# neverorfrog/vehicle-control

Measured on AMD Instinct MI355X. Metric: MPC solves/sec (batched, N=20), higher is better.
Workload: dtype f64; 1 GPU; C2 kinematic-bicycle LTV-MPC, B=1024 per GPU, N=20, fp64; batch_per_gpu=1024, global_batch=1024, horizon=20, parallelism=dp1 (independent shards)

## Files before the change

### include/vcmpc.h

```cpp
#ifndef VCMPC_H
#define VCMPC_H

#include <stdint.h>

#ifdef __cplusplus
extern "C" {
#endif

#define VCMPC_ABI_VERSION 13
#define VC_MAX_OBSTACLES 16

typedef struct vc_ctx vc_ctx;

enum vc_model { VC_MODEL_KINEMATIC = 0, VC_MODEL_DYNAMIC = 1, VC_MODEL_CASCADED = 2 };
enum vc_dtype { VC_F64 = 0, VC_F32 = 1 };
enum vc_flags { VC_HOST_PTRS = 0, VC_DEVICE_PTRS = 1 };
enum vc_tyre { VC_TYRE_FIALA = 0, VC_TYRE_LINEAR = 1 };
enum vc_status { VC_SOLVED = 0, VC_MAX_ITER = 1, VC_NONFINITE = 2, VC_OUT_OF_DOMAIN = 3, VC_INFEASIBLE = 4 };
enum vc_error {
  VC_OK = 0,
  VC_E_ARG = -1,
  VC_E_HIP = -2,
  VC_E_UNSUPPORTED = -3
};

typedef struct vc_kin_car {
  double l;
} vc_kin_car;

typedef struct vc_dyn_car {
  double l, m, Izz, a, b, h, eps, Peng;
  double Xdf, Xdr, Xbf, Xbr;
  double Caf, Car;
  double Cd, muf, mur, theta, phi, Av2, Frr;
  int32_t tyre;
  int32_t pad_;
} vc_dyn_car;

typedef struct vc_kin_mpc {
  double w_time, w_ey, w_epsi, w_v, w_w, w_a, w_dev, w_b;
  double a_min, a_max, w_min, w_max;
  double v_min, v_max, delta_min, delta_max, ey_min, ey_max;
  double w_obs;
} vc_kin_mpc;

typedef struct vc_dyn_mpc {
  double w_time, w_speed, w_ey, w_epsi, w_w, w_Fx, w_dev, w_b, w_slip;
  double w_min, w_max;
  double Ux_min, max_speed, delta_min, delta_max, ey_min, ey_max;
  double fx_scale;
  double trust_Fx;
  int32_t sqp_iters;
  int32_t pad_;
  double w_obs;
} vc_dyn_mpc;

typedef struct vc_qp {
  double prox;
  double tol;
  double trust_a;
  double trust_w;
  int32_t max_iter;
  int32_t polish;
  int32_t solver;
  int32_t kin_sqp;
  int32_t shift;
  int32_t ms;
  double elastic;
} vc_qp;

typedef struct vc_casc_mpc {
  int32_t horizon_pm;
  int32_t pad_;
  double ds_pm;
  double w_dev_pm, w_Fy, w_switch;
  double V_min, ey_min_pm, ey_max_pm;
} vc_casc_mpc;

typedef struct vc_obstacles {
  int32_t n;
  int32_t inside;
  double margin_min;
  double s[VC_MAX_OBSTACLES], ey[VC_MAX_OBSTACLES], radius[VC_MAX_OBSTACLES];
} vc_obstacles;

typedef struct vc_params {
  vc_kin_car kin_car;
  vc_dyn_car dyn_car;
  vc_kin_mpc kin_mpc;
  vc_qp qp;
  vc_dyn_mpc dyn_mpc;
  vc_obstacles obs;
  vc_casc_mpc casc;
} vc_params;

int vc_abi_version(void);
int vc_params_sizeof(void);

vc_ctx* vc_create(int device, int model, int N, int max_batch, int dtype, const vc_params* params);
void vc_destroy(vc_ctx* ctx);
const char* vc_last_error(const vc_ctx* ctx);

int vc_set_stream(vc_ctx* ctx, void* stream);

int vc_set_obstacles(vc_ctx* ctx, int n, const double* s, const double* ey, const double* radius,
                     double margin_min);
int vc_synchronize(vc_ctx* ctx);

int vc_set_infeasibility(vc_ctx* ctx, int on, double eps);

int vc_get_farkas(vc_ctx* ctx, int B, void* y, int flags);

int vc_set_sqp_infeasibility(vc_ctx* ctx, int on, double eps);

int vc_get_sqp_farkas(vc_ctx* ctx, int B, void* y, int32_t* qp_index, int flags);

int vc_set_sqp_regularization(vc_ctx* ctx, int levels, double factor);

int vc_get_sqp_regularization(vc_ctx* ctx, int B, int32_t* level, int flags);

int vc_set_casc_infeasibility(vc_ctx* ctx, int on, double eps);

int vc_get_casc_farkas(vc_ctx* ctx, int B, void* y, int32_t* qp_index, int flags);

int vc_solve(vc_ctx* ctx, int B, const void* x0, const void* kappa, const void* ds,
             void* xbar, void* ubar, void* u0, int32_t* status, int32_t* iters, int flags);

int vc_solve_from(vc_ctx* ctx, int B, const void* x0, const void* kappa, const void* ds, const void* ubar_in,
                  void* xbar, void* u_out, void* u0, int32_t* status, int32_t* iters, int flags);

int vc_solve_diag(vc_ctx* ctx, int B, const void* x0, const void* kappa, const void* ds,
                  void* xbar, void* ubar, void* u0, int32_t* status, int32_t* iters, void* diag,
                  int flags);

int vc_solve_debug(vc_ctx* ctx, int B, const void* x0, const void* kappa, const void* ds, void* xbar, void* ubar,
                   void* u0, int32_t* status, int32_t* iters, void* dbg, int flags);
int vc_debug_stride(void);

int vc_debug_qp_fault(vc_ctx* ctx, int sqp_iter, int problem);

int vc_debug_kin_merit(vc_ctx* ctx, int B, const void* x0, const void* kappa, const void* ds, const void* u_prev,
                       void* u, const void* x_prev, void* x, int32_t* status, int32_t* iters, int32_t* st_acc,
                       int32_t* it_acc, int first, int restart, void* u0, void* ls_diag, int flags);

int vc_debug_sqp_breakdown(vc_ctx* ctx, int sqp_iter, int problem, int levels);

int vc_debug_rcp(vc_ctx* ctx, int n, const void* x, void* out, int flags);

int vc_debug_kin_gdots(vc_ctx* ctx, int B, const void* G, const void* vz, const void* vc, void* out_grow,
                       void* out_gt, int flags);

int vc_rollout(vc_ctx* ctx, int B, const void* x0, const void* ubar, const void* kappa,
               const void* ds, void* xbar, int flags);

int vc_linearize(vc_ctx* ctx, int B, const void* xbar, const void* ubar, const void* kappa,
                 const void* ds, void* A, void* Bm, int flags);

int vc_condense(vc_ctx* ctx, int B, const void* x0, const void* ubar, const void* kappa,
                const void* ds, void* H, void* g, int flags);

int vc_plant_step(vc_ctx* ctx, int B, const void* x, const void* u, const void* kappa,
                  double dt, void* x_next, int flags);

int vc_spatial_step(vc_ctx* ctx, int B, const void* x, const void* u, const void* kappa,
                    const void* ds, void* x_next, int flags);

int vc_ode(vc_ctx* ctx, int B, const void* x, const void* u, const void* kappa, int space, void* f, int flags);

int vc_track_set(vc_ctx* ctx, int n_pieces, double h, double length, const double* coef);

int vc_track_k(vc_ctx* ctx, int B, const void* s, void* k, int flags);

int vc_horizon(vc_ctx* ctx, int B, const void* x0, const void* xbar, double mpc_dt, void* kappa, void* ds,
               int flags);

int vc_drive(vc_ctx* ctx, int B, double* x64, const void* u0, double dt, void* x_ctx, int flags);

int vc_simulate(vc_ctx* ctx, int B, int steps, double mpc_dt, double dt, double* x64, void* xbar, void* ubar,
                double* log_x, void* log_u, int32_t* nfail, int flags);

#ifdef __cplusplus
}
#endif
#endif
```

### vehicle-control_amd/csrc/kin_ltv.hip

```cpp
#include <hip/hip_runtime.h>

#include <cstdint>

#include "vc_kernels.hpp"
#include "vc_models.hpp"
#include "vcmpc.h"

#ifndef VC_KIN_LTV_DET
#define VC_KIN_LTV_DET 0
#endif

#ifndef KIN_NU_TOL
#define KIN_NU_TOL 1e-10
#endif
#ifndef KIN_EARLY_F
#define KIN_EARLY_F 100.0
#endif
#ifndef KIN_EARLY_ROUNDS
#define KIN_EARLY_ROUNDS 2
#endif
#ifndef KIN_TAPIA_F
#define KIN_TAPIA_F 1.02
#endif
#ifndef KIN_DUAL_TOL
#define KIN_DUAL_TOL 1e-12
#endif
#ifndef KIN_AL_RHO
#define KIN_AL_RHO 1e1
#endif
#ifndef KIN_DOT_CH
#define KIN_DOT_CH 8
#endif
#ifndef KIN_UPDATE
#define KIN_UPDATE 1
#endif
#ifndef KIN_RSQ_HALLEY
#define KIN_RSQ_HALLEY 1
#endif
#ifndef KIN_STAT_CHECK
#define KIN_STAT_CHECK 0
#endif
#ifndef KIN_STEP_F
#define KIN_STEP_F 0.99
#endif
#ifndef KIN_SOLVE_CH
#define KIN_SOLVE_CH 8
#endif
#ifndef KIN_PANEL_CH
#define KIN_PANEL_CH 6
#endif

#ifndef KIN_XPOSE_ONCE
#define KIN_XPOSE_ONCE 1
#endif

namespace vc {
namespace {

__device__ __forceinline__ double lane_bcast(double v, int src) {
  const int lo = __builtin_amdgcn_readlane(__double2loint(v), src);
  const int hi = __builtin_amdgcn_readlane(__double2hiint(v), src);
  return __hiloint2double(hi, lo);
}
__device__ int amdgcn_writelane(int v, int lane, int old) __asm("llvm.amdgcn.writelane.i32");
__device__ __forceinline__ double lane_put(double old, double v, int dst) {
  const int lo = amdgcn_writelane(__double2loint(v), dst, __double2loint(old));
  const int hi = amdgcn_writelane(__double2hiint(v), dst, __double2hiint(old));
  return __hiloint2double(hi, lo);
}
template <int K>
__device__ __forceinline__ double dpp_row_shr(double v, double ident) {
  const int lo = __builtin_amdgcn_update_dpp(__double2loint(ident), __double2loint(v), 0x110 + K, 0xf, 0xf, false);
  const int hi = __builtin_amdgcn_update_dpp(__double2hiint(ident), __double2hiint(v), 0x110 + K, 0xf, 0xf, false);
  return __hiloint2double(hi, lo);
}
template <typename Op>
__device__ __forceinline__ double wave_reduce(double v, double ident, Op op) {
  v = op(v, dpp_row_shr<1>(v, ident));
  v = op(v, dpp_row_shr<2>(v, ident));
  v = op(v, dpp_row_shr<4>(v, ident));
  v = op(v, dpp_row_shr<8>(v, ident));
  return op(op(lane_bcast(v, 15), lane_bcast(v, 31)), op(lane_bcast(v, 47), lane_bcast(v, 63)));
}
__device__ __forceinline__ double wave_sum(double v) {
  return wave_reduce(v, 0.0, [](double a, double b) { return a + b; });
}
__device__ __forceinline__ double wave_max(double v) {
  return wave_reduce(v, -__builtin_inf(), [](double a, double b) { return fmax(a, b); });
}
__device__ __forceinline__ double wave_min(double v) {
  return wave_reduce(v, __builtin_inf(), [](double a, double b) { return fmin(a, b); });
}
__device__ __forceinline__ void wave_sync() {
  asm volatile("" ::: "memory");
  __builtin_amdgcn_wave_barrier();
  asm volatile("" ::: "memory");
}
__device__ __forceinline__ void fence() { __builtin_amdgcn_sched_barrier(0); }
__device__ __forceinline__ int lane_opaque(int lane) {
  asm volatile("" : "+v"(lane));
  return lane;
}
__device__ __forceinline__ uint32_t lane_range_pick(uint32_t in, int other, int lo, int hi) {
  uint32_t r;
  asm("s_bfm_b64 vcc, %3, %4\n\t"
      "v_mov_b32_e32 %0, %2\n\tv_cndmask_b32_e32 %0, %0, %1, vcc"
      : "=&v"(r)
      : "v"(in), "i"(other), "i"(hi - lo), "i"(lo)
      : "vcc");
  return r;
}
__device__ __forceinline__ void no_hoist() { asm volatile("" ::: "memory"); }

using lds_cdouble = const __attribute__((address_space(3))) double;
__device__ __forceinline__ lds_cdouble* lds_opaque(const double* p) {
  uint32_t a = (uint32_t)(uintptr_t)(lds_cdouble*)p;
  asm volatile("" : "+v"(a));
  return (lds_cdouble*)(uintptr_t)a;
}

#ifdef VC_TIMING
#define VC_TSTAMP(var) \
  fence();              \
  const uint64_t var = __builtin_amdgcn_s_memtime(); \
  fence();
#define VC_TACC(slot, t0) \
  {                      \
    fence();             \
    tacc[slot] += __builtin_amdgcn_s_memtime() - (t0); \
    fence();             \
  }
#else
#define VC_TSTAMP(var)
#define VC_TACC(slot, t0)
#endif
enum { T_SWEEP = 0, T_SETUP, T_RESID, T_BUILD, T_CHOL, T_SOLVE, T_UPDATE, T_POLISH, T_OUT, T_S2, T_S3, T_S4, T_PAL, T_PPASS, T_NUPD, T_UCYC, T_NDROP, T_CFAIL, T_CRM, T_CADD, T_R0CHG, T_STEP, T_TOTAL, T_NSLOT };


template <int N>
struct Dims {
  static constexpr int n = 2 * N;
  static constexpr int NC = 2 * (N - 1);
  static constexpr int LD = n + 1;
  static_assert(n <= 64 && N >= 2, "one wavefront per problem needs 2 <= N <= 32");
};

template <int n>
__host__ __device__ constexpr int lc_base(int k) {
  static_assert(n % 2 == 0, "even n");
  return k * (n - 1) - k * (k - 1) / 2 + (k + 1) / 2;
}
template <int n>
__host__ __device__ constexpr int lc_start(int k) {
  return lc_base<n>(k) + k;
}

template <int N>
struct Smem {
  using D = Dims<N>;
  static constexpr int LC_DUMMY = lc_start<D::n>(D::n);
  static constexpr int LC_ZERO = LC_DUMMY + 1;
  double G[D::NC + 3][D::LD];
  double H[D::n + 1][D::LD];
  alignas(16) double Lc[LC_ZERO + 1];
  alignas(16) double zrow[48];
  double xb[N + 1][KIN_NX + 1];
  double jac[N + 1][9];
  double ub[D::n];
  double kap[N], ds[N];
  union {
    struct {
      double vz[64];
      double vc[64];
    };
    alignas(16) double tb2[128];
  };
  double dinv[64];
#if KIN_XPOSE_ONCE
  alignas(16) double tb3[8 * 18];
#endif
};
static_assert(sizeof(Smem<20>) <= 40960, "LDS of one problem: four must fit a CU's 160 KB");

template <int N>
__host__ __device__ constexpr int crow_stage(int r) {
  return r < N - 1 ? r + 1 : r - (N - 1) + 1;
}

template <int LEN, int SA, int SB, int CH = KIN_DOT_CH>
__device__ __forceinline__ double lds_dot(lds_cdouble* a, lds_cdouble* b) {
  constexpr int NCH = (LEN + CH - 1) / CH;
  double ca[2][CH], cb[2][CH];
  auto fetch = [&](int c, int buf) {
#pragma unroll
    for (int q = 0; q < CH; ++q) {
      const int i = c * CH + q;
      ca[buf][q] = (i < LEN) ? a[i * SA] : 0.0;
      cb[buf][q] = (i < LEN) ? b[i * SB] : 0.0;
    }
  };
  double a0 = 0.0, a1 = 0.0;
  fetch(0, 0);
#pragma unroll
  for (int c = 0; c < NCH; ++c) {
    if (c + 1 < NCH) fetch(c + 1, (c + 1) & 1);
    fence();
#pragma unroll
    for (int q = 0; q < CH; q += 2) {
      a0 += ca[c & 1][q] * cb[c & 1][q];
      a1 += ca[c & 1][q + 1] * cb[c & 1][q + 1];
    }
  }
  fence();
  return a0 + a1;
}

template <int N>
struct GSplit {
  static_assert(N == 20, "the lane plan below is worked out for N = 20 (the one instantiation)");
  static constexpr int NC = Dims<N>::NC, n = Dims<N>::n, LD = Dims<N>::LD;
  static constexpr int T = NC / 2;
  static constexpr int ROW_SHORT = T - (T + 1) / 2;
  static_assert(NC + 2 * (N - 1 - ROW_SHORT) <= 64, "partner lanes of the long rows");
  static constexpr int COL_LONG = n / 2;
  static_assert(n + COL_LONG <= 64, "partner lanes of the long columns");
};

__device__ __forceinline__ double lane_fetch(double v, int byte_lane) {
  const int lo = __builtin_amdgcn_ds_bpermute(byte_lane, __double2loint(v));
  const int hi = __builtin_amdgcn_ds_bpermute(byte_lane, __double2hiint(v));
  return __hiloint2double(hi, lo);
}

template <int T0, int T1, int GS, int D>
__device__ __forceinline__ void gsplit_fetch(double (&a)[5], double (&b)[5], uint32_t g, uint32_t v) {
  static_assert(2 * T0 - D >= 0, "offsets from a segment base are not negative");
  lds_cdouble* gp = (lds_cdouble*)(uintptr_t)g;
  lds_cdouble* vp = (lds_cdouble*)(uintptr_t)v;
#pragma unroll
  for (int t = T0; t < T1; ++t) {
    a[t - T0] = gp[(2 * t - D) * GS];
    b[t - T0] = vp[2 * t - D];
  }
}
template <int CNT>
__device__ __forceinline__ double gsplit_fma(const double (&a)[5], const double (&b)[5], double acc) {
#pragma unroll
  for (int q = 0; q < CNT; ++q) acc = __builtin_fma(a[q], b[q], acc);
  return acc;
}
template <int N, int GS, int D2, int D3>
__device__ __forceinline__ double gsplit_chain(const uint32_t (&g)[4], const uint32_t (&v)[4], bool shrt,
                                               double& stash) {
  static_assert(GSplit<N>::T == 19, "segments of 5, 5, 4 and 5 steps");
  double a0[5], b0[5], a1[5], b1[5];
  gsplit_fetch<0, 5, GS, 0>(a0, b0, g[0], v[0]);
  gsplit_fetch<5, 10, GS, 0>(a1, b1, g[1], v[1]);
  fence();
  double acc = gsplit_fma<5>(a0, b0, 0.0);
  gsplit_fetch<10, 14, GS, D2>(a0, b0, g[2], v[2]);
  fence();
  acc = gsplit_fma<5>(a1, b1, acc);
  gsplit_fetch<14, 19, GS, D3>(a1, b1, g[3], v[3]);
  fence();
  stash = acc;
  acc = shrt ? 0.0 : acc;
  acc = gsplit_fma<4>(a0, b0, acc);
  fence();
  acc = gsplit_fma<5>(a1, b1, acc);
  fence();
  return acc;
}

template <int N>
__device__ double grow_dot(const Smem<N>& s, int lane) {
  using P = GSplit<N>;
  constexpr int NC = P::NC, LD = P::LD;
  const int l = lane_opaque(lane);
  const bool part = l >= NC;
  const bool shrt = uint32_t(l) < uint32_t(P::ROW_SHORT) || uint32_t(l - (N - 1)) < uint32_t(P::ROW_SHORT);
  const int r = min(part ? l - (l < NC + (N - 1 - P::ROW_SHORT) ? NC - P::ROW_SHORT : N) : l, NC);
  const uint32_t odd = part ? 8u : 0u;
  const uint32_t fwd = shrt ? 0u : 8u * uint32_t(P::T);
  const uint32_t g0 = (uint32_t)(uintptr_t)(lds_cdouble*)&s.G[0][0] + uint32_t(r) * (8u * LD) + odd;
  const uint32_t v0 = (uint32_t)(uintptr_t)(lds_cdouble*)&s.vz[0] + odd;
  const uint32_t g[4] = {g0, g0, g0 + fwd, g0 + fwd}, v[4] = {v0, v0, v0 + fwd, v0 + fwd};
  double stash;
  const double acc = gsplit_chain<N, 1, P::T, P::T>(g, v, shrt, stash);
  const double other = lane_fetch(acc, 4 * (l + (l < N - 1 ? NC - P::ROW_SHORT : N)));
  const double y = acc + (shrt ? stash : other);
  return l < NC ? y : 0.0;
}

template <int N>
__device__ double gt_dot(const Smem<N>& s, int lane) {
  using P = GSplit<N>;
  constexpr int n = P::n, LD = P::LD;
  const int l = lane_opaque(lane);
  const bool part = l >= n;
  const bool shrt = uint32_t(l - P::COL_LONG) < uint32_t(n - P::COL_LONG);
  const int j = part ? l - n : l;
  const uint32_t ms = shrt ? 1u : 0u, mp = part ? 1u : 0u;
  const uint32_t gp = (uint32_t)(uintptr_t)(lds_cdouble*)&s.G[0][0] + uint32_t(j) * 8u + mp * (8u * LD);
  const uint32_t vp = (uint32_t)(uintptr_t)(lds_cdouble*)&s.vc[0] + mp * 8u;
  constexpr int SH[4] = {10, 18, 0, 1}, D[4] = {0, 0, 9, 0};
  uint32_t g[4], v[4];
#pragma unroll
  for (int k = 0; k < 4; ++k) {
    g[k] = gp + uint32_t(D[k] * 8 * LD) + ms * uint32_t((SH[k] - D[k]) * 8 * LD);
    v[k] = vp + uint32_t(D[k] * 8) + ms * uint32_t((SH[k] - D[k]) * 8);
  }
  double stash;
  const double acc = gsplit_chain<N, LD, D[2], D[3]>(g, v, shrt, stash);
  const double other = lane_fetch(acc, 4 * (l + n));
  const double y = acc + (shrt ? stash : other);
  return l < n ? y : 0.0;
}


template <int N>
__device__ double h_dot(const Smem<N>& s, int lane) {
  constexpr int n = Dims<N>::n;
  const int j = lane < n ? lane : 0;
  return lds_dot<n, 1, 1>(lds_opaque(&s.H[j][0]), lds_opaque(&s.vz[0]));
}

__device__ __forceinline__ void kin_sincos(double x, double& sn, double& cs) {
  const double n = __builtin_rint(x * 6.36619772367581382433e-01);
  const double y = fma(-n, 6.07710050650619224932e-11, fma(-n, 1.57079632673412561417e+00, x));
  const double z = y * y;
  const double rs = fma(z, fma(z, fma(z, fma(z, 1.58969099521155010221e-10, -2.50507602534068634195e-08),
                                      2.75573137070700676789e-06), -1.98412698298579493134e-04),
                        8.33333333332248946124e-03);
  const double sk = fma(z * y, fma(z, rs, -1.66666666666666324348e-01), y);
  const double rc = z * fma(z, fma(z, fma(z, fma(z, fma(z, -1.13596475577881948265e-11, 2.08757232129817482790e-09),
                                                  -2.75573143513906633035e-07), 2.48015872894767294178e-05),
                                   -1.38888888888741095749e-03), 4.16666666666666019037e-02);
  const double hz = 0.5 * z, w = 1.0 - hz;
  const double ck = w + (((1.0 - w) - hz) + z * rc);
  const int q = int(n) & 3;
  const double a = (q & 1) ? ck : sk, b = (q & 1) ? sk : ck;
  sn = (q & 2) ? -a : a;
  cs = ((q + 1) & 2) ? -b : b;
}

__device__ __forceinline__ double rsq_nr(double d) {
  double inv = __builtin_amdgcn_rsq(d);
#if KIN_RSQ_HALLEY
  const double e = fma(-d, inv * inv, 1.0);
  return fma(inv * e, fma(0.375, e, 0.5), inv);
#else
  inv = inv * (1.5 - 0.5 * d * inv * inv);
  inv = inv * (1.5 - 0.5 * d * inv * inv);
  return inv;
#endif
}

template <int N>
__device__ __forceinline__ void store_rows(const double (&Mr)[Dims<N>::n], Smem<N>& s, int lane) {
}

template <int N>
struct RowRegs {
  int lo[Dims<N>::n], hi[Dims<N>::n];
};
template <int N>
__device__ __forceinline__ void row_put(RowRegs<N>& R, int k, double v) {
  asm("v_accvgpr_write_b32 %0, %1" : "=a"(R.lo[k]) : "v"(__double2loint(v)));
  asm("v_accvgpr_write_b32 %0, %1" : "=a"(R.hi[k]) : "v"(__double2hiint(v)));
}
#define KIN_FS_STEP(k, w, lo)                    \
  "v_mul_f64 v[252:253], %[acc], %[dj]\n\t"      \
  "s_bfm_b64 exec, " #w ", " #lo "\n\t"          \
  "v_readlane_b32 vcc_lo, v252, " #k "\n\t"      \
  "v_readlane_b32 vcc_hi, v253, " #k "\n\t"      \
  "v_accvgpr_read_b32 v254, %[l" #k "]\n\t"      \
  "v_accvgpr_read_b32 v255, %[h" #k "]\n\t"      \
  "v_fma_f64 %[acc], -v[254:255], vcc, %[acc]\n\t"
#define KIN_FS_ROW(k) [l##k] "a"(Lr.lo[k]), [h##k] "a"(Lr.hi[k])
template <int N>
__device__ __forceinline__ void forward_sweep(const RowRegs<N>& Lr, double& acc, double dj) {
  static_assert(Dims<N>::n == 40, "the sweep's 40 steps are written out");
  asm("s_mov_b64 s[98:99], exec\n\t"
      KIN_FS_STEP(0,63,1) KIN_FS_STEP(1,62,2) KIN_FS_STEP(2,61,3)
      KIN_FS_STEP(3,60,4) KIN_FS_STEP(4,59,5) KIN_FS_STEP(5,58,6)
      KIN_FS_STEP(6,57,7) KIN_FS_STEP(7,56,8) KIN_FS_STEP(8,55,9)
      KIN_FS_STEP(9,54,10) KIN_FS_STEP(10,53,11) KIN_FS_STEP(11,52,12)
      KIN_FS_STEP(12,51,13) KIN_FS_STEP(13,50,14) KIN_FS_STEP(14,49,15)
      KIN_FS_STEP(15,48,16) KIN_FS_STEP(16,47,17) KIN_FS_STEP(17,46,18)
      KIN_FS_STEP(18,45,19) KIN_FS_STEP(19,44,20) KIN_FS_STEP(20,43,21)
      KIN_FS_STEP(21,42,22) KIN_FS_STEP(22,41,23) KIN_FS_STEP(23,40,24)
      KIN_FS_STEP(24,39,25) KIN_FS_STEP(25,38,26) KIN_FS_STEP(26,37,27)
      KIN_FS_STEP(27,36,28) KIN_FS_STEP(28,35,29) KIN_FS_STEP(29,34,30)
      KIN_FS_STEP(30,33,31) KIN_FS_STEP(31,32,32) KIN_FS_STEP(32,31,33)
      KIN_FS_STEP(33,30,34) KIN_FS_STEP(34,29,35) KIN_FS_STEP(35,28,36)
      KIN_FS_STEP(36,27,37) KIN_FS_STEP(37,26,38) KIN_FS_STEP(38,25,39)
      KIN_FS_STEP(39,24,40)
      "s_mov_b64 exec, s[98:99]"
      : [acc] "+v"(acc)
      : [dj] "v"(dj),
        KIN_FS_ROW(0), KIN_FS_ROW(1), KIN_FS_ROW(2), KIN_FS_ROW(3), KIN_FS_ROW(4), KIN_FS_ROW(5),
        KIN_FS_ROW(6), KIN_FS_ROW(7), KIN_FS_ROW(8), KIN_FS_ROW(9), KIN_FS_ROW(10), KIN_FS_ROW(11),
        KIN_FS_ROW(12), KIN_FS_ROW(13), KIN_FS_ROW(14), KIN_FS_ROW(15), KIN_FS_ROW(16), KIN_FS_ROW(17),
        KIN_FS_ROW(18), KIN_FS_ROW(19), KIN_FS_ROW(20), KIN_FS_ROW(21), KIN_FS_ROW(22), KIN_FS_ROW(23),
        KIN_FS_ROW(24), KIN_FS_ROW(25), KIN_FS_ROW(26), KIN_FS_ROW(27), KIN_FS_ROW(28), KIN_FS_ROW(29),
        KIN_FS_ROW(30), KIN_FS_ROW(31), KIN_FS_ROW(32), KIN_FS_ROW(33), KIN_FS_ROW(34), KIN_FS_ROW(35),
        KIN_FS_ROW(36), KIN_FS_ROW(37), KIN_FS_ROW(38), KIN_FS_ROW(39)
      : "vcc", "s98", "s99", "v252", "v253", "v254", "v255");
}
#undef KIN_FS_STEP
#undef KIN_FS_ROW

template <int N>
__device__ double chol_solve(const RowRegs<N>& Lr, const Smem<N>& s, double b, int lane) {
  constexpr int n = Dims<N>::n;
  constexpr int CH = KIN_SOLVE_CH;
  static_assert(n % CH == 0, "backward prefetch chunks");
  const int row = lane < n ? lane : 0;
  lds_cdouble* col = lds_opaque(&s.Lc[lc_base<n>(row)]);
  const double dj = s.dinv[row];
  double acc = b;
  forward_sweep<N>(Lr, acc, dj);
  acc *= dj;
  double x = 0.0;
  double lk[2][CH];
  lds_cdouble* zero = lds_opaque(&s.zrow[0]);
  auto fetch = [&](int c, int buf) {
    lds_cdouble* src = row < n - 1 - c * CH ? col : zero;
#pragma unroll
    for (int q = 0; q < CH; ++q) lk[buf][q] = src[n - 1 - c * CH - q];
  };
  fetch(0, 0);
#pragma unroll
  for (int c = 0; c < n / CH; ++c) {
    if (c + 1 < n / CH) fetch(c + 1, (c + 1) & 1);
    fence();
#pragma unroll
    for (int q = 0; q < CH; ++q) {
      const int k = n - 1 - c * CH - q;
      const double xk = lane_bcast(acc * dj, k);
      x = lane_put(x, xk, k);
      acc -= lk[c & 1][q] * xk;
    }
    fence();
  }
  return x;
}

enum { ROWS_G = 0, ROWS_E = 1 };
template <int N, int KIND>
__host__ __device__ constexpr int row_extent(int r) {
  if (KIND == ROWS_G) return r < Dims<N>::NC ? 2 * crow_stage<N>(r) : 0;
  return r < N ? 2 * (r + 1) : (r < N + 2 ? 2 * N : 0);
}
template <int N, int KIND>
__host__ __device__ constexpr int gram_rows() {
  return KIND == ROWS_G ? Dims<N>::NC : N + 2;
}
template <int N, int KIND>
__host__ __device__ constexpr bool kstep_hits(int ks, int I) {
  for (int q = 0; q < 4; ++q)
    if (row_extent<N, KIND>(4 * ks + q) > 16 * I) return true;
  return false;
}

using d4 = __attribute__((ext_vector_type(4))) double;
using d2 = __attribute__((ext_vector_type(2))) double;
template <int N>
struct Tiles {
  static constexpr int n = Dims<N>::n, NB = (n + 15) / 16, NT = NB * (NB + 1) / 2, BLD = 16 * NB + 2;
  static constexpr int count(bool full) { return full ? NB * NB : NT; }
};

template <int N, int KIND, bool FULL>
__device__ __forceinline__ void gram_mfma(d4 (&acc)[Tiles<N>::count(FULL)], const double* rows, const double* w,
                                          int lane) {
  constexpr int n = Dims<N>::n, LD = Dims<N>::LD, NB = Tiles<N>::NB;
  constexpr int KS = (gram_rows<N, KIND>() + 3) / 4;
  lane = lane_opaque(lane);
  const int lr = lane >> 4, lc = lane & 15;
  lds_cdouble* R = lds_opaque(rows);
  lds_cdouble* W = lds_opaque(w);
  double gk[KS][NB], wk[KS];
#pragma unroll
  for (int ks = 0; ks < KS; ++ks) {
    const int r = 4 * ks + lr;
    wk[ks] = W[r];
#pragma unroll
    for (int J = 0; J < NB; ++J) {
      const int c = 16 * J + lc;
      gk[ks][J] = R[r * LD + (c < n ? c : n)];
    }
  }
  fence();
#pragma unroll
  for (int ks = 0; ks < KS; ++ks) {
#pragma unroll
    for (int I = 0, t = 0; I < NB; ++I) {
      const double a = wk[ks] * gk[ks][I];
#pragma unroll
      for (int J = 0; J < (FULL ? NB : I + 1); ++J, ++t)
        if (kstep_hits<N, KIND>(ks, I > J ? I : J))
          acc[t] = __builtin_amdgcn_mfma_f64_16x16x4f64(a, gk[ks][J], acc[t], 0, 0, 0);
    }
  }
}

template <int N, bool FULL>
__device__ __forceinline__ void tiles_to_rows(double (&Mr)[Dims<N>::n], const d4 (&acc)[Tiles<N>::count(FULL)],
                                              Smem<N>& s, int lane) {
  constexpr int n = Dims<N>::n, NB = Tiles<N>::NB, BLD = Tiles<N>::BLD;
  static_assert(16 * BLD <= Smem<N>::LC_DUMMY, "transpose buffer must fit the factor storage");
  static_assert(16 * NB <= 48, "zero row length");
  lane = lane_opaque(lane);
  const int lr = lane >> 4, lc = lane & 15;
  double* buf = &s.Lc[0];
  const int myI = lane >> 4;
#pragma unroll
  for (int I = 0, t0 = 0; I < NB; ++I, t0 += FULL ? NB : I) {
    wave_sync();
#pragma unroll
    for (int J = 0; J < (FULL ? NB : I + 1); ++J) {
#pragma unroll
      for (int q = 0; q < 4; ++q) buf[(lr + 4 * q) * BLD + 16 * J + lc] = acc[t0 + J][q];
    }
    wave_sync();
    using lds_cd2 = const __attribute__((address_space(3))) d2;
    lds_cd2* brow = (lds_cd2*)lds_opaque(myI == I ? &buf[lc * BLD] : &s.zrow[0]);
#pragma unroll
    for (int i = 0; i < n; i += 2) {
      const int iend = FULL ? n : 16 * (I + 1);
      if (i < iend) {
        const d2 p = brow[i / 2];
        if (I == 0) { Mr[i] = p.x; Mr[i + 1] = p.y; }
        else { Mr[i] += p.x; Mr[i + 1] += p.y; }
      } else if (I == 0) {
        Mr[i] = 0.0;
        Mr[i + 1] = 0.0;
      }
    }
  }
  wave_sync();
}

template <int N>
__device__ __forceinline__ void build_normal_acc(d4 (&acc)[Tiles<N>::NT], Smem<N>& s, double wb, double hjj, int lane) {
  constexpr int n = Dims<N>::n, LD = Dims<N>::LD, NB = Tiles<N>::NB;
  static_assert(4 * ((Dims<N>::NC + 3) / 4) <= Dims<N>::NC + 2, "G zero rows cover the last k-step");
  lane = lane_opaque(lane);
  const int lr = lane >> 4, lc = lane & 15;
  const int jd = lane < n ? lane : n;
  s.H[jd][jd] = hjj + wb;
  wave_sync();
  {
    lds_cdouble* H = lds_opaque(&s.H[0][0]);
#pragma unroll
    for (int I = 0, t = 0; I < NB; ++I) {
#pragma unroll
      for (int J = 0; J <= I; ++J, ++t) {
        const int c = 16 * J + lc < n ? 16 * J + lc : n;
#pragma unroll
        for (int q = 0; q < 4; ++q) {
          const int r0 = 16 * I + 4 * q;
          acc[t][q] = r0 < n ? H[(r0 + lr) * LD + c] : 0.0;
        }
      }
    }
  }
  s.H[jd][jd] = hjj;
  gram_mfma<N, ROWS_G, false>(acc, &s.G[0][0], &s.vc[0], lane);
}

template <int N>
__device__ __forceinline__ void build_normal_mfma(double (&Mr)[Dims<N>::n], Smem<N>& s, double wb, double hjj,
                                                  int lane) {
  d4 acc[Tiles<N>::NT];
  build_normal_acc<N>(acc, s, wb, hjj, lane);
  tiles_to_rows<N, false>(Mr, acc, s, lane);
}

template <int N>
__device__ bool factor_blocked(RowRegs<N>& Lr, d4 (&acc)[Tiles<N>::NT], Smem<N>& s, int lane) {
  constexpr int n = Dims<N>::n, NB = Tiles<N>::NB;
  double Mr[n];
  constexpr int DUMMY = Smem<N>::LC_DUMMY;
  static_assert(NB == 3 && n > 32 && n <= 40, "three panels, the last one at most 8 wide");
  static_assert(lc_start<n>(16) + 16 * 18 <= DUMMY, "panel 0/1 transpose buffer inside the factor storage");
  static_assert((lc_start<n>(16) & 1) == 0, "16-byte aligned transpose buffer");
  lane = lane_opaque(lane);
  const int lr = lane >> 4, lc = lane & 15, myI = lane >> 4;
  bool ok = true;
  double pa, pb, pc, pi1, pl21, pi2;
  using lds_double = __attribute__((address_space(3))) double;
  using lds_char = __attribute__((address_space(3))) char;
  const uint32_t lane8 = 8u * uint32_t(lane);
  auto col_store = [&](int k, double v) {
    const uint32_t off = lane_range_pick(lane8, 8 * (DUMMY - lc_base<n>(k)), k, n);
    *(lds_double*)((lds_char*)&s.Lc[lc_base<n>(k)] + off) = v;
  };
  auto part = [&](int p, int k) {
    if (p == 0) {
      pa = lane_bcast(Mr[k], k);
      pb = lane_bcast(Mr[k], k + 1);
      pc = lane_bcast(Mr[k + 1], k + 1);
      pi1 = rsq_nr(pa);
    } else if (p == 1) {
      pl21 = pb * pi1;
      const double d2 = fma(-pl21, pl21, pc);
      pi2 = rsq_nr(d2);
      ok = ok && (pa > 0.0) && (d2 > 0.0);
    } else {
      const double x = Mr[k] * pi1;
      const double y = fma(-x, pl21, Mr[k + 1]) * pi2;
      Mr[k] = x;
      Mr[k + 1] = y;
      col_store(k, x);
      col_store(k + 1, y);
      s.dinv[k] = pi1;
      s.dinv[k + 1] = pi2;
    }
  };
  using lds_cd2 = const __attribute__((address_space(3))) d2;
#pragma unroll
  for (int p = 0; p < NB; ++p) {
    const int c0 = 16 * p, c1 = (16 * p + 16 < n) ? 16 * p + 16 : n, W = c1 - c0;
    double* tb = p < 2 ? &s.Lc[lc_start<n>(16)] : &s.tb2[0];
    const int TS = p < 2 ? 18 : 10;
#if KIN_XPOSE_ONCE
    static_assert(2 * 16 * 18 + 8 * 18 <= DUMMY, "panel 0's three buffers inside the factor storage");
    {
      auto tbuf = [&](int I) -> double* {
        return p == 0 ? &s.Lc[16 * 18 * I] : (p == 1 ? (I == 1 ? tb : &s.tb3[0]) : tb);
      };
      wave_sync();
#pragma unroll
      for (int I = p; I < NB; ++I) {
        const int t = I * (I + 1) / 2 + p;
        double* tbI = tbuf(I);
#pragma unroll
        for (int q = 0; q < 4; ++q) {
          const int r = lr + 4 * q;
          if (16 * I + 4 * q < n)
            tbI[(lc < W ? r * TS + lc : 8 * TS + lc)] = acc[t][q];
        }
      }
      wave_sync();
      const double* own = p == 0 ? &s.Lc[16 * 18 * myI + lc * TS]
                                 : (p == 1 ? (myI == 1 ? &tb[lc * TS] : &s.tb3[lc * TS]) : &tb[lc * TS]);
      lds_cd2* src = (lds_cd2*)lds_opaque(myI >= p && lane < n ? own : &s.zrow[0]);
#pragma unroll
      for (int i = 0; i < W; i += 2) {
        const d2 v = src[i / 2];
        Mr[c0 + i] = 0.0 + v.x;
        Mr[c0 + i + 1] = 0.0 + v.y;
      }
    }
#else
#pragma unroll
    for (int i = c0; i < c1; ++i) Mr[i] = 0.0;
#pragma unroll
    for (int I = p; I < NB; ++I) {
      const int t = I * (I + 1) / 2 + p;
      wave_sync();
#pragma unroll
      for (int q = 0; q < 4; ++q) {
        const int r = lr + 4 * q;
        if (4 * q < W)
          tb[(lc < W ? r * TS + lc : 8 * TS + lc)] = acc[t][q];
      }
      wave_sync();
      lds_cd2* src = (lds_cd2*)lds_opaque(myI == I && lc < W ? &tb[lc * TS] : &s.zrow[0]);
#pragma unroll
      for (int i = 0; i < W; i += 2) {
        const d2 v = src[i / 2];
        Mr[c0 + i] += v.x;
        Mr[c0 + i + 1] += v.y;
      }
    }
#endif
    wave_sync();
    part(0, c0);
    part(1, c0);
    part(2, c0);
#pragma unroll
    for (int k = c0; k + 2 < c1; k += 2) {
      wave_sync();
      fence();
      const double x = Mr[k], y = Mr[k + 1];
      const double* cA = &s.Lc[lc_base<n>(k)];
      const double* cB = &s.Lc[lc_base<n>(k + 1)];
      constexpr int CH = KIN_PANEL_CH;
      const int J0 = k + 4, NCH = (c1 - J0 + CH - 1) / CH;
      double u0[2][CH], u1[2][CH];
      auto load = [&](int ch, int buf) {
#pragma unroll
        for (int q = 0; q < CH; ++q) {
          const int j = J0 + ch * CH + q;
          u0[buf][q] = j < c1 ? cA[j] : 0.0;
          u1[buf][q] = j < c1 ? cB[j] : 0.0;
        }
      };
      if (NCH > 0) load(0, 0);
#pragma unroll
      for (int j = k + 2; j < k + 4; ++j)
        Mr[j] = fma(-y, lane_bcast(y, j), fma(-x, lane_bcast(x, j), Mr[j]));
      part(0, k + 2);
#pragma unroll
      for (int ch = 0; ch < NCH; ++ch) {
        if (ch + 1 < NCH) load(ch + 1, (ch + 1) & 1);
        fence();
#pragma unroll
        for (int q = 0; q < CH; ++q) {
          const int j = J0 + ch * CH + q;
          if (j < c1) Mr[j] = fma(-y, u1[ch & 1][q], fma(-x, u0[ch & 1][q], Mr[j]));
        }
        if (ch + 1 < 3) part(ch + 1, k + 2);
        fence();
      }
#pragma unroll
      for (int pp = NCH + 1; pp < 3; ++pp) {
        part(pp, k + 2);
        fence();
      }
    }
    wave_sync();
    if (p + 1 < NB) {
      lds_cdouble* Lc = lds_opaque(&s.Lc[0]);
      lds_cdouble* Z = lds_opaque(&s.zrow[0]);
#pragma unroll
      for (int ks = 0; ks < W / 4; ++ks) {
        const int kk = c0 + 4 * ks + lr;
        double op[NB];
#pragma unroll
        for (int I = p + 1; I < NB; ++I) {
          const int jj = 16 * I + lc;
          op[I] = jj < n ? Lc[lc_base<n>(kk) + jj] : Z[0];
        }
#pragma unroll
        for (int I = p + 1; I < NB; ++I) {
#pragma unroll
          for (int J = p + 1; J <= I; ++J) {
            const int t = I * (I + 1) / 2 + J;
            acc[t] = __builtin_amdgcn_mfma_f64_16x16x4f64(-op[I], op[J], acc[t], 0, 0, 0);
          }
        }
      }
    }
  }
#pragma unroll
  for (int k = 0; k < n; ++k) row_put<N>(Lr, k, Mr[k]);
  wave_sync();
  return ok;
}

__device__ __forceinline__ double wave_prefix(double v, int lane) {
  v += dpp_row_shr<1>(v, 0.0);
  v += dpp_row_shr<2>(v, 0.0);
  v += dpp_row_shr<4>(v, 0.0);
  v += dpp_row_shr<8>(v, 0.0);
  const double r0 = lane_bcast(v, 15), r1 = lane_bcast(v, 31), r2 = lane_bcast(v, 47);
  return v + (lane >= 16 ? r0 : 0.0) + (lane >= 32 ? r1 : 0.0) + (lane >= 48 ? r2 : 0.0);
}

template <int N>
__device__ bool factor_update(RowRegs<N>& Lr, Smem<N>& s, int upd, int j, bool fixed, double sqrho,
                              int lane) {
  constexpr int n = Dims<N>::n;
  double Mr[n];
  constexpr int DUMMY = Smem<N>::LC_DUMMY, ZERO = Smem<N>::LC_ZERO;
  lane = lane_opaque(lane);
  const int row = lane < n ? lane : 0;
  auto below = [&](int k, int other) { return lane > k && lane < n ? lc_base<n>(k) + lane : other; };
  double z;
  if (upd == 1) {
    z = s.Lc[below(j, ZERO)];
    wave_sync();
    s.Lc[below(j, DUMMY)] = 0.0;
    s.Lc[lane < j ? lc_base<n>(lane) + j : DUMMY] = 0.0;
    s.Lc[lc_start<n>(j)] = 1.0;
    s.dinv[j] = 1.0;
  } else {
    z = (lane < n && !fixed) ? sqrho * s.G[j][lane < n ? lane : n] : 0.0;
  }
  wave_sync();
  {
    lds_cdouble* L = lds_opaque(&s.Lc[0]);
#pragma unroll
    for (int k = 0; k < n; ++k) Mr[k] = L[below(k, ZERO)];
  }
#pragma unroll
  for (int k = 0; k < n; ++k) row_put<N>(Lr, k, Mr[k]);
  const double dj = s.dinv[row];
  double acc = z;
  forward_sweep<N>(Lr, acc, dj);
  const double y = lane < n ? acc * dj : 0.0;
  const double t = 1.0 + wave_prefix(y * y, lane);
  const double sk = sqrt(t / (t - y * y)), ck = y / t;
  const bool ok = __ballot(!(sk > 0.5 && sk < 1e150)) == 0ull;
  wave_sync();
  if (lane < n) {
    s.Lc[lc_start<n>(row)] *= sk;
    s.dinv[row] = dj / sk;
  }
  s.tb2[2 * lane] = ck;
  s.tb2[2 * lane + 1] = sk;
  wave_sync();
  {
    using lds_cd2 = const __attribute__((address_space(3))) d2;
    lds_cd2* cs = (lds_cd2*)lds_opaque(&s.tb2[0]);
    double w = z;
#pragma unroll
    for (int k = 0; k < n - 1; ++k) {
      const double yk = lane_bcast(y, k);
      const d2 c = cs[k];
      w = lane_put(w, 0.0, k);
      const double l = Mr[k];
      w = fma(-yk, l, w);
      Mr[k] = fma(c.x, w, l) * c.y;
    }
  }
#pragma unroll
  for (int k = 0; k < n - 1; ++k) s.Lc[below(k, DUMMY)] = Mr[k];
#pragma unroll
  for (int k = 0; k < n; ++k) row_put<N>(Lr, k, Mr[k]);
  wave_sync();
  return ok;
}

struct Side {
  double lo, hi, slo, shi, llo, lhi;
  bool hasLo, hasHi;
};

}

template <int N, bool DET>
__global__ __launch_bounds__(64) void kin_ltv_kernel(KinLtvArgs A) {
  using D = Dims<N>;
  constexpr int n = D::n, NC = D::NC;
  __shared__ Smem<N> s;
  const int lane = threadIdx.x;
  const int b = xcd_problem(blockIdx.x, A.B);
  if (b >= A.B) return;
  const vc_kin_mpc& W = A.w;
#ifdef VC_TIMING
  uint64_t tacc[T_NSLOT] = {};
#endif
  VC_TSTAMP(t_all0)

  if (lane < n) s.ub[lane] = A.ubar[(size_t)b * n + lane];
  if (lane < N) {
    s.kap[lane] = A.kappa[(size_t)b * N + lane];
    s.ds[lane] = A.ds[(size_t)b * N + lane];
  }
  if (lane < KIN_NX) s.xb[0][lane] = A.x0[(size_t)b * KIN_NX + lane];
  for (int i = lane; i < 2 * D::LD; i += 64) (&s.G[NC][0])[i] = 0.0;
  if (lane < 48) s.zrow[lane] = 0.0;
  if (lane == 0) s.Lc[Smem<N>::LC_ZERO] = 0.0;
  wave_sync();

  VC_TSTAMP(t_sweep0)
  constexpr int LD = Dims<N>::LD;
  double* E = &s.H[0][0];
  bool finite = true;
  {
    double x[KIN_NX];
#pragma unroll
    for (int i = 0; i < KIN_NX; ++i) x[i] = s.xb[0][i];
#pragma unroll 1
    for (int k = 0; k < N; ++k) {
      const double u2[2] = {s.ub[2 * k], s.ub[2 * k + 1]};
      const double h = s.ds[k];
      double f[KIN_NX];
      {
        double sn, cs;
        kin_sincos((lane & 1) ? x[1] : x[4], sn, cs);
        const double se = lane_bcast(sn, 0), ce = lane_bcast(cs, 0);
        const double sd = lane_bcast(sn, 1), cd = lane_bcast(cs, 1);
        const double kap = s.kap[k];
        const double rho = 1.0 - x[3] * kap;
        const int r4 = lane & 3;
        const double num = r4 == 0 ? se : (r4 == 1 ? sd : rho);
        const double den = r4 == 0 ? ce : (r4 == 1 ? cd * A.L : (r4 == 2 ? ce : x[0] * ce));
        const double quo = num * rcp_nr(den);
        const double te = lane_bcast(quo, 0), tdl = lane_bcast(quo, 1);
        const double rc = lane_bcast(quo, 2), q = lane_bcast(quo, 3);
        f[0] = q * u2[0];
        f[1] = q * u2[1];
        f[2] = 1.0;
        f[3] = rho * te;
        f[4] = tdl * rc - kap;
        f[5] = q;
      }
#pragma unroll
      for (int i = 0; i < KIN_NX; ++i) x[i] += h * f[i];
      if (lane == 0) {
#pragma unroll
        for (int i = 0; i < KIN_NX; ++i) s.xb[k + 1][i] = x[i];
      }
    }
#pragma unroll
    for (int i = 0; i < KIN_NX; ++i) finite = finite && isfinite(x[i]);
  }
  wave_sync();
  if (lane < N) {
    const double ey = s.xb[lane + 1][3];
    double cw, lin;
    if (lane + 1 < N) {
      const double hs = s.ds[lane + 1];
      const double td = W.w_dev * hs;
      double tb = W.w_b * hs;
      asm volatile("" : "+v"(tb));
      cw = td;
      lin = ey * td;
      if (ey < W.ey_min) { cw = __builtin_fma(W.w_dev, hs, tb); lin = __builtin_fma(ey - W.ey_min, tb, lin); }
      if (ey > W.ey_max) { cw = cw + tb; lin = __builtin_fma(ey - W.ey_max, tb, lin); }
    } else {
      cw = W.w_ey;
      lin = W.w_ey * ey;
    }
    s.vc[lane] = 2.0 * cw;
    s.vz[lane] = 2.0 * lin;
  }
  wave_sync();
  VC_TACC(T_SWEEP, t_sweep0)
  VC_TSTAMP(t_s20)
  {
    const int k = lane < N ? lane : 0;
    double xk[KIN_NX];
#pragma unroll
    for (int i = 0; i < KIN_NX; ++i) xk[i] = s.xb[k][i];
    const KinJac J = kin_spatial_jac(xk, s.kap[k], A.L);
    double* jr = s.jac[lane < N ? lane : N];
    jr[0] = J.q; jr[1] = J.qv; jr[2] = J.qey; jr[3] = J.qep;
    jr[4] = J.J33; jr[5] = J.J34; jr[6] = J.J41; jr[7] = J.J43; jr[8] = J.J44;
    if (A.obs.n > 0 && lane >= 1 && lane < N) {
      double p, q;
      obstacle_ey_model<double>(A.obs, xk[2], xk[3], W.w_obs * s.ds[k], p, q);
      s.vc[k - 1] += q;
      s.vz[k - 1] += p;
    }
  }
  wave_sync();
  VC_TACC(T_S2, t_s20)
  VC_TSTAMP(t_s30)
  double gj = 0.0;
  double cv = 0, cd = 0, cey = 0, cep = 0, ct = 0;
  {
    const int jcol = lane < n ? lane : n;
    double jn[9], hn, an, wn;
    auto fetch = [&](int k) {
#pragma unroll
      for (int q = 0; q < 9; ++q) jn[q] = s.jac[k][q];
      hn = s.ds[k]; an = s.ub[2 * k]; wn = s.ub[2 * k + 1];
    };
    fetch(0);
#pragma unroll 1
    for (int k = 0; k < N; ++k) {
      double J[9];
#pragma unroll
      for (int q = 0; q < 9; ++q) J[q] = jn[q];
      const double h = hn, a = an, w = wn;
      const double lin2 = s.vz[k];
      if (k + 1 < N) fetch(k + 1);
      const double dq = J[1] * cv + J[2] * cey + J[3] * cep;
      const double ncv = cv + h * a * dq + (lane == 2 * k ? h * J[0] : 0.0);
      const double ncd = cd + h * w * dq + (lane == 2 * k + 1 ? h * J[0] : 0.0);
      const double ncey = cey + h * (J[4] * cey + J[5] * cep);
      const double ncep = cep + h * (J[6] * cd + J[7] * cey + J[8] * cep);
      ct += h * dq;
      cv = ncv; cd = ncd; cey = ncey; cep = ncep;
      const bool has = k + 1 <= N - 1;
      s.G[has ? k : NC + 2][jcol] = cv;
      s.G[has ? (N - 1) + k : NC + 2][jcol] = cd;
      E[k * LD + jcol] = cey;
      gj += lin2 * cey;
    }
    E[N * LD + jcol] = cv;
    E[(N + 1) * LD + jcol] = cep;
  }
  wave_sync();
  VC_TACC(T_S3, t_s30)
  VC_TSTAMP(t_s40)
  double Hr[n];
  double hjj;
  {
    const double vN = s.xb[N][0];
    const double cwv = (vN >= W.v_max) ? W.w_v : 0.0;
    gj += 2.0 * cwv * (vN - W.v_max) * cv;
    gj += 2.0 * W.w_epsi * s.xb[N][4] * cep;
    gj += W.w_time * ct;
    if (lane < 4) s.vc[N + lane] = lane == 0 ? 2.0 * cwv : (lane == 1 ? 2.0 * W.w_epsi : 0.0);
    for (int i = lane; i < 2 * LD; i += 64) E[(N + 2) * LD + i] = 0.0;
    wave_sync();
    d4 acc[Tiles<N>::count(true)];
#pragma unroll
    for (int t = 0; t < Tiles<N>::count(true); ++t) acc[t] = d4{0.0, 0.0, 0.0, 0.0};
    gram_mfma<N, ROWS_E, true>(acc, E, &s.vc[0], lane);
    tiles_to_rows<N, true>(Hr, acc, s, lane);
  }
  const int kq = lane >> 1;
  double dself = 2.0 * A.qp.prox, dm2 = 0.0, dp2 = 0.0;
  if (lane < n) {
    if (lane & 1) {
      dself += 2.0 * W.w_w;
      gj += 2.0 * W.w_w * s.ub[lane];
    } else {
      if (kq >= 1) {
        dself += 2.0 * W.w_a; dm2 = -2.0 * W.w_a;
        gj += 2.0 * W.w_a * (s.ub[lane] - s.ub[lane - 2]);
      }
      if (kq <= N - 2) {
        dself += 2.0 * W.w_a; dp2 = -2.0 * W.w_a;
        gj -= 2.0 * W.w_a * (s.ub[lane + 2] - s.ub[lane]);
      }
    }
  }
  gj = (lane < n) ? gj : 0.0;
  {
    const int j = lane < n ? lane : n;
#pragma unroll
    for (int i = 0; i < n; ++i) s.H[j][i] = Hr[i];
    s.H[j][n] = 0.0;
    s.H[j][j] += dself;
    s.H[j][j >= 2 ? j - 2 : j] += dm2;
    s.H[j][j + 2 < n ? j + 2 : j] += dp2;
    hjj = lane < n ? s.H[j][j] : 0.0;
  }
  wave_sync();
  if (A.mode == 1) {
    if (lane < n) {
#pragma unroll
      for (int i = 0; i < n; ++i) A.H_out[((size_t)b * n + lane) * n + i] = s.H[lane][i];
      A.g_out[(size_t)b * n + lane] = gj;
    }
    return;
  }

  VC_TACC(T_S4, t_s40)
  VC_TSTAMP(t_setup0)
  Side bx, cs;
  {
    const bool isw = lane & 1;
    const double u = (lane < n) ? s.ub[lane] : 0.0;
    bx.lo = (isw ? W.w_min : W.a_min) - u;
    bx.hi = (isw ? W.w_max : W.a_max) - u;
    const double tr = isw ? A.qp.trust_w : A.qp.trust_a;
    if (tr > 0.0) {
      bx.lo = fmax(bx.lo, -tr);
      bx.hi = fmin(bx.hi, tr);
    }
    bx.hasLo = bx.hasHi = (lane < n);
    const int st = crow_stage<N>(lane < NC ? lane : 0);
    if (lane < N - 1) {
      cs.lo = W.v_min - s.xb[st][0];
      cs.hi = 0.0;
      cs.hasLo = true; cs.hasHi = false;
    } else if (lane < NC) {
      cs.lo = W.delta_min - s.xb[st][1];
      cs.hi = W.delta_max - s.xb[st][1];
      cs.hasLo = cs.hasHi = true;
    } else {
      cs.lo = cs.hi = 0.0;
      cs.hasLo = cs.hasHi = false;
    }
  }
  const double mtot = double(4 * N + 3 * (N - 1));
  double scale, hdiag_max;
  {
    double m = fabs(gj);
    if (bx.hasLo) m = fmax(m, fabs(bx.lo));
    if (bx.hasHi) m = fmax(m, fabs(bx.hi));
    if (cs.hasLo) m = fmax(m, fabs(cs.lo));
    if (cs.hasHi) m = fmax(m, fabs(cs.hi));
    scale = 1.0 + wave_max(m);
    hdiag_max = fmax(wave_max(hjj), 1.0);
  }
  double z = 0.0;
  bx.slo = bx.hasLo ? fmax(-bx.lo, 1.0) : 1.0;
  bx.shi = bx.hasHi ? fmax(bx.hi, 1.0) : 1.0;
  bx.llo = bx.hasLo ? 1.0 : 0.0;
  bx.lhi = bx.hasHi ? 1.0 : 0.0;
  cs.slo = cs.hasLo ? fmax(-cs.lo, 1.0) : 1.0;
  cs.shi = cs.hasHi ? fmax(cs.hi, 1.0) : 1.0;
  cs.llo = cs.hasLo ? 1.0 : 0.0;
  cs.lhi = cs.hasHi ? 1.0 : 0.0;
  [[maybe_unused]] double Rbox = 0.0, l1_inf = 1.0;
  [[maybe_unused]] bool infeas = false;
  if constexpr (DET) Rbox = wave_sum(lane < n ? fmax(bx.hi, -bx.lo) : 0.0);

  VC_TACC(T_SETUP, t_setup0)
  const int max_iter = A.qp.max_iter;
  const double tol = A.qp.tol * scale;
  int it = 0;
  bool converged = false, chol_fail = false, near = false;
  double last_res = 0.0, last_mu = 0.0;
  RowRegs<N> Mr;
  double rd = 0.0, rlo_b = 0.0, rhi_b = 0.0, rlo_c = 0.0, rhi_c = 0.0;
  auto true_residuals = [&]() {
    wave_sync();
    s.vz[lane] = (lane < n) ? z : 0.0;
    s.vc[lane] = (lane < NC) ? (cs.lhi - cs.llo) : 0.0;
    wave_sync();
    const double yc = grow_dot<N>(s, lane);
    fence();
    const double hz = h_dot<N>(s, lane);
    fence();
    const double gtl = gt_dot<N>(s, lane);
    rd = (lane < n) ? (hz + gj + (bx.lhi - bx.llo) + gtl) : 0.0;
    rlo_b = bx.hasLo ? (z - bx.lo - bx.slo) : 0.0;
    rhi_b = bx.hasHi ? (bx.hi - z - bx.shi) : 0.0;
    rlo_c = cs.hasLo ? (yc - cs.lo - cs.slo) : 0.0;
    rhi_c = cs.hasHi ? (cs.hi - yc - cs.shi) : 0.0;
  };
  auto max_residual = [&]() {
    return wave_max(fmax(fmax(fabs(rd), fmax(fabs(rlo_b), fabs(rhi_b))), fmax(fabs(rlo_c), fabs(rhi_c))));
  };
  int tapb = 0;
  const double tol_early = KIN_EARLY_F > 0.0 ? fmax(tol, KIN_EARLY_F * tol) : tol;
  int e_set = 0;
#ifdef VC_TIMING
  uint64_t e_fmask = 0;
  bool e_row = false, e_have = false;
#endif
  double tol_cur = tol_early;
  bool polished = false, pchol_fail = false;
  int rounds = 0;
#pragma unroll 1
  for (;;) {
  if (finite) {
#pragma unroll 1
    for (;;) {
      no_hoist();
      VC_TSTAMP(t_res0)
      if (it == 0) true_residuals();
      const double mu = wave_sum(__builtin_fma(cs.shi, cs.lhi,
                                               __builtin_fma(cs.slo, cs.llo,
                                                             __builtin_fma(bx.shi, bx.lhi, bx.slo * bx.llo)))) / mtot;
      double res = max_residual();
      if (it > 0 && res <= tol_cur && mu <= tol_cur) {
        true_residuals();
        res = max_residual();
      }
      converged = res <= tol_cur && mu <= tol_cur;
      last_res = res;
      last_mu = mu;
      if (converged || it >= max_iter || !isfinite(res) || !isfinite(mu)) break;
      if constexpr (DET) {
        if (it >= 1) {
          const double dcs = __builtin_fma(cs.hi, cs.lhi, -(cs.lo * cs.llo));
          const double dl = wave_sum(__builtin_fma(bx.hi, bx.lhi, __builtin_fma(-bx.lo, bx.llo, dcs)));
          if (dl < 0.0) {
            const double l1 = wave_sum((bx.llo + bx.lhi) + (cs.llo + cs.lhi));
            wave_sync();
            s.vc[lane] = (lane < NC) ? (cs.lhi - cs.llo) : 0.0;
            wave_sync();
            const double gtl = gt_dot<N>(s, lane);
            const double cmax = wave_max(lane < n ? fabs((bx.lhi - bx.llo) + gtl) : 0.0);
            if (__builtin_fma(Rbox, cmax, dl) / l1 < -A.detect_eps) {
              infeas = true;
              l1_inf = l1;
              break;
            }
            const double q = lane < n ? gtl : 0.0;
            const double aq = fabs(q);
            const double l1s = wave_sum((cs.llo + cs.lhi) + aq);
            const double dys = wave_sum(__builtin_fma(q > 0.0 ? -bx.lo : bx.hi, aq, dcs));
            if (dys / l1s < -A.detect_eps) {
              infeas = true;
              l1_inf = l1s;
              bx.lhi = fmax(-q, 0.0);
              bx.llo = fmax(q, 0.0);
              break;
            }
          }
        }
      }
      ++it;
      const double wlo_b = bx.hasLo ? bx.llo / bx.slo : 0.0;
      const double whi_b = bx.hasHi ? bx.lhi / bx.shi : 0.0;
      const double wlo_c = cs.hasLo ? cs.llo / cs.slo : 0.0;
      const double whi_c = cs.hasHi ? cs.lhi / cs.shi : 0.0;
      wave_sync();
      s.vc[lane] = (lane < NC) ? wlo_c + whi_c : 0.0;
      wave_sync();
      VC_TACC(T_RESID, t_res0)
      VC_TSTAMP(t_build0)
      d4 nacc[Tiles<N>::NT];
      build_normal_acc<N>(nacc, s, wlo_b + whi_b, hjj, lane);
      VC_TACC(T_BUILD, t_build0)
      VC_TSTAMP(t_chol0)
      const bool chol_ok = factor_blocked<N>(Mr, nacc, s, lane);
      VC_TACC(T_CHOL, t_chol0)
      if (!chol_ok) {
        chol_fail = true;
        near = res <= 1e-6 * scale && mu <= tol;
        break;
      }
#ifdef VC_TIMING
      const uint64_t t_sol_before = tacc[T_SOLVE];
#endif
      VC_TSTAMP(t_step0)
      const double islo_b = bx.hasLo ? rcp_nr(bx.slo) : 0.0, ishi_b = bx.hasHi ? rcp_nr(bx.shi) : 0.0;
      const double islo_c = cs.hasLo ? rcp_nr(cs.slo) : 0.0, ishi_c = cs.hasHi ? rcp_nr(cs.shi) : 0.0;
      const double illo_b = bx.hasLo ? rcp_nr(bx.llo) : 0.0, ilhi_b = bx.hasHi ? rcp_nr(bx.lhi) : 0.0;
      const double illo_c = cs.hasLo ? rcp_nr(cs.llo) : 0.0, ilhi_c = cs.hasHi ? rcp_nr(cs.lhi) : 0.0;
      double sm = 0.0, pp1 = 0.0, pp2 = 0.0, pp3 = 0.0, pp4 = 0.0;
#pragma unroll 1
      for (int pass = 0; pass < 2; ++pass) {
        no_hoist();
        const double rclo_b = __builtin_fma(bx.slo, bx.llo, pp1) - sm, rchi_b = __builtin_fma(bx.shi, bx.lhi, pp2) - sm;
        const double rclo_c = __builtin_fma(cs.slo, cs.llo, pp3) - sm, rchi_c = __builtin_fma(cs.shi, cs.lhi, pp4) - sm;
        const double thi_b = ishi_b * -rchi_b, thi_c = ishi_c * -rchi_c;
        const double tlo_b = islo_b * rclo_b, tlo_c = islo_c * rclo_c;
        const double eb = (bx.hasHi ? __builtin_fma(-whi_b, rhi_b, thi_b) : 0.0) +
                          (bx.hasLo ? __builtin_fma(wlo_b, rlo_b, tlo_b) : 0.0);
        const double ec = (cs.hasHi ? __builtin_fma(-whi_c, rhi_c, thi_c) : 0.0) +
                          (cs.hasLo ? __builtin_fma(wlo_c, rlo_c, tlo_c) : 0.0);
        wave_sync();
        s.vc[lane] = (lane < NC) ? ec : 0.0;
        wave_sync();
        const double gte = gt_dot<N>(s, lane);
        const double rhs = (lane < n) ? (-rd - eb - gte) : 0.0;
        VC_TSTAMP(t_sol0)
        const double dz = chol_solve<N>(Mr, s, rhs, lane);
        VC_TACC(T_SOLVE, t_sol0)
        wave_sync();
        s.vz[lane] = (lane < n) ? dz : 0.0;
        wave_sync();
        const double dyc = grow_dot<N>(s, lane);
        const double d1 = bx.hasLo ? dz + rlo_b : 0.0;
        const double d2 = bx.hasLo ? __builtin_fma(islo_b, -rclo_b, -(wlo_b * (dz + rlo_b))) : 0.0;
        const double d3 = bx.hasHi ? rhi_b - dz : 0.0;
        const double d4 = bx.hasHi ? __builtin_fma(-whi_b, rhi_b - dz, thi_b) : 0.0;
        const double e1 = cs.hasLo ? dyc + rlo_c : 0.0;
        const double e2 = cs.hasLo ? __builtin_fma(islo_c, -rclo_c, -(wlo_c * (dyc + rlo_c))) : 0.0;
        const double e3 = cs.hasHi ? rhi_c - dyc : 0.0;
        const double e4 = cs.hasHi ? __builtin_fma(-whi_c, rhi_c - dyc, thi_c) : 0.0;
        const double tmax = wave_max(fmax(fmax(fmax(-d1 * islo_b, -d2 * illo_b), fmax(-d3 * ishi_b, -d4 * ilhi_b)),
                                          fmax(fmax(-e1 * islo_c, -e2 * illo_c), fmax(-e3 * ishi_c, -e4 * ilhi_c))));
        const double amax = 1.0 / fmax(1.0, tmax);
        if (pass == 0) {
          const double mua = wave_sum((bx.slo + amax * d1) * (bx.llo + amax * d2) +
                                      (bx.shi + amax * d3) * (bx.lhi + amax * d4) +
                                      (cs.slo + amax * e1) * (cs.llo + amax * e2) +
                                      (cs.shi + amax * e3) * (cs.lhi + amax * e4)) / mtot;
          const double sr = mua / mu;
          sm = sr * sr * sr * mu;
          pp1 = d1 * d2; pp2 = d3 * d4; pp3 = e1 * e2; pp4 = e3 * e4;
        } else {
          const double al = KIN_STEP_F * amax;
          {
            auto tap = [&](double dl, double il, double dsv, double is) -> int {
              const double lr = fma(al * dl, il, 1.0), sr = fma(al * dsv, is, 1.0);
              return lr > KIN_TAPIA_F * sr ? 1 : (sr > KIN_TAPIA_F * lr ? 2 : 0);
            };
            tapb = tap(d2, illo_b, d1, islo_b) | (tap(d4, ilhi_b, d3, ishi_b) << 2) |
                   (tap(e2, illo_c, e1, islo_c) << 4) | (tap(e4, ilhi_c, e3, ishi_c) << 6);
          }
          z = (lane < n) ? z + al * dz : z;
          bx.slo += al * d1; bx.llo += al * d2; bx.shi += al * d3; bx.lhi += al * d4;
          cs.slo += al * e1; cs.llo += al * e2; cs.shi += al * e3; cs.lhi += al * e4;
          const double om = 1.0 - al;
          rd *= om; rlo_b *= om; rhi_b *= om; rlo_c *= om; rhi_c *= om;
        }
      }
      VC_TACC(T_STEP, t_step0)
#ifdef VC_TIMING
      tacc[T_STEP] -= tacc[T_SOLVE] - t_sol_before;
#endif
    }
  }

  VC_TSTAMP(t_pol0)
  if ((converged || near) && A.qp.polish > 0) {
    constexpr double AL_RHO = KIN_AL_RHO;
    constexpr int AL_MAX = 16;
    const double ptol = 1e-9 * scale, dtol = KIN_DUAL_TOL * scale;
    auto guess = [&](bool has, double l, double sv, int t) { return has && (t == 1 || (t == 0 && l > sv)); };
    bool alo_b = guess(bx.hasLo, bx.llo, bx.slo, tapb & 3);
    bool ahi_b = guess(bx.hasHi, bx.lhi, bx.shi, (tapb >> 2) & 3);
    bool alo_c = guess(cs.hasLo, cs.llo, cs.slo, (tapb >> 4) & 3);
    bool ahi_c = guess(cs.hasHi, cs.lhi, cs.shi, (tapb >> 6) & 3);
    auto pack = [&]() { return int(alo_b) | (int(ahi_b) << 1) | (int(alo_c) << 2) | (int(ahi_c) << 3); };
    if (tol_cur <= tol && __ballot(e_set != 0 && pack() != (e_set & 15)) == 0ull && __ballot(e_set != 0) != 0ull) {
      const int t = e_set >> 4;
      alo_b = t & 1; ahi_b = (t >> 1) & 1; alo_c = (t >> 2) & 1; ahi_c = (t >> 3) & 1;
    }
    const int max_rounds = tol_cur > tol ? min(A.qp.polish, KIN_EARLY_ROUNDS) : A.qp.polish;
    double rho_k = 0.0;
    int upd = 0, upd_j = 0;
#pragma unroll 1
    for (int round = 0; round < max_rounds; ++round) {
      no_hoist();
      const int set0 = pack();
#ifdef VC_TIMING
      if (round == 0 && tol_cur <= tol && e_have) {
        const bool fx = (lane < n) && (alo_b || ahi_b);
        const uint64_t fm = __ballot(fx);
        const bool ract = (lane < NC) && (alo_c || ahi_c);
        tacc[T_CFAIL] = 1;
        tacc[T_CRM] = __builtin_popcountll(e_fmask & ~fm) + __builtin_popcountll(__ballot(e_row && !ract));
        tacc[T_CADD] = __builtin_popcountll(fm & ~e_fmask) + __builtin_popcountll(__ballot(ract && !e_row));
      }
#endif
      ++rounds;
      const bool fixed = (lane < n) && (alo_b || ahi_b);
      const double zfix = fixed ? (alo_b ? bx.lo : bx.hi) : 0.0;
      const uint64_t fmask = __ballot(fixed);
      const bool act = (lane < NC) && (alo_c || ahi_c);
      wave_sync();
      s.vz[lane] = (lane < n) ? zfix : 0.0;
      wave_sync();
      const double gfix = grow_dot<N>(s, lane);
      double gn2 = 0.0;
      {
        const int r = lane < NC ? lane : 0;
#pragma unroll 2
        for (int i = 0; i < 2 * (N - 1); ++i) {
          const double gi = ((fmask >> i) & 1ull) ? 0.0 : s.G[r][i];
          gn2 += gi * gi;
        }
      }
      const double rho_new = (act && gn2 > 1e-28) ? AL_RHO * hdiag_max / gn2 : 0.0;
      const double rho_c = (KIN_UPDATE && rho_k > 0.0 && rho_new > 0.0) ? rho_k : rho_new;
      const double bnd_c = act ? ((alo_c ? cs.lo : cs.hi) - gfix) : 0.0;
      const double base = (lane < n) ? -(gj + h_dot<N>(s, lane)) : 0.0;
      wave_sync();
      s.vc[lane] = rho_c;
      wave_sync();
      VC_TSTAMP(t_pf0)
      bool updated = false;
      if (KIN_UPDATE && upd != 0) {
        const bool same = __ballot(lane < NC && rho_c != rho_k && !(upd == 2 && lane == upd_j)) == 0ull;
        VC_TSTAMP(t_u0)
        if (same) updated = factor_update<N>(Mr, s, upd, upd_j, fixed, sqrt(lane_bcast(rho_c, upd_j)), lane);
#ifdef VC_TIMING
        if (updated) tacc[T_NUPD] += 1;
#endif
        VC_TACC(T_UCYC, t_u0)
      }
      rho_k = rho_c;
      if (!updated) {
        d4 pacc[Tiles<N>::NT];
        build_normal_acc<N>(pacc, s, 0.0, hjj, lane);
        const int pl = lane_opaque(lane), plr = pl >> 4, plc = pl & 15;
#pragma unroll
        for (int I = 0, t = 0; I < Tiles<N>::NB; ++I) {
#pragma unroll
          for (int J = 0; J <= I; ++J, ++t) {
            const int c = 16 * J + plc;
            const bool fc = (fmask >> c) & 1ull;
#pragma unroll
            for (int q = 0; q < 4; ++q) {
              const int r = 16 * I + plr + 4 * q;
              const bool fr = (fmask >> r) & 1ull;
              pacc[t][q] = (fr || fc) ? (r == c ? 1.0 : 0.0) : pacc[t][q];
            }
          }
        }
        if (!factor_blocked<N>(Mr, pacc, s, lane)) {
          pchol_fail = true;
          break;
        }
      }
      VC_TACC(T_UPDATE, t_pf0)
      VC_TSTAMP(t_pal0)
      double nu_c = (act && rho_c > 0.0) ? ((ahi_c ? cs.lhi : 0.0) - (alo_c ? cs.llo : 0.0)) : 0.0;

      const bool al_act = act && rho_c > 0.0;
      const double bnd_al = alo_c ? cs.lo : cs.hi;
      double zp = 0.0, emax = 0.0;
      {
        wave_sync();
        s.vc[lane] = (lane < NC) ? (nu_c - rho_c * bnd_c) : 0.0;
        wave_sync();
        const double gtn = gt_dot<N>(s, lane);
        const double rhs = (lane < n) ? (fixed ? zfix : (base - gtn)) : 0.0;
        zp = chol_solve<N>(Mr, s, rhs, lane);
        wave_sync();
        s.vz[lane] = (lane < n) ? zp : 0.0;
        wave_sync();
        const double yr = grow_dot<N>(s, lane);
        double rr = al_act ? (yr - bnd_al) : 0.0;
        const double ie = 1.0 / (1e-14 * scale), inu = KIN_NU_TOL > 0.0 ? 1.0 / (KIN_NU_TOL * scale) : 0.0;
        auto crit = [&](double r) { return wave_max(fmax(fabs(r) * ie, fabs(rho_c * r) * inu)); };
#ifdef VC_TIMING
        tacc[T_PPASS] += 1;
#endif
        if (crit(rr) > 1.0) {
          double pd = rho_c * rr;
          double rz = wave_sum(rr * pd);
#pragma unroll 1
          for (int it = 1; it < AL_MAX; ++it) {
            no_hoist();
            wave_sync();
            s.vc[lane] = (lane < NC) ? pd : 0.0;
            wave_sync();
            const double gtp = gt_dot<N>(s, lane);
            const double zq = chol_solve<N>(Mr, s, (lane < n && !fixed) ? gtp : 0.0, lane);
            wave_sync();
            s.vz[lane] = (lane < n) ? zq : 0.0;
            wave_sync();
            const double gq = grow_dot<N>(s, lane);
            const double q = al_act ? gq : 0.0;
            const double pq = wave_sum(pd * q);
#ifdef VC_TIMING
            tacc[T_PPASS] += 1;
#endif
            if (!(pq > 0.0)) break;
            const double al = rz / pq;
            nu_c = fma(al, pd, nu_c);
            zp = fma(-al, zq, zp);
            rr = fma(-al, q, rr);
            if (crit(rr) <= 1.0) break;
            const double zt = rho_c * rr;
            const double rzn = wave_sum(rr * zt);
            pd = fma(rzn / rz, pd, zt);
            rz = rzn;
          }
        }
      }
      VC_TACC(T_PAL, t_pal0)
      wave_sync();
      s.vz[lane] = (lane < n) ? zp : 0.0;
      s.vc[lane] = (lane < NC) ? nu_c : 0.0;
      wave_sync();
      const double gtnu = gt_dot<N>(s, lane);
      const double grad = (lane < n) ? (h_dot<N>(s, lane) + gj + gtnu) : 0.0;
      const double ypc = grow_dot<N>(s, lane);
#if KIN_STAT_CHECK
      emax = wave_max(fmax(al_act ? fabs(ypc - bnd_al) : 0.0, (lane < n && !fixed) ? fabs(grad) : 0.0));
#else
      emax = wave_max(al_act ? fabs(ypc - bnd_al) : 0.0);
#endif
      const double dv_b = (lane < n) ? (ahi_b ? grad : (alo_b ? -grad : -1.0)) : -1.0;
      const double dv_c = (lane < NC) ? (ahi_c ? -nu_c : (alo_c ? nu_c : -1.0)) : -1.0;
      const double pv_b = (lane < n && !fixed) ? fmax(bx.lo - zp, zp - bx.hi) : -1.0;
      const double pv_c = (lane < NC && !(act && rho_c > 0.0))
                              ? fmax(cs.hasLo ? cs.lo - ypc : -1.0, cs.hasHi ? ypc - cs.hi : -1.0)
                              : -1.0;
      const double dmax = wave_max(fmax(dv_b, dv_c));
      const double pmax = wave_max(fmax(pv_b, pv_c));
      if (dmax <= dtol && pmax <= ptol) {
        if (emax <= ptol) {
          z = (lane < n) ? zp : z;
          polished = true;
        }
        break;
      }
      const bool dual = dmax > dtol;
      const double worst = dual ? dmax : pmax;
      const double vb = dual ? dv_b : pv_b, vcr = dual ? dv_c : pv_c;
      const uint64_t who = __ballot(fmax(vb, vcr) == worst);
      const int sel = __builtin_ffsll((long long)who) - 1;
      const bool sel_box = (__ballot(vb >= vcr) >> sel) & 1ull;
      upd = dual ? 0 : (sel_box ? 1 : 2);
      upd_j = sel;
#ifdef VC_TIMING
      if (dual) tacc[T_NDROP] += 1;
#endif
      if (lane == sel) {
        if (vb >= vcr) {
          if (dual) { alo_b = false; ahi_b = false; }
          else if (zp < bx.lo) alo_b = true;
          else ahi_b = true;
        } else {
          if (dual) { alo_c = false; ahi_c = false; }
          else if (ypc < cs.lo) alo_c = true;
          else ahi_c = true;
        }
      }
#ifdef VC_TIMING
      int r0code = 0;
      if (tol_cur > tol && round == 0) {
        int tside = 0;
        if (vb >= vcr) tside = (dual ? (ahi_b ? (tapb >> 2) : tapb) : (zp < bx.lo ? tapb : (tapb >> 2))) & 3;
        else tside = (dual ? (ahi_c ? (tapb >> 6) : (tapb >> 4)) : (ypc < cs.lo ? (tapb >> 4) : (tapb >> 6))) & 3;
        const int code = 1 + (dual ? 2 : (vb >= vcr ? 0 : 1)) + 3 * tside;
        r0code = __builtin_amdgcn_readlane(code, sel);
#ifdef VC_TIMING
        tacc[T_R0CHG] = (uint64_t)r0code;
#endif
      }
#endif
      if (tol_cur > tol) e_set = 256 | set0 | (pack() << 4);
#ifdef VC_TIMING
      if (tol_cur > tol) {
        e_fmask = fmask;
        e_row = rho_k > 0.0;
        e_have = true;
      }
#endif
    }
  }

  VC_TACC(T_POLISH, t_pol0)
  if (polished || !converged || chol_fail || tol_cur <= tol) break;
  tol_cur = tol;
  converged = false;
  pchol_fail = false;
  }
  VC_TSTAMP(t_out0)
  int32_t st;
  if (!finite) st = VC_NONFINITE;
  else if (polished || converged) st = VC_SOLVED;
  else st = VC_MAX_ITER;
  if (!finite) z = 0.0;
  if constexpr (DET) {
    if (infeas) {
      st = VC_INFEASIBLE;
      z = 0.0;
    }
    if (A.farkas) {
      double* fk = A.farkas + (size_t)b * (7 * N - 3);
      if (lane < n) {
        fk[2 * lane] = infeas ? bx.lhi / l1_inf : 0.0;
        fk[2 * lane + 1] = infeas ? bx.llo / l1_inf : 0.0;
      }
      if (lane < N - 1) {
        fk[4 * N + 3 * lane] = infeas ? cs.llo / l1_inf : 0.0;
      } else if (lane < NC) {
        const int r = lane - (N - 1);
        fk[4 * N + 3 * r + 1] = infeas ? cs.lhi / l1_inf : 0.0;
        fk[4 * N + 3 * r + 2] = infeas ? cs.llo / l1_inf : 0.0;
      }
    }
  }
  wave_sync();
  if (lane < n) {
    s.vz[lane] = z;
    A.u_out[(size_t)b * n + lane] = s.ub[lane] + z;
  }
  wave_sync();
  if (lane < 2) A.u0[(size_t)b * 2 + lane] = s.ub[lane] + s.vz[lane];
  if (lane == 0) {
    A.status[b] = st;
    A.iters[b] = it;
    if (A.diag) {
#ifdef VC_TIMING
      constexpr size_t DS = 4 + T_NSLOT;
#else
      constexpr size_t DS = 4;
#endif
      A.diag[(size_t)b * DS + 0] = last_res / scale;
      A.diag[(size_t)b * DS + 1] = last_mu / scale;
      A.diag[(size_t)b * DS + 2] = double((chol_fail ? 1 : 0) | (converged ? 2 : 0) | (polished ? 4 : 0) |
                                          (pchol_fail ? 8 : 0) | (DET && infeas ? 32 : 0));
      A.diag[(size_t)b * DS + 3] = double(rounds);
    }
  }
  {
    const double y = grow_dot<N>(s, lane);
    const int slot = lane < N - 1 ? 64 + lane + 1
                                  : (lane < NC ? n + (lane - (N - 1)) + 1 : (lane == NC ? 64 : (lane == NC + 1 ? n : 127)));
    wave_sync();
    s.tb2[slot] = y;
    wave_sync();
    double ey = 0.0, ep = 0.0, eyk = 0.0, epk = 0.0;
#pragma unroll 4
    for (int k = 0; k < N; ++k) {
      const double h = s.ds[k], dd = s.vz[n + k];
      eyk = lane_put(eyk, ey, k);
      epk = lane_put(epk, ep, k);
      const double ney = ey + h * (s.jac[k][4] * ey + s.jac[k][5] * ep);
      const double nep = ep + h * (s.jac[k][6] * dd + s.jac[k][7] * ey + s.jac[k][8] * ep);
      ey = ney; ep = nep;
    }
    eyk = lane_put(eyk, ey, N);
    epk = lane_put(epk, ep, N);
    const double eyn = __shfl_down(eyk, 1), epn = __shfl_down(epk, 1);
    const int k = lane < N ? lane : 0;
    const double q = s.jac[k][0], qv = s.jac[k][1], qey = s.jac[k][2], qep = s.jac[k][3];
    const double h = s.ds[k], a = s.ub[2 * k], w = s.ub[2 * k + 1];
    const double da = s.vz[2 * k], dw = s.vz[2 * k + 1];
    const double dv = s.vc[k], dd = s.vz[n + k];
    const double dq = qv * dv + qey * eyk + qep * epk;
    const double dt = wave_prefix(lane < N ? h * dq : 0.0, lane);
    wave_sync();
    if (lane < N) {
      double* xr = s.xb[k + 1];
      xr[0] += dv + h * (a * dq + q * da);
      xr[1] += dd + h * (w * dq + q * dw);
      xr[3] += eyn;
      xr[4] += epn;
      xr[5] += dt;
    }
    wave_sync();
    double* xo = A.x_out + (size_t)b * (N + 1) * KIN_NX;
    for (int i = lane; i < (N + 1) * KIN_NX; i += 64) xo[i] = s.xb[i / KIN_NX][i % KIN_NX];
  }
  VC_TACC(T_OUT, t_out0)
  VC_TACC(T_TOTAL, t_all0)
#ifdef VC_TIMING
  if (A.diag && lane < T_NSLOT) {
    double v = 0.0;
#pragma unroll
    for (int i = 0; i < T_NSLOT; ++i) v = (i == lane) ? double(tacc[i]) : v;
    A.diag[(size_t)b * (4 + T_NSLOT) + 4 + lane] = v;
  }
#endif
}

#if VC_KIN_LTV_DET
hipError_t launch_kin_ltv_det(const KinLtvArgs& a, int N, hipStream_t stream) {
  if (a.B <= 0) return hipSuccess;
  switch (N) {
    case 20:
      hipLaunchKernelGGL((kin_ltv_kernel<20, true>), dim3(a.B), dim3(64), 0, stream, a);
      return hipGetLastError();
    default:
      return hipErrorInvalidValue;
  }
}
#else
template <int N>
__global__ __launch_bounds__(64) void kin_gdots_kernel(int B, const double* G, const double* vz, const double* vc,
                                                       double* out_grow, double* out_gt) {
  constexpr int n = Dims<N>::n, NC = Dims<N>::NC, LD = Dims<N>::LD;
  __shared__ Smem<N> s;
  const int lane = threadIdx.x;
  const int b = blockIdx.x;
  if (b >= B) return;
  for (int i = lane; i < (NC + 3) * LD; i += 64) (&s.G[0][0])[i] = 0.0;
  wave_sync();
  for (int i = lane; i < NC * n; i += 64) s.G[i / n][i % n] = G[(size_t)b * NC * n + i];
  s.vz[lane] = lane < n ? vz[(size_t)b * n + lane] : 0.0;
  s.vc[lane] = lane < NC ? vc[(size_t)b * NC + lane] : 0.0;
  wave_sync();
  out_grow[(size_t)b * 64 + lane] = grow_dot<N>(s, lane);
  out_gt[(size_t)b * 64 + lane] = gt_dot<N>(s, lane);
}

hipError_t launch_kin_gdots(int B, int N, const double* G, const double* vz, const double* vc, double* out_grow,
                            double* out_gt, hipStream_t stream) {
  if (B <= 0) return hipSuccess;
  if (N != 20) return hipErrorInvalidValue;
  hipLaunchKernelGGL(kin_gdots_kernel<20>, dim3(B), dim3(64), 0, stream, B, G, vz, vc, out_grow, out_gt);
  return hipGetLastError();
}

size_t kin_ltv_smem_bytes(int N) {
  switch (N) {
    case 20: return sizeof(Smem<20>);
    default: return 0;
  }
}

hipError_t launch_kin_ltv(const KinLtvArgs& a, int N, hipStream_t stream) {
  if (a.B <= 0) return hipSuccess;
  if (a.detect && a.mode == 0) return launch_kin_ltv_det(a, N, stream);
  switch (N) {
    case 20:
      hipLaunchKernelGGL((kin_ltv_kernel<20, false>), dim3(a.B), dim3(64), 0, stream, a);
      return hipGetLastError();
    default:
      return hipErrorInvalidValue;
  }
}
#endif

}
```

### vehicle-control_amd/csrc/vc_kernels.hpp

```cpp
#pragma once
#include <hip/hip_runtime.h>

#include <cstddef>
#include <cstdint>

#include "vc_models.hpp"
#include "vcmpc.h"

#ifdef VC_TIMING
#define VC_DIAG_COLS 16
#define VC_DYN_DIAG_COLS 19
#define VC_CASC_DIAG_COLS 17
#define VC_ST_DIAG_COLS 13
#else
#define VC_DIAG_COLS 4
#define VC_DYN_DIAG_COLS 4
#define VC_CASC_DIAG_COLS 4
#define VC_ST_DIAG_COLS 4
#endif

#define VC_OBS_MARGIN_MIN 0.05

namespace vc {

__device__ __forceinline__ int xcd_problem(int g, int B) {
  const int q = B >> 3;
  return g < 8 * q ? (g & 7) * q + (g >> 3) : g;
}

inline int device_cus() {
  int dev = 0, n = 0;
  if (hipGetDevice(&dev) != hipSuccess || hipDeviceGetAttribute(&n, hipDeviceAttributeMultiprocessorCount, dev) != hipSuccess)
    return 256;
  return n > 0 ? n : 256;
}
constexpr int wg_per_cu(size_t lds) {
  const size_t g = (lds + 511) / 512 * 512, n = 163840 / (g ? g : 1);
  return n < 4 ? (int)n : 4;
}

struct GBuf {
  __amdgpu_buffer_rsrc_t r;
  static __device__ __forceinline__ double* uniform(double* p) {
    const uint64_t u = (uint64_t)p;
    const uint32_t lo = __builtin_amdgcn_readfirstlane((uint32_t)u), hi = __builtin_amdgcn_readfirstlane((uint32_t)(u >> 32));
    return (double*)(((uint64_t)hi << 32) | lo);
  }
  __device__ __forceinline__ GBuf(double* base, uint32_t bytes)
      : r(__builtin_amdgcn_make_buffer_rsrc(base, (short)0, (int)bytes, 0x00020000)) {}
  __device__ __forceinline__ double ld(uint32_t off) const {
    return __builtin_bit_cast(double, __builtin_amdgcn_raw_buffer_load_b64(r, off, 0, 0));
  }

  __device__ __forceinline__ void st(uint32_t off, double v) const {
    typedef __attribute__((ext_vector_type(2))) unsigned u2;
    __builtin_amdgcn_raw_buffer_store_b64(__builtin_bit_cast(u2, v), r, off, 0, 0);
  }
  __device__ __forceinline__ void st2(uint32_t off, double v0, double v1) const {
    typedef __attribute__((ext_vector_type(4))) unsigned u4;
    typedef __attribute__((ext_vector_type(2))) double d2v;
    const d2v v = {v0, v1};
    __builtin_amdgcn_raw_buffer_store_b128(__builtin_bit_cast(u4, v), r, off, 0, 0);
  }
};

__device__ __forceinline__ double rcp_nr(double x) {
  const double r0 = __builtin_amdgcn_rcp(x);
  double e = fma(-x, r0, 1.0);
  double r = fma(r0, e, r0);
  e = fma(-x, r, 1.0);
  r = fma(r, e, r);
  return isfinite(r) ? r : r0;
}

constexpr int DOM_HALVINGS = 8;
template <typename T>
__device__ __forceinline__ bool dyn_in_domain(const T* x, T kappa) {
  const T sdot = (x[0] * cos(x[6]) - x[1] * sin(x[6])) / (T(1) - kappa * x[5]);
  return x[0] > T(0) && sdot > T(0);
}

template <typename T>
__device__ __forceinline__ bool pm_in_domain(const T* p, T kappa) {
  const T sdot = p[0] * cos(p[3]) / (T(1) - kappa * p[2]);
  return p[0] > T(0) && sdot > T(0);
}

template <typename T>
__device__ __forceinline__ void obstacle_ey_model(const vc_obstacles& o, T s, T ey, T wds, T& p, T& q) {
  T ps = T(0), qs = T(0);
  const T mmin = T(o.margin_min);
  for (int j = 0; j < o.n; ++j) {
    const T a = s - T(o.s[j]);
    const T e = ey - T(o.ey[j]);
    const T d2 = a * a + e * e;
    const T d = sqrt(d2);
    const T dc = d > T(1e-6) ? d : T(1e-6);
    const T m0 = d - (T(o.radius[j]) + T(0.1));
    const T m = (o.inside && m0 < -mmin) ? m0 : (m0 > mmin ? m0 : mmin);
    const T d1 = e / dc;
    const T dd = (a * a) / (dc * dc * dc);
    const T im = T(1) / m;
    const T c1 = wds * im * im;
    ps -= c1 * d1;
    qs += c1 * (T(2) * d1 * d1 * im - dd);
  }
  p = ps;
  q = qs > T(0) ? qs : T(0);
}

template <int R>
struct StageRows8 {
  double m[R][8];
  __device__ __forceinline__ double& at(int k, int i) { return m[k][(i + (k >> 2)) & 7]; }
  __device__ __forceinline__ const double& at(int k, int i) const { return m[k][(i + (k >> 2)) & 7]; }
};

struct KinLtvArgs {
  const double* x0;
  const double* kappa;
  const double* ds;
  const double* ubar;
  double* u_out;
  double* x_out;
  const double* x_in;
  double* u0;
  int32_t* status;
  int32_t* iters;
  double* diag;
  double* H_out;
  double* g_out;
  int mode;
  int B;
  double L;
  vc_kin_mpc w;
  vc_qp qp;
  vc_obstacles obs;
  int detect;
  double detect_eps;
  double* farkas;
};

struct KinMeritArgs {
  const double* x0;
  const double* kappa;
  const double* ds;
  const double* u_prev;
  double* ubar;
  double* x_out;
  const double* x_prev;
  double* u0;
  const int32_t* qp_status;
  const int32_t* qp_iters;
  int32_t* status;
  int32_t* iters;
  int32_t* st_acc;
  int32_t* it_acc;
  double* ls_diag;
  int B, N;
  int first;
  int restart;
  int ms;
  double L;
  vc_kin_mpc w;
  vc_obstacles obs;
};

struct DynSqpArgs {
  const float* x0;
  const float* kappa;
  const float* ds;
  const float* ubar;
  float* u_out;
  float* x_out;
  float* u0;
  int32_t* status;
  int32_t* iters;
  float* diag;
  float* dbg;
  int B;
  DynCoef<float> car;
  vc_dyn_mpc w;
  vc_qp qp;
  vc_obstacles obs;
};

struct StSqpArgs {
  const double* x0;
  const double* kappa;
  const double* ds;
  const double* ubar;
  double* u_out;
  double* x_out;
  double* u0;
  int32_t* status;
  int32_t* iters;
  double* diag;
  double* jws;
  int B;
  DynCoef<double> car;
  vc_dyn_mpc w;
  vc_qp qp;
  vc_obstacles obs;
  int detect;
  double detect_eps;
  double* farkas;
  int32_t* qp_index;
  int reg_levels;
  double reg_factor;
  int32_t* level;
  int dbg_levels;
  int dbg_sqp_iter;
  int dbg_problem;
};

struct CascSqpArgs {
  const double* x0;
  const double* kappa;
  const double* ds;
  const double* ubar;
  double* u_out;
  double* x_out;
  double* u0;
  int32_t* status;
  int32_t* iters;
  double* diag;
  double* jws;
  double* H_out;
  double* g_out;
  int mode;
  int B;
  DynCoef<double> car;
  vc_dyn_mpc w;
  vc_casc_mpc cw;
  vc_qp qp;
  vc_obstacles obs;
  int detect;
  double detect_eps;
  double* farkas;
  int32_t* qp_index;
};

struct ModelArgs {
  int model;
  int B, N;
  int M;
  int shift;
  double L;
  DynCoef<double> dyn64;
  DynCoef<float> dyn32;
};
template <typename T>
__host__ __device__ inline const DynCoef<T>& dyn_coef(const ModelArgs& m);
template <>
__host__ __device__ inline const DynCoef<double>& dyn_coef<double>(const ModelArgs& m) { return m.dyn64; }
template <>
__host__ __device__ inline const DynCoef<float>& dyn_coef<float>(const ModelArgs& m) { return m.dyn32; }

struct TrackTable {
  const double* coef;
  int n;
  double h, length;
};

hipError_t launch_track_k(const TrackTable& tt, int dtype, int B, const void* s, void* k, hipStream_t st);
hipError_t launch_horizon(const TrackTable& tt, int model, int dtype, int B, int N, int M, double ds_pm,
                          const void* x0, bool x0_fp64, const void* xbar, double mpc_dt, void* kappa, void* ds,
                          void* x0_out, hipStream_t st);
hipError_t launch_drive(const ModelArgs& m, int dtype, const TrackTable& tt, double* x64, const void* u0, double dt,
                        void* x_ctx, const int32_t* status, void* xbar, void* ubar, int32_t* nfail, double* log_x,
                        void* log_u, const void* kappa, hipStream_t st);
hipError_t launch_kin_ltv(const KinLtvArgs& a, int N, hipStream_t stream);
hipError_t launch_kin_ltv_det(const KinLtvArgs& a, int N, hipStream_t stream);
hipError_t launch_kin_ric(const KinLtvArgs& a, int N, hipStream_t stream);
hipError_t launch_kin_merit(const KinMeritArgs& a, hipStream_t stream);
hipError_t launch_rcp_probe(int n, const double* x, double* out, hipStream_t st);
hipError_t launch_kin_gdots(int B, int N, const double* G, const double* vz, const double* vc, double* out_grow,
                            double* out_gt, hipStream_t stream);
hipError_t launch_kin_qp_fault(const KinLtvArgs& a, int N, int b, hipStream_t stream);
bool kin_ric_built(int N);
hipError_t launch_dyn_sqp(const DynSqpArgs& a, int N, hipStream_t stream);
hipError_t launch_casc_sqp(const CascSqpArgs& a, int N, int M, hipStream_t stream);
hipError_t launch_casc_ric(const CascSqpArgs& a, int N, int M, hipStream_t stream);
bool casc_ric_built(int N, int M);
size_t casc_ric_jws_doubles(int N, int M, int B);
hipError_t launch_st_sqp(const StSqpArgs& a, int N, hipStream_t stream);
hipError_t launch_st_sqp_reg(const StSqpArgs& a, int N, hipStream_t stream);
bool st_sqp_built(int N);
size_t st_sqp_jws_doubles(int N, int B);
bool casc_sqp_built(int N, int M);
size_t dyn_sqp_smem_bytes(int N);
int dyn_sqp_debug_stride();
size_t kin_ltv_smem_bytes(int N);
hipError_t launch_ode(const ModelArgs& m, int dtype, const void* x, const void* u, const void* kappa, int space,
                      void* f, hipStream_t st);
hipError_t launch_plant_step(const ModelArgs& m, int dtype, const void* x, const void* u, const void* kappa, double dt,
                             void* xn, hipStream_t st);
hipError_t launch_spatial_step(const ModelArgs& m, int dtype, const void* x, const void* u, const void* kappa,
                               const void* ds, void* xn, hipStream_t st);
hipError_t launch_rollout(const ModelArgs& m, int dtype, const void* x0, const void* ubar, const void* kappa,
                          const void* ds, void* xbar, hipStream_t st);
hipError_t launch_kin_linearize(const ModelArgs& m, const void* xbar, const void* ubar, const void* kappa,
                                const void* ds, void* A, void* Bm, hipStream_t st);

}
```

### vehicle-control_amd/csrc/vcmpc_abi.hip

```cpp
#include <hip/hip_runtime.h>

#include <cmath>
#include <cstdarg>
#include <cstdio>
#include <cstring>
#include <string>
#include <vector>

#include "vc_kernels.hpp"
#include "vcmpc.h"


struct Detect {
  bool on = false;
  double eps = 1e-9;
  void* farkas = nullptr;
  void* qp_index = nullptr;
  size_t rows = 0;
  int B = 0;
};

struct Regularize {
  int levels = 0;
  double factor = 10.0;
  void* level = nullptr;
  size_t level_bytes = 0;
  int B = 0, K = 0;
  int dbg_sqp_iter = -1, dbg_problem = -1, dbg_levels = 0;
};

struct vc_ctx {
  int device = 0, model = 0, N = 0, max_batch = 0, dtype = 0;
  vc_params p{};
  hipStream_t own = nullptr;
  hipStream_t stream = nullptr;
  void* arena = nullptr;
  size_t arena_bytes = 0;
  void* track = nullptr;
  int track_n = 0;
  double track_h = 0.0, track_len = 0.0;
  void* sim = nullptr;
  size_t sim_bytes = 0;
  void* ls = nullptr;
  size_t ls_bytes = 0;
  void* jw = nullptr;
  size_t jw_bytes = 0;
  int fault_iter = -1, fault_problem = -1;
  Detect det;
  Regularize reg;
  std::string err;
};

namespace {
thread_local std::string g_create_err;

int fail(vc_ctx* c, int code, const char* fmt, ...) {
  char buf[512];
  va_list ap;
  va_start(ap, fmt);
  vsnprintf(buf, sizeof(buf), fmt, ap);
  va_end(ap);
  if (c) c->err = buf;
  else g_create_err = buf;
  return code;
}

#define VC_HIP(ctx, call)                                                                         \
  do {                                                                                            \
    hipError_t e_ = (call);                                                                       \
    if (e_ != hipSuccess) return fail((ctx), VC_E_HIP, "%s: %s", #call, hipGetErrorString(e_)); \
  } while (0)

size_t esize(const vc_ctx* c) { return c->dtype == VC_F32 ? 4 : 8; }

int ensure_scratch(vc_ctx* c, void** p, size_t* have, size_t need) {
  if (need <= *have) return 0;
  VC_HIP(c, hipStreamSynchronize(c->stream));
  if (*p) VC_HIP(c, hipFree(*p));
  *p = nullptr;
  *have = 0;
  VC_HIP(c, hipMalloc(p, need));
  *have = need;
  return 0;
}
int nx_of(const vc_ctx* c) { return c->model == VC_MODEL_KINEMATIC ? 6 : 8; }

int ensure_arena(vc_ctx* c, size_t bytes) {
  if (bytes <= c->arena_bytes) return 0;
  VC_HIP(c, hipSetDevice(c->device));
  if (c->arena) VC_HIP(c, hipFree(c->arena));
  c->arena = nullptr;
  c->arena_bytes = 0;
  VC_HIP(c, hipMalloc(&c->arena, bytes));
  c->arena_bytes = bytes;
  return 0;
}

size_t al256(size_t b) { return (b + 255) & ~size_t(255); }

struct Ptr {
  void* p = nullptr;
  template <class T> operator T*() const { return static_cast<T*>(p); }
};

class Staging {
 public:
  Staging(vc_ctx* c, int flags) : c_(c), host_(flags == VC_HOST_PTRS) {}

  struct Pair {
    Ptr rd, wr;
  };
  Pair pair(const void* src, void* dst, size_t bytes) {
    if (!host_) return {{const_cast<void*>(src)}, {dst}};
    if (!src && !dst) return {};
    const size_t at = off_;
    off_ += al256(bytes);
    if (!placing_) return {};
    void* dev = static_cast<char*>(c_->arena) + at;
    if (src && bytes && err_ == hipSuccess) err_ = hipMemcpyAsync(dev, src, bytes, hipMemcpyHostToDevice, c_->stream);
    if (dst && bytes) outs_.push_back({dst, dev, bytes});
    return {{src ? dev : nullptr}, {dst ? dev : nullptr}};
  }
  Ptr in(const void* host, size_t bytes) { return pair(host, nullptr, bytes).rd; }
  Ptr out(void* host, size_t bytes) { return pair(nullptr, host, bytes).wr; }
  Ptr inout(void* host, size_t bytes) { return pair(host, host, bytes).wr; }

  template <class F>
  int bind(F&& declare) {
    declare();
    if (!host_) return 0;
    if (int r = ensure_arena(c_, off_ ? off_ : 256)) return r;
    off_ = 0;
    placing_ = true;
    declare();
    if (err_ != hipSuccess) return fail(c_, VC_E_HIP, "hipMemcpyAsync (H2D): %s", hipGetErrorString(err_));
    return 0;
  }

  int finish() {
    if (!host_) return 0;
    for (const Out& o : outs_) VC_HIP(c_, hipMemcpyAsync(o.host, o.dev, o.bytes, hipMemcpyDeviceToHost, c_->stream));
    VC_HIP(c_, hipStreamSynchronize(c_->stream));
    return 0;
  }

 private:
  struct Out {
    void* host;
    const void* dev;
    size_t bytes;
  };
  vc_ctx* c_;
  bool host_, placing_ = false;
  size_t off_ = 0;
  hipError_t err_ = hipSuccess;
  std::vector<Out> outs_;
};

int check_common(vc_ctx* c, int B, int flags) {
  if (!c) return VC_E_ARG;
  if (B < 0 || B > c->max_batch) return fail(c, VC_E_ARG, "batch %d outside [0, max_batch=%d]", B, c->max_batch);
  if (flags != VC_HOST_PTRS && flags != VC_DEVICE_PTRS) return fail(c, VC_E_ARG, "bad flags %d", flags);
  hipError_t e = hipSetDevice(c->device);
  if (e != hipSuccess) return fail(c, VC_E_HIP, "hipSetDevice: %s", hipGetErrorString(e));
  return 0;
}

vc::ModelArgs model_args(const vc_ctx* c, int B) {
  vc::ModelArgs m{};
  m.model = c->model;
  m.B = B;
  m.N = c->N;
  m.M = c->model == VC_MODEL_CASCADED ? c->p.casc.horizon_pm : 0;
  m.shift = c->p.qp.shift;
  m.L = c->p.kin_car.l;
  m.dyn64 = vc::make_dyn_coef<double>(c->p.dyn_car);
  m.dyn32 = vc::make_dyn_coef<float>(c->p.dyn_car);
  return m;
}

int nh_of(const vc_ctx* c) { return c->N + (c->model == VC_MODEL_CASCADED ? c->p.casc.horizon_pm : 0); }
int ns_of(const vc_ctx* c) { return c->model == VC_MODEL_KINEMATIC ? c->N + 1 : nh_of(c); }
vc::TrackTable track_table(const vc_ctx* c) {
  return vc::TrackTable{static_cast<const double*>(c->track), c->track_n, c->track_h, c->track_len};
}

bool kin_condensed_cfg(const vc_ctx* c) {
  return vc::kin_ltv_smem_bytes(c->N) > 0 && (c->p.qp.solver == 0 || c->p.qp.solver == 2) && c->p.qp.kin_sqp <= 0 &&
         !c->p.qp.ms && c->p.qp.elastic == 0.0;
}
bool kin_condensed(const vc_ctx* c) { return kin_condensed_cfg(c) && (!c->det.on || c->p.qp.solver == 2); }
bool kin_solve_built(const vc_ctx* c) {
  return c->model == VC_MODEL_KINEMATIC && c->dtype == VC_F64 && (kin_condensed(c) || vc::kin_ric_built(c->N));
}
bool dyn_solve_built(const vc_ctx* c) {
  if (c->model != VC_MODEL_DYNAMIC) return false;
  if (c->dtype == VC_F32) return vc::dyn_sqp_smem_bytes(c->N) > 0;
  return vc::st_sqp_built(c->N);
}
bool casc_stagewise(const vc_ctx* c) {
  return c->p.qp.solver != 2 && vc::casc_ric_built(c->N, c->p.casc.horizon_pm);
}
bool casc_solve_built(const vc_ctx* c) {
  return c->model == VC_MODEL_CASCADED && c->dtype == VC_F64 &&
         (casc_stagewise(c) || vc::casc_sqp_built(c->N, c->p.casc.horizon_pm));
}

int set_detection(vc_ctx* c, int on, double eps, size_t rows, bool with_index) {
  Detect& d = c->det;
  if (on && !d.farkas) {
    VC_HIP(c, hipSetDevice(c->device));
    const size_t nb = (size_t)(c->max_batch > 0 ? c->max_batch : 1);
    VC_HIP(c, hipMalloc(&d.farkas, nb * rows * 8));
    if (with_index) VC_HIP(c, hipMalloc(&d.qp_index, nb * 4));
  }
  d.on = on != 0;
  d.eps = eps > 0.0 ? eps : 1e-9;
  d.rows = rows;
  d.B = 0;
  return 0;
}

int get_detection(vc_ctx* c, const char* who, int model, int B, void* y, int32_t* qp_index, bool with_index,
                  int flags) {
  if (int r = check_common(c, B, flags)) return r;
  const Detect& d = c->det;
  if (c->model != model || !d.on || !d.farkas || (with_index && !d.qp_index))
    return fail(c, VC_E_ARG, "%s: infeasibility detection is off", who);
  if (model == VC_MODEL_KINEMATIC && c->p.qp.kin_sqp > 0)
    return fail(c, VC_E_UNSUPPORTED, "%s: kin_sqp > 0 solves several QPs per call", who);
  if (B > d.B) return fail(c, VC_E_ARG, "%s: B=%d exceeds the last solve's %d", who, B, d.B);
  if (!y) return fail(c, VC_E_ARG, "null pointer");
  if (B == 0) return 0;
  const hipMemcpyKind kind = flags == VC_DEVICE_PTRS ? hipMemcpyDeviceToDevice : hipMemcpyDeviceToHost;
  VC_HIP(c, hipMemcpyAsync(y, d.farkas, (size_t)B * d.rows * 8, kind, c->stream));
  if (qp_index) VC_HIP(c, hipMemcpyAsync(qp_index, d.qp_index, (size_t)B * 4, kind, c->stream));
  if (flags != VC_DEVICE_PTRS) VC_HIP(c, hipStreamSynchronize(c->stream));
  return 0;
}

template <class Args>
bool arm_detection(vc_ctx* c, Args& a, int B) {
  if (!c->det.on) return false;
  a.detect = 1;
  a.detect_eps = c->det.eps;
  a.farkas = (double*)c->det.farkas;
  c->det.B = B;
  return true;
}

int arm_regularization(vc_ctx* c, vc::StSqpArgs& a, int B) {
  Regularize& r = c->reg;
  if (r.levels > 0) {
    const int K = c->p.dyn_mpc.sqp_iters;
    if (int e = ensure_scratch(c, &r.level, &r.level_bytes, (size_t)B * K * 4)) return e;
    a.reg_levels = r.levels;
    a.reg_factor = r.factor;
    a.level = (int32_t*)r.level;
    r.B = B;
    r.K = K;
  }
  if (r.dbg_sqp_iter >= 0 && r.dbg_levels > 0) {
    a.dbg_levels = r.dbg_levels;
    a.dbg_sqp_iter = r.dbg_sqp_iter;
    a.dbg_problem = r.dbg_problem;
  }
  return 0;
}

int casc_solve(vc_ctx* c, int B, const void* x0, const void* kappa, const void* ds, void* xbar, void* ubar, void* u0,
               int32_t* status, int32_t* iters, void* diag, int flags, int mode = 0, void* H_out = nullptr,
               void* g_out = nullptr) {
  const int Hs = c->N + c->p.casc.horizon_pm, n = 2 * Hs, nx = 8, nu = 2;
  const vc_dyn_mpc& w = c->p.dyn_mpc;
  if (w.sqp_iters < 1 || w.sqp_iters > 64) return fail(c, VC_E_ARG, "dyn_mpc.sqp_iters=%d outside [1,64]", w.sqp_iters);
  if (!(w.fx_scale > 0)) return fail(c, VC_E_ARG, "dyn_mpc.fx_scale must be > 0");
  if (c->p.qp.max_iter < 1) return fail(c, VC_E_ARG, "qp.max_iter must be >= 1");
  if (!(c->p.casc.ds_pm > 0)) return fail(c, VC_E_ARG, "casc.ds_pm must be > 0");
  vc::CascSqpArgs a{};
  a.B = B;
  a.mode = mode;
  a.car = vc::make_dyn_coef<double>(c->p.dyn_car);
  a.w = w;
  a.cw = c->p.casc;
  a.qp = c->p.qp;
  a.obs = c->p.obs;
  Staging st(c, flags);
  if (int r = st.bind([&] {
        a.x0 = st.in(x0, (size_t)B * nx * 8);
        a.kappa = st.in(kappa, (size_t)B * Hs * 8);
        a.ds = st.in(ds, (size_t)B * Hs * 8);
        const Staging::Pair u = st.pair(ubar, mode == 0 ? ubar : nullptr, (size_t)B * Hs * nu * 8);
        a.ubar = u.rd;
        a.u_out = u.wr;
        if (mode == 0) {
          a.x_out = st.out(xbar, (size_t)B * Hs * nx * 8);
          a.u0 = st.out(u0, (size_t)B * nu * 8);
          a.status = st.out(status, (size_t)B * 4);
          a.iters = st.out(iters, (size_t)B * 4);
          a.diag = st.out(diag, (size_t)B * VC_CASC_DIAG_COLS * 8);
        } else {
          a.H_out = st.out(H_out, (size_t)B * n * n * 8);
          a.g_out = st.out(g_out, (size_t)B * n * 8);
        }
      }))
    return r;
  if (mode == 0 && casc_stagewise(c)) {
    if (const size_t jd = vc::casc_ric_jws_doubles(c->N, c->p.casc.horizon_pm, B)) {
      if (int r = ensure_scratch(c, &c->jw, &c->jw_bytes, (size_t)B * jd * 8)) return r;
      a.jws = (double*)c->jw;
    }
    if (arm_detection(c, a, B)) a.qp_index = (int32_t*)c->det.qp_index;
    VC_HIP(c, vc::launch_casc_ric(a, c->N, c->p.casc.horizon_pm, c->stream));
  }
  else VC_HIP(c, vc::launch_casc_sqp(a, c->N, c->p.casc.horizon_pm, c->stream));
  return st.finish();
}

int st_solve(vc_ctx* c, int B, const void* x0, const void* kappa, const void* ds, void* xbar, void* ubar, void* u0,
             int32_t* status, int32_t* iters, void* diag, int flags) {
  const int N = c->N, nx = 8, nu = 2;
  const vc_dyn_mpc& w = c->p.dyn_mpc;
  vc::StSqpArgs a{};
  a.B = B;
  a.car = vc::make_dyn_coef<double>(c->p.dyn_car);
  a.w = w;
  a.qp = c->p.qp;
  a.obs = c->p.obs;
  Staging st(c, flags);
  if (int r = st.bind([&] {
        a.x0 = st.in(x0, (size_t)B * nx * 8);
        a.kappa = st.in(kappa, (size_t)B * N * 8);
        a.ds = st.in(ds, (size_t)B * N * 8);
        a.ubar = a.u_out = st.inout(ubar, (size_t)B * N * nu * 8);
        a.x_out = st.out(xbar, (size_t)B * N * nx * 8);
        a.u0 = st.out(u0, (size_t)B * nu * 8);
        a.status = st.out(status, (size_t)B * 4);
        a.iters = st.out(iters, (size_t)B * 4);
        a.diag = st.out(diag, (size_t)B * VC_ST_DIAG_COLS * 8);
      }))
    return r;
  if (const size_t jd = vc::st_sqp_jws_doubles(N, B)) {
    if (int r = ensure_scratch(c, &c->jw, &c->jw_bytes, (size_t)B * jd * 8)) return r;
    a.jws = (double*)c->jw;
  }
  if (arm_detection(c, a, B)) a.qp_index = (int32_t*)c->det.qp_index;
  if (int r = arm_regularization(c, a, B)) return r;
  VC_HIP(c, vc::launch_st_sqp(a, N, c->stream));
  return st.finish();
}

int dyn_solve(vc_ctx* c, int B, const void* x0, const void* kappa, const void* ds, void* xbar, void* ubar, void* u0,
              int32_t* status, int32_t* iters, void* diag, int flags, void* dbg = nullptr) {
  const int N = c->N, nx = 8, nu = 2;
  const vc_dyn_mpc& w = c->p.dyn_mpc;
  if (w.sqp_iters < 1 || w.sqp_iters > 64) return fail(c, VC_E_ARG, "dyn_mpc.sqp_iters=%d outside [1,64]", w.sqp_iters);
  if (!(w.fx_scale > 0)) return fail(c, VC_E_ARG, "dyn_mpc.fx_scale must be > 0");
  if (c->p.qp.max_iter < 1) return fail(c, VC_E_ARG, "qp.max_iter must be >= 1");
  if (c->dtype == VC_F64) return st_solve(c, B, x0, kappa, ds, xbar, ubar, u0, status, iters, diag, flags);
  vc::DynSqpArgs a{};
  a.B = B;
  a.car = vc::make_dyn_coef<float>(c->p.dyn_car);
  a.w = w;
  a.qp = c->p.qp;
  a.obs = c->p.obs;
  Staging st(c, flags);
  if (int r = st.bind([&] {
        a.x0 = st.in(x0, (size_t)B * nx * 4);
        a.kappa = st.in(kappa, (size_t)B * N * 4);
        a.ds = st.in(ds, (size_t)B * N * 4);
        a.ubar = a.u_out = st.inout(ubar, (size_t)B * N * nu * 4);
        a.x_out = st.out(xbar, (size_t)B * N * nx * 4);
        a.u0 = st.out(u0, (size_t)B * nu * 4);
        a.status = st.out(status, (size_t)B * 4);
        a.iters = st.out(iters, (size_t)B * 4);
        a.diag = st.out(diag, (size_t)B * VC_DYN_DIAG_COLS * 4);
        a.dbg = st.out(dbg, (size_t)B * vc::dyn_sqp_debug_stride() * 4);
      }))
    return r;
  VC_HIP(c, vc::launch_dyn_sqp(a, N, c->stream));
  return st.finish();
}
}

extern "C" {

int vc_abi_version(void) { return VCMPC_ABI_VERSION; }
int vc_params_sizeof(void) { return (int)sizeof(vc_params); }

static const char* obstacles_invalid(const vc_obstacles& o) {
  static thread_local char msg[96];
  if (o.n < 0 || o.n > VC_MAX_OBSTACLES) {
    snprintf(msg, sizeof msg, "n=%d obstacles outside [0,%d]", o.n, VC_MAX_OBSTACLES);
    return msg;
  }
  for (int j = 0; j < o.n; ++j)
    if (!std::isfinite(o.s[j]) || !std::isfinite(o.ey[j]) || !std::isfinite(o.radius[j])) {
      snprintf(msg, sizeof msg, "obstacle %d is not finite", j);
      return msg;
    }
  return nullptr;
}

vc_ctx* vc_create(int device, int model, int N, int max_batch, int dtype, const vc_params* params) {
  g_create_err.clear();
  if (!params) { fail(nullptr, VC_E_ARG, "params is NULL"); return nullptr; }
  if (model != VC_MODEL_KINEMATIC && model != VC_MODEL_DYNAMIC && model != VC_MODEL_CASCADED) {
    fail(nullptr, VC_E_ARG, "bad model %d", model);
    return nullptr;
  }
  if (model == VC_MODEL_CASCADED && (params->casc.horizon_pm < 1 || params->casc.horizon_pm > 4096)) {
    fail(nullptr, VC_E_ARG, "cascaded context needs casc.horizon_pm >= 1 (got %d)", params->casc.horizon_pm);
    return nullptr;
  }
  if (dtype != VC_F64 && dtype != VC_F32) { fail(nullptr, VC_E_ARG, "bad dtype %d", dtype); return nullptr; }
  if (N < 1 || N > 4096) { fail(nullptr, VC_E_ARG, "bad horizon N=%d", N); return nullptr; }
  if (max_batch < 1) { fail(nullptr, VC_E_ARG, "bad max_batch %d", max_batch); return nullptr; }
  if (params->obs.inside != 0 && params->obs.inside != 1) {
    fail(nullptr, VC_E_ARG, "obs.inside=%d must be 0 or 1", params->obs.inside);
    return nullptr;
  }
  if (model == VC_MODEL_KINEMATIC && params->obs.inside) {
    fail(nullptr, VC_E_ARG, "obs.inside=1 is not supported by the kinematic model (dynamic / cascaded only)");
    return nullptr;
  }
  int ndev = 0;
  hipError_t e = hipGetDeviceCount(&ndev);
  if (e != hipSuccess || ndev == 0) {
    fail(nullptr, VC_E_HIP, "no HIP device available (%s)", hipGetErrorString(e));
    return nullptr;
  }
  if (device < 0 || device >= ndev) { fail(nullptr, VC_E_ARG, "device %d not in [0,%d)", device, ndev); return nullptr; }
  e = hipSetDevice(device);
  if (e != hipSuccess) { fail(nullptr, VC_E_HIP, "hipSetDevice: %s", hipGetErrorString(e)); return nullptr; }
  if (const char* why = obstacles_invalid(params->obs)) {
    fail(nullptr, VC_E_ARG, "params->obs: %s", why);
    return nullptr;
  }
  vc_ctx* c = new vc_ctx();
  c->device = device;
  c->model = model;
  c->N = N;
  c->max_batch = max_batch;
  c->dtype = dtype;
  c->p = *params;
  if (!(c->p.obs.margin_min > 0)) c->p.obs.margin_min = VC_OBS_MARGIN_MIN;
  e = hipStreamCreateWithFlags(&c->own, hipStreamNonBlocking);
  if (e != hipSuccess) {
    fail(nullptr, VC_E_HIP, "hipStreamCreate: %s", hipGetErrorString(e));
    delete c;
    return nullptr;
  }
  c->stream = c->own;
  return c;
}

void vc_destroy(vc_ctx* c) {
  if (!c) return;
  (void)hipSetDevice(c->device);
  if (c->stream) (void)hipStreamSynchronize(c->stream);
  if (c->arena) (void)hipFree(c->arena);
  if (c->track) (void)hipFree(c->track);
  if (c->sim) (void)hipFree(c->sim);
  if (c->ls) (void)hipFree(c->ls);
  if (c->jw) (void)hipFree(c->jw);
  if (c->det.farkas) (void)hipFree(c->det.farkas);
  if (c->det.qp_index) (void)hipFree(c->det.qp_index);
  if (c->reg.level) (void)hipFree(c->reg.level);
  if (c->own) (void)hipStreamDestroy(c->own);
  delete c;
}

const char* vc_last_error(const vc_ctx* c) { return c ? c->err.c_str() : g_create_err.c_str(); }

int vc_set_stream(vc_ctx* c, void* stream) {
  if (!c) return VC_E_ARG;
  c->stream = stream ? static_cast<hipStream_t>(stream) : c->own;
  return 0;
}

int vc_set_obstacles(vc_ctx* c, int n, const double* s, const double* ey, const double* radius, double margin_min) {
  if (!c) return VC_E_ARG;
  if (n < 0 || n > VC_MAX_OBSTACLES) return fail(c, VC_E_ARG, "n=%d obstacles outside [0,%d]", n, VC_MAX_OBSTACLES);
  if (n > 0 && (!s || !ey || !radius)) return fail(c, VC_E_ARG, "null pointer");
  vc_obstacles o{};
  o.n = n;
  o.inside = c->p.obs.inside;
  o.margin_min = margin_min > 0 ? margin_min : c->p.obs.margin_min;
  for (int j = 0; j < n; ++j) {
    o.s[j] = s[j];
    o.ey[j] = ey[j];
    o.radius[j] = radius[j];
  }
  if (const char* why = obstacles_invalid(o)) return fail(c, VC_E_ARG, "%s", why);
  c->p.obs = o;
  return 0;
}

int vc_synchronize(vc_ctx* c) {
  if (!c) return VC_E_ARG;
  VC_HIP(c, hipSetDevice(c->device));
  VC_HIP(c, hipStreamSynchronize(c->stream));
  return 0;
}

int vc_set_infeasibility(vc_ctx* c, int on, double eps) {
  if (!c) return VC_E_ARG;
  if (c->model != VC_MODEL_KINEMATIC || c->dtype != VC_F64 || !vc::kin_ric_built(c->N))
    return fail(c, VC_E_UNSUPPORTED,
                "vc_set_infeasibility: the stagewise kinematic kernel only (kinematic fp64, N=10..60 step 10); "
                "model=%d dtype=%d N=%d", c->model, c->dtype, c->N);
  return set_detection(c, on, eps, (size_t)(7 * c->N - 3), false);
}

int vc_get_farkas(vc_ctx* c, int B, void* y, int flags) {
  return get_detection(c, "vc_get_farkas", VC_MODEL_KINEMATIC, B, y, nullptr, false, flags);
}

int vc_set_sqp_infeasibility(vc_ctx* c, int on, double eps) {
  if (!c) return VC_E_ARG;
  if (c->model != VC_MODEL_DYNAMIC || c->dtype != VC_F64 || !vc::st_sqp_built(c->N))
    return fail(c, VC_E_UNSUPPORTED,
                "vc_set_sqp_infeasibility: the single-track fp64 SQP kernel only (dynamic fp64, N=20..60 step 10); "
                "model=%d dtype=%d N=%d", c->model, c->dtype, c->N);
  if (!(c->p.dyn_mpc.trust_Fx > 0))
    return fail(c, VC_E_ARG, "vc_set_sqp_infeasibility: dyn_mpc.trust_Fx must be > 0 (it bounds |dz|_1)");
  return set_detection(c, on, eps, (size_t)(12 * c->N - 3), true);
}

int vc_get_sqp_farkas(vc_ctx* c, int B, void* y, int32_t* qp_index, int flags) {
  return get_detection(c, "vc_get_sqp_farkas", VC_MODEL_DYNAMIC, B, y, qp_index, true, flags);
}

int vc_set_sqp_regularization(vc_ctx* c, int levels, double factor) {
  if (!c) return VC_E_ARG;
  if (c->model != VC_MODEL_DYNAMIC || c->dtype != VC_F64 || !vc::st_sqp_built(c->N))
    return fail(c, VC_E_UNSUPPORTED,
                "vc_set_sqp_regularization: the single-track fp64 SQP kernel only (dynamic fp64, N=20..60 step 10); "
                "model=%d dtype=%d N=%d", c->model, c->dtype, c->N);
  if (levels < 0 || levels > 6) return fail(c, VC_E_ARG, "vc_set_sqp_regularization: levels=%d outside [0,6]", levels);
  const double f = factor <= 0.0 ? 10.0 : factor;
  if (!(f > 1.0)) return fail(c, VC_E_ARG, "vc_set_sqp_regularization: factor=%g must be > 1 (<= 0 keeps 10)", factor);
  c->reg.levels = levels;
  c->reg.factor = f;
  c->reg.B = 0;
  return 0;
}

int vc_get_sqp_regularization(vc_ctx* c, int B, int32_t* level, int flags) {
  if (int r = check_common(c, B, flags)) return r;
  const Regularize& g = c->reg;
  if (g.levels <= 0) return fail(c, VC_E_ARG, "vc_get_sqp_regularization: the regularised retry is off");
  if (B > g.B) return fail(c, VC_E_ARG, "vc_get_sqp_regularization: B=%d exceeds the last solve's %d", B, g.B);
  if (!level) return fail(c, VC_E_ARG, "null pointer");
  if (B == 0) return 0;
  const hipMemcpyKind kind = flags == VC_DEVICE_PTRS ? hipMemcpyDeviceToDevice : hipMemcpyDeviceToHost;
  VC_HIP(c, hipMemcpyAsync(level, g.level, (size_t)B * g.K * 4, kind, c->stream));
  if (flags != VC_DEVICE_PTRS) VC_HIP(c, hipStreamSynchronize(c->stream));
  return 0;
}

int vc_debug_sqp_breakdown(vc_ctx* c, int sqp_iter, int problem, int levels) {
  if (!c) return VC_E_ARG;
  c->reg.dbg_sqp_iter = sqp_iter;
  c->reg.dbg_problem = problem;
  c->reg.dbg_levels = levels;
  return 0;
}

int vc_set_casc_infeasibility(vc_ctx* c, int on, double eps) {
  if (!c) return VC_E_ARG;
  if (c->model != VC_MODEL_CASCADED || c->dtype != VC_F64 || !vc::casc_ric_built(c->N, c->p.casc.horizon_pm))
    return fail(c, VC_E_UNSUPPORTED,
                "vc_set_casc_infeasibility: the stagewise cascaded fp64 SQP kernel only (cascaded fp64, N=20, "
                "horizon_pm=15/25/35/40); model=%d dtype=%d N=%d horizon_pm=%d", c->model, c->dtype, c->N,
                c->p.casc.horizon_pm);
  if (c->p.qp.solver == 2)
    return fail(c, VC_E_UNSUPPORTED,
                "vc_set_casc_infeasibility: qp.solver=2 asks for the condensed kernel, which has no detection");
  if (!(c->p.dyn_mpc.trust_Fx > 0))
    return fail(c, VC_E_ARG, "vc_set_casc_infeasibility: dyn_mpc.trust_Fx must be > 0 (it bounds |dz|_1)");
  return set_detection(c, on, eps, (size_t)(12 * c->N - 3 + 6 * c->p.casc.horizon_pm), true);
}

int vc_get_casc_farkas(vc_ctx* c, int B, void* y, int32_t* qp_index, int flags) {
  return get_detection(c, "vc_get_casc_farkas", VC_MODEL_CASCADED, B, y, qp_index, true, flags);
}

static int kin_solve(vc_ctx* c, int B, const void* x0, const void* kappa, const void* ds, void* xbar,
                     const void* ubar_in, void* u_out, void* u0, int32_t* status, int32_t* iters, void* diag,
                     int flags);

int vc_solve(vc_ctx* c, int B, const void* x0, const void* kappa, const void* ds, void* xbar, void* ubar, void* u0,
             int32_t* status, int32_t* iters, int flags) {
  return vc_solve_diag(c, B, x0, kappa, ds, xbar, ubar, u0, status, iters, nullptr, flags);
}

int vc_solve_from(vc_ctx* c, int B, const void* x0, const void* kappa, const void* ds, const void* ubar_in,
                  void* xbar, void* u_out, void* u0, int32_t* status, int32_t* iters, int flags) {
  if (int r = check_common(c, B, flags)) return r;
  if (!ubar_in || !u_out) return fail(c, VC_E_ARG, "null pointer");
  if (ubar_in == u_out) return vc_solve(c, B, x0, kappa, ds, xbar, u_out, u0, status, iters, flags);
  if (c->model == VC_MODEL_KINEMATIC && kin_solve_built(c)) {
    if (!x0 || !kappa || !ds || !xbar || !u0 || !status || !iters) return fail(c, VC_E_ARG, "null pointer");
    if (B == 0) return 0;
    return kin_solve(c, B, x0, kappa, ds, xbar, ubar_in, u_out, u0, status, iters, nullptr, flags);
  }
  const int H = c->N + (c->model == VC_MODEL_CASCADED ? c->p.casc.horizon_pm : 0);
  const size_t bytes = (size_t)B * H * 2 * (c->dtype == VC_F32 ? 4 : 8);
  if (flags == VC_HOST_PTRS) std::memcpy(u_out, ubar_in, bytes);
  else VC_HIP(c, hipMemcpyAsync(u_out, ubar_in, bytes, hipMemcpyDeviceToDevice, c->stream));
  return vc_solve(c, B, x0, kappa, ds, xbar, u_out, u0, status, iters, flags);
}

int vc_solve_diag(vc_ctx* c, int B, const void* x0, const void* kappa, const void* ds, void* xbar, void* ubar,
                  void* u0, int32_t* status, int32_t* iters, void* diag, int flags) {
  if (int r = check_common(c, B, flags)) return r;
  if (!kin_solve_built(c) && !dyn_solve_built(c) && !casc_solve_built(c))
    return fail(c, VC_E_UNSUPPORTED,
                "vc_solve: model=%d dtype=%d N=%d not built (kinematic fp64 N=10..60 step 10, dynamic fp64 "
                "N=20..60 step 10, dynamic fp32 N=40, cascaded fp64 N=20 + 40 are)", c->model, c->dtype, c->N);
  if (!x0 || !kappa || !ds || !xbar || !ubar || !u0 || !status || !iters) return fail(c, VC_E_ARG, "null pointer");
  if (B == 0) return 0;
  if (c->model == VC_MODEL_DYNAMIC) return dyn_solve(c, B, x0, kappa, ds, xbar, ubar, u0, status, iters, diag, flags);
  if (c->model == VC_MODEL_CASCADED) return casc_solve(c, B, x0, kappa, ds, xbar, ubar, u0, status, iters, diag, flags);
  return kin_solve(c, B, x0, kappa, ds, xbar, ubar, ubar, u0, status, iters, diag, flags);
}

static int kin_solve(vc_ctx* c, int B, const void* x0, const void* kappa, const void* ds, void* xbar,
                     const void* ubar_in, void* u_out, void* u0, int32_t* status, int32_t* iters, void* diag,
                     int flags) {
  if (c->p.qp.elastic < 0.0 && c->p.qp.kin_sqp <= 0)
    return fail(c, VC_E_ARG, "vc_qp.elastic < 0 (elastic on failure) needs kin_sqp > 0; rho > 0 for one QP step");
  const int N = c->N, nx = 6, nu = 2;
  vc::KinLtvArgs a{};
  a.mode = 0;
  a.B = B;
  a.L = c->p.kin_car.l;
  a.w = c->p.kin_mpc;
  a.qp = c->p.qp;
  a.obs = c->p.obs;
  const size_t u_bytes = (size_t)B * N * nu * 8, x_bytes = (size_t)B * (N + 1) * nx * 8;
  Staging st(c, flags);
  if (int r = st.bind([&] {
        a.x0 = st.in(x0, (size_t)B * nx * 8);
        a.kappa = st.in(kappa, (size_t)B * N * 8);
        a.ds = st.in(ds, (size_t)B * N * 8);
        const Staging::Pair u = st.pair(ubar_in, u_out, u_bytes);
        a.ubar = u.rd;
        a.u_out = u.wr;
        a.x_in = a.x_out = st.pair(c->p.qp.ms ? xbar : nullptr, xbar, x_bytes).wr;
        a.u0 = st.out(u0, (size_t)B * nu * 8);
        a.status = st.out(status, (size_t)B * 4);
        a.iters = st.out(iters, (size_t)B * 4);
        a.diag = st.out(diag, (size_t)B * VC_DIAG_COLS * 8);
      }))
    return r;
  arm_detection(c, a, B);
  const int S = c->p.qp.kin_sqp;
  if (S > 0 && (const void*)a.ubar != (const void*)a.u_out) {
    VC_HIP(c, hipMemcpyAsync(a.u_out, a.ubar, u_bytes, hipMemcpyDeviceToDevice, c->stream));
    a.ubar = a.u_out;
  }
  if (S <= 0) {
    if (kin_condensed(c)) VC_HIP(c, vc::launch_kin_ltv(a, N, c->stream));
    else VC_HIP(c, vc::launch_kin_ric(a, N, c->stream));
  } else {
    const size_t o_up = 0, o_st = al256(u_bytes), o_it = o_st + al256((size_t)B * 4),
                 o_xp = o_it + al256((size_t)B * 4), total = o_xp + al256(x_bytes);
    if (int r = ensure_scratch(c, &c->ls, &c->ls_bytes, total)) return r;
    char* base = static_cast<char*>(c->ls);
    vc::KinMeritArgs m{};
    m.x0 = a.x0;
    m.kappa = a.kappa;
    m.ds = a.ds;
    m.u_prev = (const double*)(base + o_up);
    m.ubar = a.u_out;
    m.x_out = a.x_out;
    m.u0 = a.u0;
    m.qp_status = a.status;
    m.qp_iters = a.iters;
    m.status = a.status;
    m.iters = a.iters;
    m.st_acc = (int32_t*)(base + o_st);
    m.it_acc = (int32_t*)(base + o_it);
    m.ls_diag = nullptr;
    m.ms = c->p.qp.ms;
    m.restart = S > 1;
    m.x_prev = (const double*)(base + o_xp);
    m.B = B;
    m.N = N;
    m.L = a.L;
    m.w = a.w;
    m.obs = a.obs;
    const bool elastic_retry = c->p.qp.elastic < 0.0 && !kin_condensed(c);
    if (c->p.qp.elastic < 0.0) a.qp.elastic = 0.0;
    for (int i = 0; i < S; ++i) {
      VC_HIP(c, hipMemcpyAsync(base + o_up, a.u_out, u_bytes, hipMemcpyDeviceToDevice, c->stream));
      if (m.ms) VC_HIP(c, hipMemcpyAsync(base + o_xp, a.x_out, x_bytes, hipMemcpyDeviceToDevice, c->stream));
      if (kin_condensed(c)) VC_HIP(c, vc::launch_kin_ltv(a, N, c->stream));
      else VC_HIP(c, vc::launch_kin_ric(a, N, c->stream));
      if (elastic_retry) {
        vc::KinLtvArgs e = a;
        e.qp.elastic = c->p.qp.elastic;
        e.ubar = (const double*)(base + o_up);
        if (m.ms) e.x_in = (const double*)(base + o_xp);
        VC_HIP(c, vc::launch_kin_ric(e, N, c->stream));
      }
      if (i == c->fault_iter && c->fault_problem >= 0 && c->fault_problem < B)
        VC_HIP(c, vc::launch_kin_qp_fault(a, N, c->fault_problem, c->stream));
      m.first = i == 0;
      VC_HIP(c, vc::launch_kin_merit(m, c->stream));
    }
  }
  return st.finish();
}

int vc_solve_debug(vc_ctx* c, int B, const void* x0, const void* kappa, const void* ds, void* xbar, void* ubar,
                   void* u0, int32_t* status, int32_t* iters, void* dbg, int flags) {
  if (int r = check_common(c, B, flags)) return r;
  if (!dyn_solve_built(c)) return fail(c, VC_E_UNSUPPORTED, "vc_solve_debug: dynamic fp32 N=40 contexts only");
  if (!x0 || !kappa || !ds || !xbar || !ubar || !u0 || !status || !iters || !dbg)
    return fail(c, VC_E_ARG, "null pointer");
  if (B == 0) return 0;
  return dyn_solve(c, B, x0, kappa, ds, xbar, ubar, u0, status, iters, nullptr, flags, dbg);
}

int vc_debug_stride(void) { return vc::dyn_sqp_debug_stride(); }

int vc_debug_rcp(vc_ctx* c, int n, const void* x, void* out, int flags) {
  if (!c) return VC_E_ARG;
  if (n < 0 || n > c->max_batch) return fail(c, VC_E_ARG, "n %d outside [0, max_batch=%d]", n, c->max_batch);
  if (int r = check_common(c, 0, flags)) return r;
  if (!x || !out) return fail(c, VC_E_ARG, "null pointer");
  if (n == 0) return 0;
  Ptr dx, dout;
  Staging st(c, flags);
  if (int r = st.bind([&] {
        dx = st.in(x, (size_t)n * 8);
        dout = st.out(out, (size_t)n * 32);
      }))
    return r;
  VC_HIP(c, vc::launch_rcp_probe(n, dx, dout, c->stream));
  return st.finish();
}

int vc_debug_kin_gdots(vc_ctx* c, int B, const void* G, const void* vz, const void* vc, void* out_grow,
                       void* out_gt, int flags) {
  if (int r = check_common(c, B, flags)) return r;
  if (c->model != VC_MODEL_KINEMATIC || c->dtype != VC_F64 || vc::kin_ltv_smem_bytes(c->N) == 0)
    return fail(c, VC_E_UNSUPPORTED, "vc_debug_kin_gdots: kinematic fp64 contexts with the fused kernel's N only");
  if (!G || !vz || !vc || !out_grow || !out_gt) return fail(c, VC_E_ARG, "null pointer");
  if (B == 0) return 0;
  const int N = c->N, n = 2 * N, NC = 2 * (N - 1);
  Ptr dG, dvz, dvc, dgrow, dgt;
  Staging st(c, flags);
  if (int r = st.bind([&] {
        dG = st.in(G, (size_t)B * NC * n * 8);
        dvz = st.in(vz, (size_t)B * n * 8);
        dvc = st.in(vc, (size_t)B * NC * 8);
        dgrow = st.out(out_grow, (size_t)B * 64 * 8);
        dgt = st.out(out_gt, (size_t)B * 64 * 8);
      }))
    return r;
  VC_HIP(c, vc::launch_kin_gdots(B, N, dG, dvz, dvc, dgrow, dgt, c->stream));
  return st.finish();
}

int vc_debug_qp_fault(vc_ctx* c, int sqp_iter, int problem) {
  if (!c) return VC_E_ARG;
  c->fault_iter = sqp_iter;
  c->fault_problem = problem;
  return 0;
}

int vc_debug_kin_merit(vc_ctx* c, int B, const void* x0, const void* kappa, const void* ds, const void* u_prev,
                       void* u, const void* x_prev, void* x, int32_t* status, int32_t* iters, int32_t* st_acc,
                       int32_t* it_acc, int first, int restart, void* u0, void* ls_diag, int flags) {
  if (int r = check_common(c, B, flags)) return r;
  if (c->model != VC_MODEL_KINEMATIC || c->dtype != VC_F64)
    return fail(c, VC_E_UNSUPPORTED, "vc_debug_kin_merit: kinematic fp64 contexts only; model=%d dtype=%d", c->model,
                c->dtype);
  const bool ms = c->p.qp.ms != 0;
  if (!x0 || !kappa || !ds || !u_prev || !u || !x || !status || !iters || !st_acc || !it_acc || !u0 || !ls_diag ||
      (ms && !x_prev))
    return fail(c, VC_E_ARG, "null pointer");
  if (B == 0) return 0;
  const int N = c->N, nx = 6, nu = 2;
  const size_t u_bytes = (size_t)B * N * nu * 8, x_bytes = (size_t)B * (N + 1) * nx * 8;
  vc::KinMeritArgs m{};
  m.B = B;
  m.N = N;
  m.first = first != 0;
  m.restart = restart != 0;
  m.ms = ms;
  m.L = c->p.kin_car.l;
  m.w = c->p.kin_mpc;
  m.obs = c->p.obs;
  Staging st(c, flags);
  if (int r = st.bind([&] {
        m.x0 = st.in(x0, (size_t)B * nx * 8);
        m.kappa = st.in(kappa, (size_t)B * N * 8);
        m.ds = st.in(ds, (size_t)B * N * 8);
        m.u_prev = st.in(u_prev, u_bytes);
        m.ubar = st.inout(u, u_bytes);
        m.x_out = st.pair(ms ? x : nullptr, x, x_bytes).wr;
        m.x_prev = ms ? (const double*)st.in(x_prev, x_bytes) : (const double*)m.x_out;
        m.qp_status = m.status = st.inout(status, (size_t)B * 4);
        m.qp_iters = m.iters = st.inout(iters, (size_t)B * 4);
        m.st_acc = st.inout(st_acc, (size_t)B * 4);
        m.it_acc = st.inout(it_acc, (size_t)B * 4);
        m.u0 = st.out(u0, (size_t)B * nu * 8);
        m.ls_diag = st.out(ls_diag, (size_t)B * 4 * 8);
      }))
    return r;
  VC_HIP(c, vc::launch_kin_merit(m, c->stream));
  return st.finish();
}

int vc_condense(vc_ctx* c, int B, const void* x0, const void* ubar, const void* kappa, const void* ds, void* H,
                void* g, int flags) {
  if (int r = check_common(c, B, flags)) return r;
  const bool casc_cond = c->model == VC_MODEL_CASCADED && c->dtype == VC_F64 &&
                         vc::casc_sqp_built(c->N, c->p.casc.horizon_pm);
  if (!(kin_solve_built(c) && kin_condensed_cfg(c)) && !casc_cond)
    return fail(c, VC_E_UNSUPPORTED, "vc_condense: model=%d dtype=%d N=%d not built", c->model, c->dtype, c->N);
  if (!x0 || !kappa || !ds || !ubar || !H || !g) return fail(c, VC_E_ARG, "null pointer");
  if (B == 0) return 0;
  if (c->model == VC_MODEL_CASCADED)
    return casc_solve(c, B, x0, kappa, ds, nullptr, const_cast<void*>(ubar), nullptr, nullptr, nullptr, nullptr, flags,
                      1, H, g);
  const int N = c->N, n = 2 * N;
  vc::KinLtvArgs a{};
  a.mode = 1;
  a.B = B;
  a.L = c->p.kin_car.l;
  a.w = c->p.kin_mpc;
  a.qp = c->p.qp;
  a.obs = c->p.obs;
  Staging st(c, flags);
  if (int r = st.bind([&] {
        a.x0 = st.in(x0, (size_t)B * 6 * 8);
        a.kappa = st.in(kappa, (size_t)B * N * 8);
        a.ds = st.in(ds, (size_t)B * N * 8);
        a.ubar = st.in(ubar, (size_t)B * n * 8);
        a.H_out = st.out(H, (size_t)B * n * n * 8);
        a.g_out = st.out(g, (size_t)B * n * 8);
      }))
    return r;
  VC_HIP(c, vc::launch_kin_ltv(a, N, c->stream));
  return st.finish();
}

int vc_rollout(vc_ctx* c, int B, const void* x0, const void* ubar, const void* kappa, const void* ds, void* xbar,
               int flags) {
  if (int r = check_common(c, B, flags)) return r;
  if (!x0 || !ubar || !kappa || !ds || !xbar) return fail(c, VC_E_ARG, "null pointer");
  if (B == 0) return 0;
  const int N = c->N, nx = nx_of(c);
  const size_t es = esize(c);
  vc::ModelArgs m = model_args(c, B);
  Ptr dx0, dubar, dkappa, dds, dxbar;
  Staging st(c, flags);
  if (int r = st.bind([&] {
        dx0 = st.in(x0, (size_t)B * nx * es);
        dubar = st.in(ubar, (size_t)B * N * 2 * es);
        dkappa = st.in(kappa, (size_t)B * N * es);
        dds = st.in(ds, (size_t)B * N * es);
        dxbar = st.out(xbar, (size_t)B * (N + 1) * nx * es);
      }))
    return r;
  VC_HIP(c, vc::launch_rollout(m, c->dtype, dx0, dubar, dkappa, dds, dxbar, c->stream));
  return st.finish();
}

int vc_linearize(vc_ctx* c, int B, const void* xbar, const void* ubar, const void* kappa, const void* ds, void* A,
                 void* Bm, int flags) {
  if (int r = check_common(c, B, flags)) return r;
  if (c->model != VC_MODEL_KINEMATIC || c->dtype != VC_F64)
    return fail(c, VC_E_UNSUPPORTED, "vc_linearize: only the kinematic fp64 model is built");
  if (!xbar || !ubar || !kappa || !ds || !A || !Bm) return fail(c, VC_E_ARG, "null pointer");
  if (B == 0) return 0;
  const int N = c->N;
  vc::ModelArgs m = model_args(c, B);
  Ptr dxbar, dubar, dkappa, dds, dA, dBm;
  Staging st(c, flags);
  if (int r = st.bind([&] {
        dxbar = st.in(xbar, (size_t)B * (N + 1) * 6 * 8);
        dubar = st.in(ubar, (size_t)B * N * 2 * 8);
        dkappa = st.in(kappa, (size_t)B * N * 8);
        dds = st.in(ds, (size_t)B * N * 8);
        dA = st.out(A, (size_t)B * N * 36 * 8);
        dBm = st.out(Bm, (size_t)B * N * 12 * 8);
      }))
    return r;
  VC_HIP(c, vc::launch_kin_linearize(m, dxbar, dubar, dkappa, dds, dA, dBm, c->stream));
  return st.finish();
}

int vc_plant_step(vc_ctx* c, int B, const void* x, const void* u, const void* kappa, double dt, void* x_next,
                  int flags) {
  if (int r = check_common(c, B, flags)) return r;
  if (!x || !u || !kappa || !x_next) return fail(c, VC_E_ARG, "null pointer");
  if (B == 0) return 0;
  const int nx = nx_of(c);
  const size_t es = esize(c);
  vc::ModelArgs m = model_args(c, B);
  Ptr dx, du, dkappa, dnext;
  Staging st(c, flags);
  if (int r = st.bind([&] {
        dx = st.in(x, (size_t)B * nx * es);
        du = st.in(u, (size_t)B * 2 * es);
        dkappa = st.in(kappa, (size_t)B * es);
        dnext = st.out(x_next, (size_t)B * nx * es);
      }))
    return r;
  VC_HIP(c, vc::launch_plant_step(m, c->dtype, dx, du, dkappa, dt, dnext, c->stream));
  return st.finish();
}

int vc_ode(vc_ctx* c, int B, const void* x, const void* u, const void* kappa, int space, void* f, int flags) {
  if (int r = check_common(c, B, flags)) return r;
  if (!x || !u || !kappa || !f) return fail(c, VC_E_ARG, "null pointer");
  if (space != 0 && space != 1) return fail(c, VC_E_ARG, "vc_ode: space must be 0 (temporal) or 1 (spatial)");
  if (B == 0) return 0;
  const int nx = nx_of(c);
  const size_t es = esize(c);
  vc::ModelArgs m = model_args(c, B);
  Ptr dx, du, dkappa, df;
  Staging st(c, flags);
  if (int r = st.bind([&] {
        dx = st.in(x, (size_t)B * nx * es);
        du = st.in(u, (size_t)B * 2 * es);
        dkappa = st.in(kappa, (size_t)B * es);
        df = st.out(f, (size_t)B * nx * es);
      }))
    return r;
  VC_HIP(c, vc::launch_ode(m, c->dtype, dx, du, dkappa, space, df, c->stream));
  return st.finish();
}

int vc_spatial_step(vc_ctx* c, int B, const void* x, const void* u, const void* kappa, const void* ds, void* x_next,
                    int flags) {
  if (int r = check_common(c, B, flags)) return r;
  if (!x || !u || !kappa || !ds || !x_next) return fail(c, VC_E_ARG, "null pointer");
  if (B == 0) return 0;
  const int nx = nx_of(c);
  const size_t es = esize(c);
  vc::ModelArgs m = model_args(c, B);
  Ptr dx, du, dkappa, dds, dnext;
  Staging st(c, flags);
  if (int r = st.bind([&] {
        dx = st.in(x, (size_t)B * nx * es);
        du = st.in(u, (size_t)B * 2 * es);
        dkappa = st.in(kappa, (size_t)B * es);
        dds = st.in(ds, (size_t)B * es);
        dnext = st.out(x_next, (size_t)B * nx * es);
      }))
    return r;
  VC_HIP(c, vc::launch_spatial_step(m, c->dtype, dx, du, dkappa, dds, dnext, c->stream));
  return st.finish();
}

int vc_track_set(vc_ctx* c, int n_pieces, double h, double length, const double* coef) {
  if (!c) return VC_E_ARG;
  if (n_pieces < 1 || !(h > 0) || !(length > 0) || !coef)
    return fail(c, VC_E_ARG, "vc_track_set: need n_pieces >= 1, h > 0, length > 0, coef");
  for (int i = 0; i < 4 * n_pieces; ++i)
    if (!std::isfinite(coef[i])) return fail(c, VC_E_ARG, "vc_track_set: coef[%d] not finite", i);
  VC_HIP(c, hipSetDevice(c->device));
  VC_HIP(c, hipStreamSynchronize(c->stream));
  if (c->track) VC_HIP(c, hipFree(c->track));
  c->track = nullptr;
  c->track_n = 0;
  VC_HIP(c, hipMalloc(&c->track, (size_t)n_pieces * 4 * sizeof(double)));
  VC_HIP(c, hipMemcpy(c->track, coef, (size_t)n_pieces * 4 * sizeof(double), hipMemcpyHostToDevice));
  c->track_n = n_pieces;
  c->track_h = h;
  c->track_len = length;
  return 0;
}

int vc_track_k(vc_ctx* c, int B, const void* s, void* k, int flags) {
  if (int r = check_common(c, B, flags)) return r;
  if (!s || !k) return fail(c, VC_E_ARG, "null pointer");
  if (!c->track) return fail(c, VC_E_ARG, "vc_track_k: no track table (vc_track_set)");
  if (B == 0) return 0;
  const size_t es = esize(c);
  Ptr dpos, dk;
  Staging st(c, flags);
  if (int r = st.bind([&] {
        dpos = st.in(s, B * es);
        dk = st.out(k, B * es);
      }))
    return r;
  VC_HIP(c, vc::launch_track_k(track_table(c), c->dtype, B, dpos, dk, c->stream));
  return st.finish();
}

int vc_horizon(vc_ctx* c, int B, const void* x0, const void* xbar, double mpc_dt, void* kappa, void* ds,
               int flags) {
  if (int r = check_common(c, B, flags)) return r;
  if (!x0 || !xbar || !kappa || !ds) return fail(c, VC_E_ARG, "null pointer");
  if (!c->track) return fail(c, VC_E_ARG, "vc_horizon: no track table (vc_track_set)");
  if (B == 0) return 0;
  const int N = c->N, nx = nx_of(c), NS = ns_of(c), NH = nh_of(c), M = NH - N;
  const double ds_pm = c->p.casc.ds_pm;
  const size_t es = esize(c);
  Ptr dx0, dxbar, dkappa, dds;
  Staging st(c, flags);
  if (int r = st.bind([&] {
        dx0 = st.in(x0, (size_t)B * nx * es);
        dxbar = st.in(xbar, (size_t)B * NS * nx * es);
        dkappa = st.out(kappa, (size_t)B * NH * es);
        dds = st.out(ds, (size_t)B * NH * es);
      }))
    return r;
  VC_HIP(c, vc::launch_horizon(track_table(c), c->model, c->dtype, B, N, M, ds_pm, dx0, c->dtype == VC_F64, dxbar,
                               mpc_dt, dkappa, dds, nullptr, c->stream));
  return st.finish();
}

int vc_drive(vc_ctx* c, int B, double* x64, const void* u0, double dt, void* x_ctx, int flags) {
  if (int r = check_common(c, B, flags)) return r;
  if (!x64 || !u0) return fail(c, VC_E_ARG, "null pointer");
  if (!c->track) return fail(c, VC_E_ARG, "vc_drive: no track table (vc_track_set)");
  if (B == 0) return 0;
  const int nx = nx_of(c);
  const size_t es = esize(c);
  vc::ModelArgs m = model_args(c, B);
  Ptr dx, du0, dctx;
  Staging st(c, flags);
  if (int r = st.bind([&] {
        dx = st.inout(x64, (size_t)B * nx * 8);
        du0 = st.in(u0, (size_t)B * 2 * es);
        dctx = st.out(x_ctx, (size_t)B * nx * es);
      }))
    return r;
  VC_HIP(c, vc::launch_drive(m, c->dtype, track_table(c), dx, du0, dt, dctx, nullptr, nullptr, nullptr, nullptr,
                             nullptr, nullptr, nullptr, c->stream));
  return st.finish();
}

int vc_simulate(vc_ctx* c, int B, int steps, double mpc_dt, double dt, double* x64, void* xbar, void* ubar,
                double* log_x, void* log_u, int32_t* nfail, int flags) {
  if (int r = check_common(c, B, flags)) return r;
  if (!x64 || !xbar || !ubar) return fail(c, VC_E_ARG, "null pointer");
  if (steps < 0) return fail(c, VC_E_ARG, "steps %d < 0", steps);
  if (!c->track) return fail(c, VC_E_ARG, "vc_simulate: no track table (vc_track_set)");
  if (!kin_solve_built(c) && !dyn_solve_built(c) && !casc_solve_built(c))
    return fail(c, VC_E_UNSUPPORTED, "vc_simulate: model=%d dtype=%d N=%d has no built vc_solve", c->model, c->dtype,
                c->N);
  if (B == 0 || steps == 0) return 0;
  const int N = c->N, nx = nx_of(c), NS = ns_of(c), NH = nh_of(c), M = NH - N;
  const double ds_pm = c->p.casc.ds_pm;
  const size_t es = esize(c), x_bytes = (size_t)B * nx * 8;
  double *dx, *dlx;
  void *dxbar, *dubar, *dlu;
  int32_t* dnf;
  Staging st(c, flags);
  if (int r = st.bind([&] {
        dx = st.inout(x64, x_bytes);
        dxbar = st.inout(xbar, (size_t)B * NS * nx * es);
        dubar = st.inout(ubar, (size_t)B * NH * 2 * es);
        dlx = st.out(log_x, (size_t)(steps + 1) * B * nx * 8);
        dlu = st.out(log_u, (size_t)steps * B * 2 * es);
        dnf = st.inout(nfail, (size_t)B * 4);
      }))
    return r;
  const size_t o_kap = 0, o_ds = o_kap + al256((size_t)B * NH * es), o_x = o_ds + al256((size_t)B * NH * es),
               o_u0 = o_x + al256((size_t)B * nx * es), o_st = o_u0 + al256((size_t)B * 2 * es),
               o_it = o_st + al256((size_t)B * 4), total = o_it + al256((size_t)B * 4);
  if (int r = ensure_scratch(c, &c->sim, &c->sim_bytes, total)) return r;
  char* base = static_cast<char*>(c->sim);
  void *kap = base + o_kap, *dsv = base + o_ds, *xc = base + o_x, *u0 = base + o_u0;
  int32_t *stat = (int32_t*)(base + o_st), *it = (int32_t*)(base + o_it);
  const vc::TrackTable tt = track_table(c);
  vc::ModelArgs m = model_args(c, B);
  if (dlx) VC_HIP(c, hipMemcpyAsync(dlx, dx, x_bytes, hipMemcpyDeviceToDevice, c->stream));
  for (int step = 0; step < steps; ++step) {
    VC_HIP(c, vc::launch_horizon(tt, c->model, c->dtype, B, N, M, ds_pm, dx, true, dxbar, mpc_dt, kap, dsv, xc,
                                 c->stream));
    if (int r = vc_solve_diag(c, B, xc, kap, dsv, dxbar, dubar, u0, stat, it, nullptr, VC_DEVICE_PTRS)) return r;
    VC_HIP(c, vc::launch_drive(m, c->dtype, tt, dx, u0, dt, nullptr, stat, dxbar, dubar, dnf,
                               dlx ? dlx + (size_t)(step + 1) * B * nx : nullptr,
                               dlu ? (char*)dlu + (size_t)step * B * 2 * es : nullptr, kap, c->stream));
  }
  return st.finish();
}

}
```

### vehicle-control_amd/vcmpc/_abi.py

```python
from __future__ import annotations

import ctypes as C
import os

LIB_NAME = "libvcmpc.so"
LIB_PATH = os.environ.get("VCMPC_LIB", os.path.join(os.path.dirname(os.path.abspath(__file__)), LIB_NAME))
ABI_VERSION = 13
VC_MAX_OBSTACLES = 16
OBS_MARGIN_MIN = 0.05

VC_MODEL_KINEMATIC, VC_MODEL_DYNAMIC, VC_MODEL_CASCADED = 0, 1, 2
VC_F64, VC_F32 = 0, 1
VC_HOST_PTRS, VC_DEVICE_PTRS = 0, 1
VC_TYRE_FIALA, VC_TYRE_LINEAR = 0, 1
VC_SOLVED, VC_MAX_ITER, VC_NONFINITE, VC_OUT_OF_DOMAIN, VC_INFEASIBLE = 0, 1, 2, 3, 4
VC_OK, VC_E_ARG, VC_E_HIP, VC_E_UNSUPPORTED = 0, -1, -2, -3

STATUS_NAMES = {VC_SOLVED: "solved", VC_MAX_ITER: "max_iter", VC_NONFINITE: "nonfinite",
                VC_OUT_OF_DOMAIN: "out_of_domain", VC_INFEASIBLE: "infeasible"}


class vc_kin_car(C.Structure):
    _fields_ = [("l", C.c_double)]


class vc_dyn_car(C.Structure):
    _fields_ = [(k, C.c_double) for k in (
        "l", "m", "Izz", "a", "b", "h", "eps", "Peng",
        "Xdf", "Xdr", "Xbf", "Xbr", "Caf", "Car",
        "Cd", "muf", "mur", "theta", "phi", "Av2", "Frr")] + [("tyre", C.c_int32), ("pad_", C.c_int32)]


class vc_kin_mpc(C.Structure):
    _fields_ = [(k, C.c_double) for k in (
        "w_time", "w_ey", "w_epsi", "w_v", "w_w", "w_a", "w_dev", "w_b",
        "a_min", "a_max", "w_min", "w_max",
        "v_min", "v_max", "delta_min", "delta_max", "ey_min", "ey_max", "w_obs")]


class vc_dyn_mpc(C.Structure):
    _fields_ = [(k, C.c_double) for k in (
        "w_time", "w_speed", "w_ey", "w_epsi", "w_w", "w_Fx", "w_dev", "w_b", "w_slip",
        "w_min", "w_max", "Ux_min", "max_speed", "delta_min", "delta_max", "ey_min", "ey_max",
        "fx_scale", "trust_Fx")] + [("sqp_iters", C.c_int32), ("pad_", C.c_int32), ("w_obs", C.c_double)]


class vc_qp(C.Structure):
    _fields_ = [("prox", C.c_double), ("tol", C.c_double), ("trust_a", C.c_double), ("trust_w", C.c_double),
                ("max_iter", C.c_int32), ("polish", C.c_int32), ("solver", C.c_int32), ("kin_sqp", C.c_int32),
                ("shift", C.c_int32), ("ms", C.c_int32), ("elastic", C.c_double)]


class vc_obstacles(C.Structure):
    _fields_ = [("n", C.c_int32), ("inside", C.c_int32), ("margin_min", C.c_double),
                ("s", C.c_double * VC_MAX_OBSTACLES), ("ey", C.c_double * VC_MAX_OBSTACLES),
                ("radius", C.c_double * VC_MAX_OBSTACLES)]


class vc_casc_mpc(C.Structure):
    _fields_ = [("horizon_pm", C.c_int32), ("pad_", C.c_int32)] + [(k, C.c_double) for k in (
        "ds_pm", "w_dev_pm", "w_Fy", "w_switch", "V_min", "ey_min_pm", "ey_max_pm")]


class vc_params(C.Structure):
    _fields_ = [("kin_car", vc_kin_car), ("dyn_car", vc_dyn_car), ("kin_mpc", vc_kin_mpc), ("qp", vc_qp),
                ("dyn_mpc", vc_dyn_mpc), ("obs", vc_obstacles), ("casc", vc_casc_mpc)]


class VcError(RuntimeError):

    def __init__(self, code: int, msg: str):
        super().__init__(f"vcmpc error {code}: {msg}")
        self.code = code


_vp = C.c_void_p
_i32p = C.POINTER(C.c_int32)

PROTOTYPES = {
    "vc_abi_version": (C.c_int, []),
    "vc_params_sizeof": (C.c_int, []),
    "vc_create": (_vp, [C.c_int, C.c_int, C.c_int, C.c_int, C.c_int, C.POINTER(vc_params)]),
    "vc_destroy": (None, [_vp]),
    "vc_last_error": (C.c_char_p, [_vp]),
    "vc_set_stream": (C.c_int, [_vp, _vp]),
    "vc_synchronize": (C.c_int, [_vp]),
    "vc_set_obstacles": (C.c_int, [_vp, C.c_int, _vp, _vp, _vp, C.c_double]),
    "vc_set_infeasibility": (C.c_int, [_vp, C.c_int, C.c_double]),
    "vc_get_farkas": (C.c_int, [_vp, C.c_int, _vp, C.c_int]),
    "vc_set_sqp_infeasibility": (C.c_int, [_vp, C.c_int, C.c_double]),
    "vc_get_sqp_farkas": (C.c_int, [_vp, C.c_int, _vp, _vp, C.c_int]),
    "vc_set_sqp_regularization": (C.c_int, [_vp, C.c_int, C.c_double]),
    "vc_get_sqp_regularization": (C.c_int, [_vp, C.c_int, _vp, C.c_int]),
    "vc_debug_sqp_breakdown": (C.c_int, [_vp, C.c_int, C.c_int, C.c_int]),
    "vc_set_casc_infeasibility": (C.c_int, [_vp, C.c_int, C.c_double]),
    "vc_get_casc_farkas": (C.c_int, [_vp, C.c_int, _vp, _vp, C.c_int]),
    "vc_solve": (C.c_int, [_vp, C.c_int, _vp, _vp, _vp, _vp, _vp, _vp, _vp, _vp, C.c_int]),
    "vc_solve_diag": (C.c_int, [_vp, C.c_int, _vp, _vp, _vp, _vp, _vp, _vp, _vp, _vp, _vp, C.c_int]),
    "vc_solve_from": (C.c_int, [_vp, C.c_int, _vp, _vp, _vp, _vp, _vp, _vp, _vp, _vp, _vp, C.c_int]),
    "vc_solve_debug": (C.c_int, [_vp, C.c_int, _vp, _vp, _vp, _vp, _vp, _vp, _vp, _vp, _vp, C.c_int]),
    "vc_debug_stride": (C.c_int, []),
    "vc_debug_qp_fault": (C.c_int, [_vp, C.c_int, C.c_int]),
    "vc_debug_kin_merit": (C.c_int, [_vp, C.c_int] + [_vp] * 11 + [C.c_int, C.c_int, _vp, _vp, C.c_int]),
    "vc_debug_rcp": (C.c_int, [_vp, C.c_int, _vp, _vp, C.c_int]),
    "vc_debug_kin_gdots": (C.c_int, [_vp, C.c_int, _vp, _vp, _vp, _vp, _vp, C.c_int]),
    "vc_rollout": (C.c_int, [_vp, C.c_int, _vp, _vp, _vp, _vp, _vp, C.c_int]),
    "vc_linearize": (C.c_int, [_vp, C.c_int, _vp, _vp, _vp, _vp, _vp, _vp, C.c_int]),
    "vc_condense": (C.c_int, [_vp, C.c_int, _vp, _vp, _vp, _vp, _vp, _vp, C.c_int]),
    "vc_plant_step": (C.c_int, [_vp, C.c_int, _vp, _vp, _vp, C.c_double, _vp, C.c_int]),
    "vc_spatial_step": (C.c_int, [_vp, C.c_int, _vp, _vp, _vp, _vp, _vp, C.c_int]),
    "vc_ode": (C.c_int, [_vp, C.c_int, _vp, _vp, _vp, C.c_int, _vp, C.c_int]),
    "vc_track_set": (C.c_int, [_vp, C.c_int, C.c_double, C.c_double, _vp]),
    "vc_track_k": (C.c_int, [_vp, C.c_int, _vp, _vp, C.c_int]),
    "vc_horizon": (C.c_int, [_vp, C.c_int, _vp, _vp, C.c_double, _vp, _vp, C.c_int]),
    "vc_drive": (C.c_int, [_vp, C.c_int, _vp, _vp, C.c_double, _vp, C.c_int]),
    "vc_simulate": (C.c_int, [_vp, C.c_int, C.c_int, C.c_double, C.c_double, _vp, _vp, _vp, _vp, _vp, _vp, C.c_int]),
}

_LIB = None


def load_library(path: str | None = None) -> C.CDLL:
    global _LIB
    if _LIB is not None and path is None:
        return _LIB
    p = path or LIB_PATH
    try:
        import torch
    except ImportError:
        pass
    if not os.path.exists(p):
        raise ImportError(
            f"{p} not found: build it with `make -C vehicle-control_amd/csrc` "
            "(or __graft_entry__.build()); vcmpc has no CPU fallback")
    lib = C.CDLL(p)
    for name, (res, args) in PROTOTYPES.items():
        fn = getattr(lib, name)
        fn.restype = res
        fn.argtypes = args
    if lib.vc_abi_version() != ABI_VERSION:
        raise ImportError(f"{p}: ABI version {lib.vc_abi_version()} != {ABI_VERSION}")
    if lib.vc_params_sizeof() != C.sizeof(vc_params):
        raise ImportError(f"{p}: sizeof(vc_params) {lib.vc_params_sizeof()} != ctypes {C.sizeof(vc_params)}")
    if path is None:
        _LIB = lib
    return lib


def check(lib, ctx, code: int) -> None:
    if code != VC_OK:
        msg = lib.vc_last_error(ctx)
        raise VcError(code, msg.decode() if msg else "")
```

### vehicle-control_amd/vcmpc/solver.py

```python
from __future__ import annotations

import ctypes as C

import numpy as np

from . import _abi
from .config import make_params

NX = {_abi.VC_MODEL_KINEMATIC: 6, _abi.VC_MODEL_DYNAMIC: 8, _abi.VC_MODEL_CASCADED: 8}
NU = 2
_NP_DT = {_abi.VC_F64: np.float64, _abi.VC_F32: np.float32}


def _is_torch(a) -> bool:
    return type(a).__module__.startswith("torch")


class Context:

    def __init__(self, model: int = _abi.VC_MODEL_KINEMATIC, N: int = 20, max_batch: int = 1024,
                 dtype: int = _abi.VC_F64, device: int = 0, params: _abi.vc_params | None = None,
                 detect_infeasible: bool = False, infeasible_eps: float = 0.0,
                 regularize_levels: int = 0, regularize_factor: float = 0.0, **cfgs):
        self.lib = _abi.load_library()
        self.model, self.N, self.max_batch, self.dtype, self.device = model, int(N), int(max_batch), dtype, device
        self.nx = NX[model]
        self.params = params if params is not None else make_params(**cfgs)
        self.NH = self.N + (int(self.params.casc.horizon_pm) if model == _abi.VC_MODEL_CASCADED else 0)
        self.ns_solve = self.N + 1 if model == _abi.VC_MODEL_KINEMATIC else self.NH
        h = self.lib.vc_create(device, model, self.N, self.max_batch, dtype, C.byref(self.params))
        if not h:
            raise _abi.VcError(_abi.VC_E_HIP, self.lib.vc_last_error(None).decode())
        self._h = C.c_void_p(h)
        self.detect_infeasible = False
        self._last = None
        self.regularize_levels = 0
        if regularize_levels:
            try:
                self.set_sqp_regularization(regularize_levels, regularize_factor)
            except Exception:
                self.close()
                raise
        if detect_infeasible:
            try:
                if model == _abi.VC_MODEL_DYNAMIC and dtype == _abi.VC_F64:
                    self.set_sqp_infeasibility(True, infeasible_eps)
                elif model == _abi.VC_MODEL_CASCADED and dtype == _abi.VC_F64:
                    self.set_casc_infeasibility(True, infeasible_eps)
                else:
                    self.set_infeasibility(True, infeasible_eps)
            except Exception:
                self.close()
                raise

    def close(self):
        if getattr(self, "_h", None):
            self.lib.vc_destroy(self._h)
            self._h = None

    def __del__(self):
        try:
            self.close()
        except Exception:
            pass

    def __enter__(self):
        return self

    def __exit__(self, *exc):
        self.close()

    def _check(self, code):
        _abi.check(self.lib, self._h, code)

    def set_stream(self, stream_handle: int | None):
        self._check(self.lib.vc_set_stream(self._h, C.c_void_p(stream_handle or 0)))

    def set_obstacles(self, obstacles, margin_min: float = 0.0):
        rows = np.asarray([tuple(r) for r in (obstacles or [])], np.float64).reshape(-1, 3)
        cols = [np.ascontiguousarray(rows[:, i]) for i in range(3)]
        self._check(self.lib.vc_set_obstacles(self._h, len(rows), *[C.c_void_p(c.ctypes.data) for c in cols],
                                              float(margin_min)))

    def set_infeasibility(self, on: bool, eps: float = 0.0):
        self._set_detection(self.lib.vc_set_infeasibility, on, eps)

    def farkas(self, B: int | None = None):
        return self._certificates(self.lib.vc_get_farkas, B, 7 * self.N - 3, False)[0]

    def set_sqp_infeasibility(self, on: bool, eps: float = 0.0):
        self._set_detection(self.lib.vc_set_sqp_infeasibility, on, eps)

    def sqp_farkas(self, B: int | None = None):
        return self._certificates(self.lib.vc_get_sqp_farkas, B, 12 * self.N - 3, True)

    def set_sqp_regularization(self, levels: int, factor: float = 0.0):
        self._check(self.lib.vc_set_sqp_regularization(self._h, int(levels), float(factor)))
        self.regularize_levels = int(levels)
        self._last = None

    def sqp_regularization(self, B: int | None = None):
        last_B, dev = self._last if self._last is not None else (0, None)
        B = last_B if B is None else int(B)
        K = int(self.params.dyn_mpc.sqp_iters)
        if dev is not None:
            import torch
            out = torch.empty((B, K), dtype=torch.int32, device=dev)
            ptr, flags = C.c_void_p(out.data_ptr()), _abi.VC_DEVICE_PTRS
        else:
            out = np.empty((B, K), np.int32)
            ptr, flags = C.c_void_p(out.ctypes.data), _abi.VC_HOST_PTRS
        self._check(self.lib.vc_get_sqp_regularization(self._h, B, ptr, flags))
        return out

    def debug_sqp_breakdown(self, sqp_iter: int, problem: int = 0, levels: int = 1):
        self._check(self.lib.vc_debug_sqp_breakdown(self._h, int(sqp_iter), int(problem), int(levels)))

    def set_casc_infeasibility(self, on: bool, eps: float = 0.0):
        self._set_detection(self.lib.vc_set_casc_infeasibility, on, eps)

    def casc_farkas(self, B: int | None = None):
        return self._certificates(self.lib.vc_get_casc_farkas, B, 12 * self.N - 3 + 6 * (self.NH - self.N), True)

    def _set_detection(self, fn, on, eps):
        self._check(fn(self._h, int(bool(on)), float(eps)))
        self.detect_infeasible = bool(on)
        self._last = None

    def _certificates(self, fn, B, rows, with_index):
        last_B, dev = self._last if self._last is not None else (0, None)
        B = last_B if B is None else int(B)
        if dev is not None:
            import torch
            out = (torch.empty((B, rows), dtype=torch.float64, device=dev),
                   torch.empty((B,), dtype=torch.int32, device=dev))[:1 + with_index]
            ptrs, flags = [C.c_void_p(a.data_ptr()) for a in out], _abi.VC_DEVICE_PTRS
        else:
            out = (np.empty((B, rows), np.float64), np.empty((B,), np.int32))[:1 + with_index]
            ptrs, flags = [C.c_void_p(a.ctypes.data) for a in out], _abi.VC_HOST_PTRS
        self._check(fn(self._h, B, *ptrs, flags))
        return out

    def synchronize(self):
        self._check(self.lib.vc_synchronize(self._h))

    def _marshal(self, arrays, shapes, dtypes):
        dev = [_is_torch(a) for a in arrays]
        if any(dev) and not all(dev):
            raise TypeError("mix of host and device buffers in one call")
        ptrs = []
        for a, shp, dt in zip(arrays, shapes, dtypes):
            if dev[0]:
                import torch
                tdt = {np.float64: torch.float64, np.float32: torch.float32, np.int32: torch.int32}[dt]
                if a.dtype != tdt or not a.is_contiguous() or tuple(a.shape) != tuple(shp):
                    raise ValueError(f"device buffer must be contiguous {tdt}{tuple(shp)}, got {a.dtype}{tuple(a.shape)}")
                if not a.is_cuda or a.device.index != self.device:
                    raise ValueError(f"device buffer must live on cuda:{self.device}")
                ptrs.append(C.c_void_p(a.data_ptr()))
            else:
                if not isinstance(a, np.ndarray) or a.dtype != dt or not a.flags.c_contiguous or a.shape != tuple(shp):
                    got = f"{getattr(a, 'dtype', type(a))}{getattr(a, 'shape', '')}"
                    raise ValueError(f"host buffer must be C-contiguous {np.dtype(dt)}{tuple(shp)}, got {got}")
                ptrs.append(C.c_void_p(a.ctypes.data))
        return ptrs, (_abi.VC_DEVICE_PTRS if dev[0] else _abi.VC_HOST_PTRS)

    def _batch(self, x):
        B = int(x.shape[0])
        if B > self.max_batch:
            raise ValueError(f"batch {B} > max_batch {self.max_batch}")
        return B

    def solve(self, x0, kappa, ds, ubar, xbar=None, u0=None, status=None, iters=None, diag=None):
        B, N, nx, f = self._batch(x0), self.NH, self.nx, _NP_DT[self.dtype]
        NS = self.ns_solve
        xbar, u0, status, iters = self._solve_outputs(x0, B, xbar, u0, status, iters)
        bufs = [x0, kappa, ds, xbar, ubar, u0, status, iters]
        shapes = [(B, nx), (B, N), (B, N), (B, NS, nx), (B, N, NU), (B, NU), (B,), (B,)]
        dts = [f, f, f, f, f, f, np.int32, np.int32]
        self._last = (B, x0.device if _is_torch(x0) else None)
        if diag is not None and diag is not False:
            if diag is True:
                diag = self._like(x0, (B, 4))
            ptrs, flags = self._marshal(bufs + [diag], shapes + [(B, int(diag.shape[1]))], dts + [f])
            self._check(self.lib.vc_solve_diag(self._h, B, *ptrs, flags))
            return u0, xbar, ubar, status, iters, diag
        ptrs, flags = self._marshal(bufs, shapes, dts)
        self._check(self.lib.vc_solve(self._h, B, *ptrs, flags))
        return u0, xbar, ubar, status, iters

    def _solve_outputs(self, x0, B, xbar, u0, status, iters):
        NS, nx, f = self.ns_solve, self.nx, _NP_DT[self.dtype]
        if xbar is None and self.model == _abi.VC_MODEL_KINEMATIC and self.params.qp.ms:
            raise ValueError("vc_qp.ms: multiple shooting linearises at the state iterate; pass xbar")
        if _is_torch(x0):
            import torch
            kw = dict(device=x0.device)
            xbar = torch.empty((B, NS, nx), dtype=x0.dtype, **kw) if xbar is None else xbar
            u0 = torch.empty((B, NU), dtype=x0.dtype, **kw) if u0 is None else u0
            status = torch.empty((B,), dtype=torch.int32, **kw) if status is None else status
            iters = torch.empty((B,), dtype=torch.int32, **kw) if iters is None else iters
        else:
            xbar = np.empty((B, NS, nx), f) if xbar is None else xbar
            u0 = np.empty((B, NU), f) if u0 is None else u0
            status = np.empty((B,), np.int32) if status is None else status
            iters = np.empty((B,), np.int32) if iters is None else iters
        return xbar, u0, status, iters

    def solve_from(self, x0, kappa, ds, ubar_in, u_out, xbar=None, u0=None, status=None, iters=None):
        B, N, nx, f = self._batch(x0), self.NH, self.nx, _NP_DT[self.dtype]
        NS = self.ns_solve
        xbar, u0, status, iters = self._solve_outputs(x0, B, xbar, u0, status, iters)
        bufs = [x0, kappa, ds, ubar_in, xbar, u_out, u0, status, iters]
        self._last = (B, x0.device if _is_torch(x0) else None)
        shapes = [(B, nx), (B, N), (B, N), (B, N, NU), (B, NS, nx), (B, N, NU), (B, NU), (B,), (B,)]
        dts = [f, f, f, f, f, f, f, np.int32, np.int32]
        ptrs, flags = self._marshal(bufs, shapes, dts)
        self._check(self.lib.vc_solve_from(self._h, B, *ptrs, flags))
        return u0, xbar, u_out, status, iters

    def solve_debug(self, x0, kappa, ds, ubar):
        B, N, nx, f = self._batch(x0), self.N, self.nx, np.float32
        stride = self.lib.vc_debug_stride()
        xbar, u0 = np.empty((B, self.ns_solve, nx), f), np.empty((B, NU), f)
        status, iters, dbg = np.empty(B, np.int32), np.empty(B, np.int32), np.empty((B, stride), f)
        ptrs, flags = self._marshal([x0, kappa, ds, xbar, ubar, u0, status, iters, dbg],
                                    [(B, nx), (B, N), (B, N), (B, self.ns_solve, nx), (B, N, NU), (B, NU), (B,),
                                     (B,), (B, stride)], [f] * 6 + [np.int32, np.int32, f])
        self._check(self.lib.vc_solve_debug(self._h, B, *ptrs, flags))
        n = 2 * N
        return dict(u0=u0, xbar=xbar, ubar=ubar, status=status, iters=iters, g=dbg[:, :n],
                    M=dbg[:, n:n + n * n].reshape(B, n, n), Y=dbg[:, n + n * n:n + 2 * n * n].reshape(B, n, n),
                    rhs=dbg[:, n + 2 * n * n:2 * n + 2 * n * n], dz=dbg[:, 2 * n + 2 * n * n:3 * n + 2 * n * n])

    def debug_kin_merit(self, x0, kappa, ds, u_prev, u, status, iters, st_acc, it_acc, first=True, restart=False,
                        x_prev=None, x=None):
        B, N, nx, f = self._batch(x0), self.N, self.nx, np.float64
        ms = bool(self.params.qp.ms)
        if ms and (x is None or x_prev is None):
            raise ValueError("vc_qp.ms: pass the state iterate x_prev and the QP's x")
        x = self._like(x0, (B, N + 1, nx)) if x is None else x
        u0, diag = self._like(x0, (B, NU)), self._like(x0, (B, 4))
        bufs = [x0, kappa, ds, u_prev, u] + ([x_prev] if ms else []) + [x, status, iters, st_acc, it_acc, u0, diag]
        xs = [(B, N + 1, nx)]
        shapes = [(B, nx), (B, N), (B, N), (B, N, NU), (B, N, NU)] + xs * ms + xs + [(B,)] * 4 + [(B, NU), (B, 4)]
        dts = [f] * (6 + ms) + [np.int32] * 4 + [f, f]
        p, flags = self._marshal(bufs, shapes, dts)
        if not ms:
            p.insert(5, C.c_void_p(0))
        self._check(self.lib.vc_debug_kin_merit(self._h, B, *p[:11], int(bool(first)), int(bool(restart)), *p[11:],
                                                flags))
        return u0, x, u, status, iters, diag

    def rollout(self, x0, ubar, kappa, ds):
        B, N, nx, f = self._batch(x0), self.N, self.nx, _NP_DT[self.dtype]
        xbar = self._like(x0, (B, N + 1, nx))
        ptrs, flags = self._marshal([x0, ubar, kappa, ds, xbar],
                                    [(B, nx), (B, N, NU), (B, N), (B, N), (B, N + 1, nx)], [f] * 5)
        self._check(self.lib.vc_rollout(self._h, B, *ptrs, flags))
        return xbar

    def linearize(self, xbar, ubar, kappa, ds):
        B, N, nx, f = self._batch(xbar), self.N, self.nx, _NP_DT[self.dtype]
        A = self._like(xbar, (B, N, nx, nx))
        Bm = self._like(xbar, (B, N, nx, NU))
        ptrs, flags = self._marshal([xbar, ubar, kappa, ds, A, Bm],
                                    [(B, N + 1, nx), (B, N, NU), (B, N), (B, N), (B, N, nx, nx), (B, N, nx, NU)],
                                    [f] * 6)
        self._check(self.lib.vc_linearize(self._h, B, *ptrs, flags))
        return A, Bm

    def condense(self, x0, ubar, kappa, ds):
        B, N, nx, f = self._batch(x0), self.NH, self.nx, _NP_DT[self.dtype]
        n = NU * N
        H = self._like(x0, (B, n, n))
        g = self._like(x0, (B, n))
        ptrs, flags = self._marshal([x0, ubar, kappa, ds, H, g],
                                    [(B, nx), (B, N, NU), (B, N), (B, N), (B, n, n), (B, n)], [f] * 6)
        self._check(self.lib.vc_condense(self._h, B, *ptrs, flags))
        return H, g

    def plant_step(self, x, u, kappa, dt):
        B, nx, f = self._batch(x), self.nx, _NP_DT[self.dtype]
        xn = self._like(x, (B, nx))
        px, pu, pk, pxn = self._marshal([x, u, kappa, xn], [(B, nx), (B, NU), (B,), (B, nx)], [f] * 4)[0]
        flags = _abi.VC_DEVICE_PTRS if _is_torch(x) else _abi.VC_HOST_PTRS
        self._check(self.lib.vc_plant_step(self._h, B, px, pu, pk, float(dt), pxn, flags))
        return xn

    def ode(self, x, u, kappa, space=False):
        B, nx, f = self._batch(x), self.nx, _NP_DT[self.dtype]
        fo = self._like(x, (B, nx))
        ptrs, flags = self._marshal([x, u, kappa, fo], [(B, nx), (B, NU), (B,), (B, nx)], [f] * 4)
        p = ptrs
        self._check(self.lib.vc_ode(self._h, B, p[0], p[1], p[2], int(bool(space)), p[3], flags))
        return fo

    def spatial_step(self, x, u, kappa, ds):
        B, nx, f = self._batch(x), self.nx, _NP_DT[self.dtype]
        xn = self._like(x, (B, nx))
        ptrs, flags = self._marshal([x, u, kappa, ds, xn], [(B, nx), (B, NU), (B,), (B,), (B, nx)], [f] * 5)
        self._check(self.lib.vc_spatial_step(self._h, B, *ptrs, flags))
        return xn

    def set_track(self, track):
        coef, h, length = track.kappa_table()
        coef = np.ascontiguousarray(coef, np.float64)
        self._check(self.lib.vc_track_set(self._h, int(coef.shape[0]), float(h), float(length),
                                          C.c_void_p(coef.ctypes.data)))
        self.track = track

    def track_k(self, s):
        B, f = self._batch(s), _NP_DT[self.dtype]
        k = self._like(s, (B,))
        ptrs, flags = self._marshal([s, k], [(B,), (B,)], [f, f])
        self._check(self.lib.vc_track_k(self._h, B, *ptrs, flags))
        return k

    def horizon(self, x0, xbar, mpc_dt):
        B, N, nx, f = self._batch(x0), self.NH, self.nx, _NP_DT[self.dtype]
        kappa, ds = self._like(x0, (B, N)), self._like(x0, (B, N))
        ptrs, flags = self._marshal([x0, xbar, kappa, ds], [(B, nx), (B, self.ns_solve, nx), (B, N), (B, N)], [f] * 4)
        self._check(self.lib.vc_horizon(self._h, B, ptrs[0], ptrs[1], float(mpc_dt), ptrs[2], ptrs[3], flags))
        return kappa, ds

    def drive(self, x64, u0, dt, x_ctx=None):
        B, nx, f = self._batch(x64), self.nx, _NP_DT[self.dtype]
        arrs, shapes, dts = [x64, u0], [(B, nx), (B, NU)], [np.float64, f]
        if x_ctx is not None:
            arrs, shapes, dts = arrs + [x_ctx], shapes + [(B, nx)], dts + [f]
        ptrs, flags = self._marshal(arrs, shapes, dts)
        xc = ptrs[2] if x_ctx is not None else None
        self._check(self.lib.vc_drive(self._h, B, ptrs[0], ptrs[1], float(dt), xc, flags))
        return x64

    def simulate(self, x64, xbar, ubar, steps, mpc_dt, dt, log=False, nfail=None):
        B, N, nx, f = self._batch(x64), self.NH, self.nx, _NP_DT[self.dtype]
        steps = int(steps)
        dev = _is_torch(x64)
        if nfail is None:
            if dev:
                import torch
                nfail = torch.zeros((B,), dtype=torch.int32, device=x64.device)
            else:
                nfail = np.zeros((B,), np.int32)
        arrs = [x64, xbar, ubar, nfail]
        shapes = [(B, nx), (B, self.ns_solve, nx), (B, N, NU), (B,)]
        dts = [np.float64, f, f, np.int32]
        log_x = log_u = None
        if log:
            if dev:
                import torch
                log_x = torch.empty((steps + 1, B, nx), dtype=torch.float64, device=x64.device)
                log_u = torch.empty((steps, B, NU), dtype=xbar.dtype, device=x64.device)
            else:
                log_x, log_u = np.empty((steps + 1, B, nx)), np.empty((steps, B, NU), f)
            arrs, shapes, dts = arrs + [log_x, log_u], shapes + [(steps + 1, B, nx), (steps, B, NU)], dts + [np.float64, f]
        ptrs, flags = self._marshal(arrs, shapes, dts)
        lx, lu = (ptrs[4], ptrs[5]) if log else (None, None)
        self._check(self.lib.vc_simulate(self._h, B, steps, float(mpc_dt), float(dt), ptrs[0], ptrs[1], ptrs[2],
                                         lx, lu, ptrs[3], flags))
        return log_x, log_u, nfail

    def _like(self, ref, shape):
        if _is_torch(ref):
            import torch
            return torch.empty(shape, dtype=ref.dtype, device=ref.device)
        return np.empty(shape, _NP_DT[self.dtype])
```

Measured before the change: 5.959 million solves/s.

## Hand-schedule Cholesky back-substitution in asm and precompute G-dot lane plans in AGPRs

Replaces the compiler-generated backward substitution in chol_solve with a hand-written inline-asm sweep. It streams L columns from LDS through ds_read_b128 quads with explicit lgkmcnt waits and fuses it with the existing asm forward sweep. The per-lane address plans for grow_dot and gt_dot are now computed once per solve and parked in AGPRs, so the repeated index arithmetic is replaced by accvgpr reads. The dinv load is hoisted out of the AL inner loop. The change also adds a debug trisolve kernel and ABI entry for testing, at the cost of hard-coded VGPR clobbers (v236-v255) that may increase register pressure.

```diff
diff --git a/include/vcmpc.h b/include/vcmpc.h
--- a/include/vcmpc.h
+++ b/include/vcmpc.h
@@ -150,6 +150,9 @@
 int vc_debug_kin_gdots(vc_ctx* ctx, int B, const void* G, const void* vz, const void* vc, void* out_grow,
                        void* out_gt, int flags);
 
+int vc_debug_kin_trisolve(vc_ctx* ctx, int B, const void* L, const void* dinv, const void* b, void* out,
+                          int flags);
+
 int vc_rollout(vc_ctx* ctx, int B, const void* x0, const void* ubar, const void* kappa,
                const void* ds, void* xbar, int flags);
 
diff --git a/vehicle-control_amd/csrc/kin_ltv.hip b/vehicle-control_amd/csrc/kin_ltv.hip
--- a/vehicle-control_amd/csrc/kin_ltv.hip
+++ b/vehicle-control_amd/csrc/kin_ltv.hip
@@ -42,9 +42,6 @@
 #endif
 #ifndef KIN_STEP_F
 #define KIN_STEP_F 0.99
-#endif
-#ifndef KIN_SOLVE_CH
-#define KIN_SOLVE_CH 8
 #endif
 #ifndef KIN_PANEL_CH
 #define KIN_PANEL_CH 6
@@ -222,7 +219,7 @@
   static constexpr int T = NC / 2;
   static constexpr int ROW_SHORT = T - (T + 1) / 2;
   static_assert(NC + 2 * (N - 1 - ROW_SHORT) <= 64, "partner lanes of the long rows");
-  static constexpr int COL_LONG = n / 2;
+  static constexpr int COL_LONG = n / 2, COL_D2 = 9;
   static_assert(n + COL_LONG <= 64, "partner lanes of the long columns");
 };
 
@@ -273,48 +270,87 @@
 }
 
 template <int N>
-__device__ double grow_dot(const Smem<N>& s, int lane) {
+struct GPlan {
+  int rg0, rg2, rv0, rv2, rf;
+  int cg[4], cv[4], cf;
+};
+__device__ __forceinline__ int agpr_put(uint32_t v) {
+  int a;
+  asm("v_accvgpr_write_b32 %0, %1" : "=a"(a) : "v"(v));
+  return a;
+}
+template <int N>
+__device__ __forceinline__ GPlan<N> gplan_make(const Smem<N>& s, int lane) {
   using P = GSplit<N>;
-  constexpr int NC = P::NC, LD = P::LD;
+  constexpr int n = P::n, NC = P::NC, LD = P::LD;
   const int l = lane_opaque(lane);
-  const bool part = l >= NC;
-  const bool shrt = uint32_t(l) < uint32_t(P::ROW_SHORT) || uint32_t(l - (N - 1)) < uint32_t(P::ROW_SHORT);
-  const int r = min(part ? l - (l < NC + (N - 1 - P::ROW_SHORT) ? NC - P::ROW_SHORT : N) : l, NC);
-  const uint32_t odd = part ? 8u : 0u;
-  const uint32_t fwd = shrt ? 0u : 8u * uint32_t(P::T);
-  const uint32_t g0 = (uint32_t)(uintptr_t)(lds_cdouble*)&s.G[0][0] + uint32_t(r) * (8u * LD) + odd;
-  const uint32_t v0 = (uint32_t)(uintptr_t)(lds_cdouble*)&s.vz[0] + odd;
-  const uint32_t g[4] = {g0, g0, g0 + fwd, g0 + fwd}, v[4] = {v0, v0, v0 + fwd, v0 + fwd};
+  GPlan<N> pl;
+  {
+    const bool part = l >= NC;
+    const bool shrt = uint32_t(l) < uint32_t(P::ROW_SHORT) || uint32_t(l - (N - 1)) < uint32_t(P::ROW_SHORT);
+    const int r = min(part ? l - (l < NC + (N - 1 - P::ROW_SHORT) ? NC - P::ROW_SHORT : N) : l, NC);
+    const uint32_t odd = part ? 8u : 0u;
+    const uint32_t fwd = shrt ? 0u : 8u * uint32_t(P::T);
+    const uint32_t g0 = (uint32_t)(uintptr_t)(lds_cdouble*)&s.G[0][0] + uint32_t(r) * (8u * LD) + odd;
+    const uint32_t v0 = (uint32_t)(uintptr_t)(lds_cdouble*)&s.vz[0] + odd;
+    pl.rg0 = agpr_put(g0);
+    pl.rg2 = agpr_put(g0 + fwd);
+    pl.rv0 = agpr_put(v0);
+    pl.rv2 = agpr_put(v0 + fwd);
+    pl.rf = agpr_put(uint32_t(4 * (l + (l < N - 1 ? NC - P::ROW_SHORT : N))));
+  }
+  {
+    const bool part = l >= n;
+    const bool shrt = uint32_t(l - P::COL_LONG) < uint32_t(n - P::COL_LONG);
+    const int j = part ? l - n : l;
+    const uint32_t ms = shrt ? 1u : 0u, mp = part ? 1u : 0u;
+    const uint32_t gp = (uint32_t)(uintptr_t)(lds_cdouble*)&s.G[0][0] + uint32_t(j) * 8u + mp * (8u * LD);
+    const uint32_t vp = (uint32_t)(uintptr_t)(lds_cdouble*)&s.vc[0] + mp * 8u;
+    constexpr int SH[4] = {10, 18, 0, 1};
+#pragma unroll
+    for (int k = 0; k < 4; ++k) {
+      const int D = k == 2 ? P::COL_D2 : 0;
+      pl.cg[k] = agpr_put(gp + uint32_t(D * 8 * LD) + ms * uint32_t((SH[k] - D) * 8 * LD));
+      pl.cv[k] = agpr_put(vp + uint32_t(D * 8) + ms * uint32_t((SH[k] - D) * 8));
+    }
+    pl.cf = agpr_put(uint32_t(4 * (l + n)));
+  }
+  return pl;
+}
+
+template <int N>
+__device__ double grow_dot(const GPlan<N>& pl, int lane) {
+  using P = GSplit<N>;
+  uint32_t g0, g2, v0, v2, f;
+  asm volatile("v_accvgpr_read_b32 %0, %5\n\tv_accvgpr_read_b32 %1, %6\n\tv_accvgpr_read_b32 %2, %7\n\t"
+               "v_accvgpr_read_b32 %3, %8\n\tv_accvgpr_read_b32 %4, %9"
+               : "=v"(g0), "=v"(g2), "=v"(v0), "=v"(v2), "=v"(f)
+               : "a"(pl.rg0), "a"(pl.rg2), "a"(pl.rv0), "a"(pl.rv2), "a"(pl.rf));
+  const bool shrt = g2 == g0;
+  const uint32_t g[4] = {g0, g0, g2, g2}, v[4] = {v0, v0, v2, v2};
   double stash;
   const double acc = gsplit_chain<N, 1, P::T, P::T>(g, v, shrt, stash);
-  const double other = lane_fetch(acc, 4 * (l + (l < N - 1 ? NC - P::ROW_SHORT : N)));
+  const double other = lane_fetch(acc, int(f));
   const double y = acc + (shrt ? stash : other);
-  return l < NC ? y : 0.0;
-}
-
-template <int N>
-__device__ double gt_dot(const Smem<N>& s, int lane) {
+  return lane_opaque(lane) < P::NC ? y : 0.0;
+}
+
+template <int N>
+__device__ double gt_dot(const GPlan<N>& pl, int lane) {
   using P = GSplit<N>;
-  constexpr int n = P::n, LD = P::LD;
-  const int l = lane_opaque(lane);
-  const bool part = l >= n;
-  const bool shrt = uint32_t(l - P::COL_LONG) < uint32_t(n - P::COL_LONG);
-  const int j = part ? l - n : l;
-  const uint32_t ms = shrt ? 1u : 0u, mp = part ? 1u : 0u;
-  const uint32_t gp = (uint32_t)(uintptr_t)(lds_cdouble*)&s.G[0][0] + uint32_t(j) * 8u + mp * (8u * LD);
-  const uint32_t vp = (uint32_t)(uintptr_t)(lds_cdouble*)&s.vc[0] + mp * 8u;
-  constexpr int SH[4] = {10, 18, 0, 1}, D[4] = {0, 0, 9, 0};
-  uint32_t g[4], v[4];
-#pragma unroll
-  for (int k = 0; k < 4; ++k) {
-    g[k] = gp + uint32_t(D[k] * 8 * LD) + ms * uint32_t((SH[k] - D[k]) * 8 * LD);
-    v[k] = vp + uint32_t(D[k] * 8) + ms * uint32_t((SH[k] - D[k]) * 8);
-  }
+  uint32_t g[4], v[4], f;
+  asm volatile("v_accvgpr_read_b32 %0, %9\n\tv_accvgpr_read_b32 %1, %10\n\tv_accvgpr_read_b32 %2, %11\n\t"
+               "v_accvgpr_read_b32 %3, %12\n\tv_accvgpr_read_b32 %4, %13\n\tv_accvgpr_read_b32 %5, %14\n\t"
+               "v_accvgpr_read_b32 %6, %15\n\tv_accvgpr_read_b32 %7, %16\n\tv_accvgpr_read_b32 %8, %17"
+               : "=v"(g[0]), "=v"(g[1]), "=v"(g[2]), "=v"(g[3]), "=v"(v[0]), "=v"(v[1]), "=v"(v[2]), "=v"(v[3]), "=v"(f)
+               : "a"(pl.cg[0]), "a"(pl.cg[1]), "a"(pl.cg[2]), "a"(pl.cg[3]), "a"(pl.cv[0]), "a"(pl.cv[1]),
+                 "a"(pl.cv[2]), "a"(pl.cv[3]), "a"(pl.cf));
+  const bool shrt = g[1] != g[0];
   double stash;
-  const double acc = gsplit_chain<N, LD, D[2], D[3]>(g, v, shrt, stash);
-  const double other = lane_fetch(acc, 4 * (l + n));
+  const double acc = gsplit_chain<N, P::LD, P::COL_D2, 0>(g, v, shrt, stash);
+  const double other = lane_fetch(acc, int(f));
   const double y = acc + (shrt ? stash : other);
-  return l < n ? y : 0.0;
+  return lane_opaque(lane) < P::n ? y : 0.0;
 }
 
 
@@ -378,74 +414,110 @@
   "v_accvgpr_read_b32 v255, %[h" #k "]\n\t"      \
   "v_fma_f64 %[acc], -v[254:255], vcc, %[acc]\n\t"
 #define KIN_FS_ROW(k) [l##k] "a"(Lr.lo[k]), [h##k] "a"(Lr.hi[k])
+#define KIN_FS_STEPS                                                 \
+  KIN_FS_STEP(0,63,1) KIN_FS_STEP(1,62,2) KIN_FS_STEP(2,61,3)        \
+  KIN_FS_STEP(3,60,4) KIN_FS_STEP(4,59,5) KIN_FS_STEP(5,58,6)        \
+  KIN_FS_STEP(6,57,7) KIN_FS_STEP(7,56,8) KIN_FS_STEP(8,55,9)        \
+  KIN_FS_STEP(9,54,10) KIN_FS_STEP(10,53,11) KIN_FS_STEP(11,52,12)   \
+  KIN_FS_STEP(12,51,13) KIN_FS_STEP(13,50,14) KIN_FS_STEP(14,49,15)  \
+  KIN_FS_STEP(15,48,16) KIN_FS_STEP(16,47,17) KIN_FS_STEP(17,46,18)  \
+  KIN_FS_STEP(18,45,19) KIN_FS_STEP(19,44,20) KIN_FS_STEP(20,43,21)  \
+  KIN_FS_STEP(21,42,22) KIN_FS_STEP(22,41,23) KIN_FS_STEP(23,40,24)  \
+  KIN_FS_STEP(24,39,25) KIN_FS_STEP(25,38,26) KIN_FS_STEP(26,37,27)  \
+  KIN_FS_STEP(27,36,28) KIN_FS_STEP(28,35,29) KIN_FS_STEP(29,34,30)  \
+  KIN_FS_STEP(30,33,31) KIN_FS_STEP(31,32,32) KIN_FS_STEP(32,31,33)  \
+  KIN_FS_STEP(33,30,34) KIN_FS_STEP(34,29,35) KIN_FS_STEP(35,28,36)  \
+  KIN_FS_STEP(36,27,37) KIN_FS_STEP(37,26,38) KIN_FS_STEP(38,25,39)  \
+  KIN_FS_STEP(39,24,40)
+#define KIN_FS_ROWS                                                                                       \
+  KIN_FS_ROW(0), KIN_FS_ROW(1), KIN_FS_ROW(2), KIN_FS_ROW(3), KIN_FS_ROW(4), KIN_FS_ROW(5),               \
+  KIN_FS_ROW(6), KIN_FS_ROW(7), KIN_FS_ROW(8), KIN_FS_ROW(9), KIN_FS_ROW(10), KIN_FS_ROW(11),             \
+  KIN_FS_ROW(12), KIN_FS_ROW(13), KIN_FS_ROW(14), KIN_FS_ROW(15), KIN_FS_ROW(16), KIN_FS_ROW(17),         \
+  KIN_FS_ROW(18), KIN_FS_ROW(19), KIN_FS_ROW(20), KIN_FS_ROW(21), KIN_FS_ROW(22), KIN_FS_ROW(23),         \
+  KIN_FS_ROW(24), KIN_FS_ROW(25), KIN_FS_ROW(26), KIN_FS_ROW(27), KIN_FS_ROW(28), KIN_FS_ROW(29),         \
+  KIN_FS_ROW(30), KIN_FS_ROW(31), KIN_FS_ROW(32), KIN_FS_ROW(33), KIN_FS_ROW(34), KIN_FS_ROW(35),         \
+  KIN_FS_ROW(36), KIN_FS_ROW(37), KIN_FS_ROW(38), KIN_FS_ROW(39)
 template <int N>
 __device__ __forceinline__ void forward_sweep(const RowRegs<N>& Lr, double& acc, double dj) {
   static_assert(Dims<N>::n == 40, "the sweep's 40 steps are written out");
   asm("s_mov_b64 s[98:99], exec\n\t"
-      KIN_FS_STEP(0,63,1) KIN_FS_STEP(1,62,2) KIN_FS_STEP(2,61,3)
-      KIN_FS_STEP(3,60,4) KIN_FS_STEP(4,59,5) KIN_FS_STEP(5,58,6)
-      KIN_FS_STEP(6,57,7) KIN_FS_STEP(7,56,8) KIN_FS_STEP(8,55,9)
-      KIN_FS_STEP(9,54,10) KIN_FS_STEP(10,53,11) KIN_FS_STEP(11,52,12)
-      KIN_FS_STEP(12,51,13) KIN_FS_STEP(13,50,14) KIN_FS_STEP(14,49,15)
-      KIN_FS_STEP(15,48,16) KIN_FS_STEP(16,47,17) KIN_FS_STEP(17,46,18)
-      KIN_FS_STEP(18,45,19) KIN_FS_STEP(19,44,20) KIN_FS_STEP(20,43,21)
-      KIN_FS_STEP(21,42,22) KIN_FS_STEP(22,41,23) KIN_FS_STEP(23,40,24)
-      KIN_FS_STEP(24,39,25) KIN_FS_STEP(25,38,26) KIN_FS_STEP(26,37,27)
-      KIN_FS_STEP(27,36,28) KIN_FS_STEP(28,35,29) KIN_FS_STEP(29,34,30)
-      KIN_FS_STEP(30,33,31) KIN_FS_STEP(31,32,32) KIN_FS_STEP(32,31,33)
-      KIN_FS_STEP(33,30,34) KIN_FS_STEP(34,29,35) KIN_FS_STEP(35,28,36)
-      KIN_FS_STEP(36,27,37) KIN_FS_STEP(37,26,38) KIN_FS_STEP(38,25,39)
-      KIN_FS_STEP(39,24,40)
+      KIN_FS_STEPS
       "s_mov_b64 exec, s[98:99]"
       : [acc] "+v"(acc)
-      : [dj] "v"(dj),
-        KIN_FS_ROW(0), KIN_FS_ROW(1), KIN_FS_ROW(2), KIN_FS_ROW(3), KIN_FS_ROW(4), KIN_FS_ROW(5),
-        KIN_FS_ROW(6), KIN_FS_ROW(7), KIN_FS_ROW(8), KIN_FS_ROW(9), KIN_FS_ROW(10), KIN_FS_ROW(11),
-        KIN_FS_ROW(12), KIN_FS_ROW(13), KIN_FS_ROW(14), KIN_FS_ROW(15), KIN_FS_ROW(16), KIN_FS_ROW(17),
-        KIN_FS_ROW(18), KIN_FS_ROW(19), KIN_FS_ROW(20), KIN_FS_ROW(21), KIN_FS_ROW(22), KIN_FS_ROW(23),
-        KIN_FS_ROW(24), KIN_FS_ROW(25), KIN_FS_ROW(26), KIN_FS_ROW(27), KIN_FS_ROW(28), KIN_FS_ROW(29),
-        KIN_FS_ROW(30), KIN_FS_ROW(31), KIN_FS_ROW(32), KIN_FS_ROW(33), KIN_FS_ROW(34), KIN_FS_ROW(35),
-        KIN_FS_ROW(36), KIN_FS_ROW(37), KIN_FS_ROW(38), KIN_FS_ROW(39)
+      : [dj] "v"(dj), KIN_FS_ROWS
       : "vcc", "s98", "s99", "v252", "v253", "v254", "v255");
 }
+
+#define KIN_BS_Q0 "v[236:239]"
+#define KIN_BS_Q1 "v[240:243]"
+#define KIN_BS_Q2 "v[244:247]"
+#define KIN_BS_Q3 "v[248:251]"
+#define KIN_BS_L0 "v[236:237]"
+#define KIN_BS_H0 "v[238:239]"
+#define KIN_BS_L1 "v[240:241]"
+#define KIN_BS_H1 "v[242:243]"
+#define KIN_BS_L2 "v[244:245]"
+#define KIN_BS_H2 "v[246:247]"
+#define KIN_BS_L3 "v[248:249]"
+#define KIN_BS_H3 "v[250:251]"
+#define KIN_BS_HEAD(k)                       \
+  "v_mul_f64 v[252:253], %[acc], %[dj]\n\t"  \
+  "s_bfm_b64 exec, " #k ", 0\n\t"            \
+  "v_readlane_b32 vcc_lo, v252, " #k "\n\t"  \
+  "v_readlane_b32 vcc_hi, v253, " #k "\n\t"
+#define KIN_BS_FMA(reg) "v_fma_f64 %[acc], -" reg ", vcc, %[acc]\n\t"
+#define KIN_BS_READ(q, off) "ds_read_b128 " KIN_BS_Q##q ", %[col] offset:" #off "\n\t"
+#define KIN_BS_EVEN(k, q) KIN_BS_HEAD(k) "s_nop 1\n\t" KIN_BS_FMA(KIN_BS_L##q)
+#define KIN_BS_ODD(k, q, w) KIN_BS_HEAD(k) "s_waitcnt lgkmcnt(" #w ")\n\ts_nop 0\n\t" KIN_BS_FMA(KIN_BS_H##q)
+#define KIN_BS_PAIR(ko, ke, q, rq, off)                                                          \
+  KIN_BS_HEAD(ko) "s_waitcnt lgkmcnt(2)\n\t" KIN_BS_READ(rq, off) KIN_BS_FMA(KIN_BS_H##q) KIN_BS_EVEN(ke, q)
+#define KIN_BS_PAIR_NR(ko, ke, q, w) KIN_BS_ODD(ko, q, w) KIN_BS_EVEN(ke, q)
+#define KIN_BS_STEPS                                                                                  \
+  KIN_BS_PAIR(39,38,3,0,256) KIN_BS_PAIR(37,36,2,3,240) KIN_BS_PAIR(35,34,1,2,224)                    \
+  KIN_BS_PAIR(33,32,0,1,208) KIN_BS_PAIR(31,30,3,0,192) KIN_BS_PAIR(29,28,2,3,176)                    \
+  KIN_BS_PAIR(27,26,1,2,160) KIN_BS_PAIR(25,24,0,1,144) KIN_BS_PAIR(23,22,3,0,128)                    \
+  KIN_BS_PAIR(21,20,2,3,112) KIN_BS_PAIR(19,18,1,2,96) KIN_BS_PAIR(17,16,0,1,80)                      \
+  KIN_BS_PAIR(15,14,3,0,64) KIN_BS_PAIR(13,12,2,3,48) KIN_BS_PAIR(11,10,1,2,32)                       \
+  KIN_BS_PAIR(9,8,0,1,16) KIN_BS_PAIR(7,6,3,0,0) KIN_BS_PAIR_NR(5,4,2,2) KIN_BS_PAIR_NR(3,2,1,1)     \
+  KIN_BS_ODD(1,0,0)
+
+template <int N>
+__device__ double chol_solve(const RowRegs<N>& Lr, const Smem<N>& s, double b, int lane, double dj) {
+  constexpr int n = Dims<N>::n;
+  static_assert(n == 40, "the sweeps' 40 steps are written out");
+  const int row = lane < n ? lane : 0;
+  const uint32_t col = (uint32_t)(uintptr_t)lds_opaque(&s.Lc[lc_base<n>(row)]);
+  double acc = b;
+  asm volatile("s_mov_b64 s[98:99], exec\n\t"
+               KIN_BS_READ(3, 304) KIN_BS_READ(2, 288) KIN_BS_READ(1, 272)
+               KIN_FS_STEPS
+               "s_mov_b64 exec, s[98:99]\n\t"
+               "v_mul_f64 %[acc], %[acc], %[dj]\n\t"
+               KIN_BS_STEPS
+               "s_mov_b64 exec, s[98:99]\n\t"
+               "v_mul_f64 %[acc], %[acc], %[dj]"
+               : [acc] "+v"(acc)
+               : [dj] "v"(dj), [col] "v"(col), KIN_FS_ROWS
+               : "vcc", "s98", "s99", "v236", "v237", "v238", "v239", "v240", "v241", "v242", "v243", "v244", "v245",
+                 "v246", "v247", "v248", "v249", "v250", "v251", "v252", "v253", "v254", "v255", "memory");
+  return lane < n ? acc : 0.0;
+}
+template <int N>
+__device__ double chol_solve(const RowRegs<N>& Lr, const Smem<N>& s, double b, int lane) {
+  return chol_solve<N>(Lr, s, b, lane, s.dinv[lane < Dims<N>::n ? lane : 0]);
+}
+#undef KIN_BS_STEPS
+#undef KIN_BS_PAIR_NR
+#undef KIN_BS_PAIR
+#undef KIN_BS_ODD
+#undef KIN_BS_EVEN
+#undef KIN_BS_READ
+#undef KIN_BS_FMA
+#undef KIN_BS_HEAD
+#undef KIN_FS_STEPS
+#undef KIN_FS_ROWS
 #undef KIN_FS_STEP
 #undef KIN_FS_ROW
-
-template <int N>
-__device__ double chol_solve(const RowRegs<N>& Lr, const Smem<N>& s, double b, int lane) {
-  constexpr int n = Dims<N>::n;
-  constexpr int CH = KIN_SOLVE_CH;
-  static_assert(n % CH == 0, "backward prefetch chunks");
-  const int row = lane < n ? lane : 0;
-  lds_cdouble* col = lds_opaque(&s.Lc[lc_base<n>(row)]);
-  const double dj = s.dinv[row];
-  double acc = b;
-  forward_sweep<N>(Lr, acc, dj);
-  acc *= dj;
-  double x = 0.0;
-  double lk[2][CH];
-  lds_cdouble* zero = lds_opaque(&s.zrow[0]);
-  auto fetch = [&](int c, int buf) {
-    lds_cdouble* src = row < n - 1 - c * CH ? col : zero;
-#pragma unroll
-    for (int q = 0; q < CH; ++q) lk[buf][q] = src[n - 1 - c * CH - q];
-  };
-  fetch(0, 0);
-#pragma unroll
-  for (int c = 0; c < n / CH; ++c) {
-    if (c + 1 < n / CH) fetch(c + 1, (c + 1) & 1);
-    fence();
-#pragma unroll
-    for (int q = 0; q < CH; ++q) {
-      const int k = n - 1 - c * CH - q;
-      const double xk = lane_bcast(acc * dj, k);
-      x = lane_put(x, xk, k);
-      acc -= lk[c & 1][q] * xk;
-    }
-    fence();
-  }
-  return x;
-}
 
 enum { ROWS_G = 0, ROWS_E = 1 };
 template <int N, int KIND>
@@ -857,6 +929,7 @@
   for (int i = lane; i < 2 * D::LD; i += 64) (&s.G[NC][0])[i] = 0.0;
   if (lane < 48) s.zrow[lane] = 0.0;
   if (lane == 0) s.Lc[Smem<N>::LC_ZERO] = 0.0;
+  const GPlan<N> gpl = gplan_make<N>(s, lane);
   wave_sync();
 
   VC_TSTAMP(t_sweep0)
@@ -1102,11 +1175,11 @@
     s.vz[lane] = (lane < n) ? z : 0.0;
     s.vc[lane] = (lane < NC) ? (cs.lhi - cs.llo) : 0.0;
     wave_sync();
-    const double yc = grow_dot<N>(s, lane);
+    const double yc = grow_dot<N>(gpl, lane);
     fence();
     const double hz = h_dot<N>(s, lane);
     fence();
-    const double gtl = gt_dot<N>(s, lane);
+    const double gtl = gt_dot<N>(gpl, lane);
     rd = (lane < n) ? (hz + gj + (bx.lhi - bx.llo) + gtl) : 0.0;
     rlo_b = bx.hasLo ? (z - bx.lo - bx.slo) : 0.0;
     rhi_b = bx.hasHi ? (bx.hi - z - bx.shi) : 0.0;
@@ -1155,7 +1228,7 @@
             wave_sync();
             s.vc[lane] = (lane < NC) ? (cs.lhi - cs.llo) : 0.0;
             wave_sync();
-            const double gtl = gt_dot<N>(s, lane);
+            const double gtl = gt_dot<N>(gpl, lane);
             const double cmax = wave_max(lane < n ? fabs((bx.lhi - bx.llo) + gtl) : 0.0);
             if (__builtin_fma(Rbox, cmax, dl) / l1 < -A.detect_eps) {
               infeas = true;
@@ -1205,6 +1278,7 @@
       const double islo_c = cs.hasLo ? rcp_nr(cs.slo) : 0.0, ishi_c = cs.hasHi ? rcp_nr(cs.shi) : 0.0;
       const double illo_b = bx.hasLo ? rcp_nr(bx.llo) : 0.0, ilhi_b = bx.hasHi ? rcp_nr(bx.lhi) : 0.0;
       const double illo_c = cs.hasLo ? rcp_nr(cs.llo) : 0.0, ilhi_c = cs.hasHi ? rcp_nr(cs.lhi) : 0.0;
+      const double dj = s.dinv[lane < n ? lane : 0];
       double sm = 0.0, pp1 = 0.0, pp2 = 0.0, pp3 = 0.0, pp4 = 0.0;
 #pragma unroll 1
       for (int pass = 0; pass < 2; ++pass) {
@@ -1220,15 +1294,15 @@
         wave_sync();
         s.vc[lane] = (lane < NC) ? ec : 0.0;
         wave_sync();
-        const double gte = gt_dot<N>(s, lane);
+        const double gte = gt_dot<N>(gpl, lane);
         const double rhs = (lane < n) ? (-rd - eb - gte) : 0.0;
         VC_TSTAMP(t_sol0)
-        const double dz = chol_solve<N>(Mr, s, rhs, lane);
+        const double dz = chol_solve<N>(Mr, s, rhs, lane, dj);
         VC_TACC(T_SOLVE, t_sol0)
         wave_sync();
         s.vz[lane] = (lane < n) ? dz : 0.0;
         wave_sync();
-        const double dyc = grow_dot<N>(s, lane);
+        const double dyc = grow_dot<N>(gpl, lane);
         const double d1 = bx.hasLo ? dz + rlo_b : 0.0;
         const double d2 = bx.hasLo ? __builtin_fma(islo_b, -rclo_b, -(wlo_b * (dz + rlo_b))) : 0.0;
         const double d3 = bx.hasHi ? rhi_b - dz : 0.0;
@@ -1312,7 +1386,7 @@
       wave_sync();
       s.vz[lane] = (lane < n) ? zfix : 0.0;
       wave_sync();
-      const double gfix = grow_dot<N>(s, lane);
+      const double gfix = grow_dot<N>(gpl, lane);
       double gn2 = 0.0;
       {
         const int r = lane < NC ? lane : 0;
@@ -1372,16 +1446,17 @@
       const double bnd_al = alo_c ? cs.lo : cs.hi;
       double zp = 0.0, emax = 0.0;
       {
+        const double dj = s.dinv[lane < n ? lane : 0];
         wave_sync();
         s.vc[lane] = (lane < NC) ? (nu_c - rho_c * bnd_c) : 0.0;
         wave_sync();
-        const double gtn = gt_dot<N>(s, lane);
+        const double gtn = gt_dot<N>(gpl, lane);
         const double rhs = (lane < n) ? (fixed ? zfix : (base - gtn)) : 0.0;
-        zp = chol_solve<N>(Mr, s, rhs, lane);
+        zp = chol_solve<N>(Mr, s, rhs, lane, dj);
         wave_sync();
         s.vz[lane] = (lane < n) ? zp : 0.0;
         wave_sync();
-        const double yr = grow_dot<N>(s, lane);
+        const double yr = grow_dot<N>(gpl, lane);
         double rr = al_act ? (yr - bnd_al) : 0.0;
         const double ie = 1.0 / (1e-14 * scale), inu = KIN_NU_TOL > 0.0 ? 1.0 / (KIN_NU_TOL * scale) : 0.0;
         auto crit = [&](double r) { return wave_max(fmax(fabs(r) * ie, fabs(rho_c * r) * inu)); };
@@ -1397,12 +1472,12 @@
             wave_sync();
             s.vc[lane] = (lane < NC) ? pd : 0.0;
             wave_sync();
-            const double gtp = gt_dot<N>(s, lane);
-            const double zq = chol_solve<N>(Mr, s, (lane < n && !fixed) ? gtp : 0.0, lane);
+            const double gtp = gt_dot<N>(gpl, lane);
+            const double zq = chol_solve<N>(Mr, s, (lane < n && !fixed) ? gtp : 0.0, lane, dj);
             wave_sync();
             s.vz[lane] = (lane < n) ? zq : 0.0;
             wave_sync();
-            const double gq = grow_dot<N>(s, lane);
+            const double gq = grow_dot<N>(gpl, lane);
             const double q = al_act ? gq : 0.0;
             const double pq = wave_sum(pd * q);
 #ifdef VC_TIMING
@@ -1426,9 +1501,9 @@
       s.vz[lane] = (lane < n) ? zp : 0.0;
       s.vc[lane] = (lane < NC) ? nu_c : 0.0;
       wave_sync();
-      const double gtnu = gt_dot<N>(s, lane);
+      const double gtnu = gt_dot<N>(gpl, lane);
       const double grad = (lane < n) ? (h_dot<N>(s, lane) + gj + gtnu) : 0.0;
-      const double ypc = grow_dot<N>(s, lane);
+      const double ypc = grow_dot<N>(gpl, lane);
 #if KIN_STAT_CHECK
       emax = wave_max(fmax(al_act ? fabs(ypc - bnd_al) : 0.0, (lane < n && !fixed) ? fabs(grad) : 0.0));
 #else
@@ -1551,7 +1626,7 @@
     }
   }
   {
-    const double y = grow_dot<N>(s, lane);
+    const double y = grow_dot<N>(gpl, lane);
     const int slot = lane < N - 1 ? 64 + lane + 1
                                   : (lane < NC ? n + (lane - (N - 1)) + 1 : (lane == NC ? 64 : (lane == NC + 1 ? n : 127)));
     wave_sync();
@@ -1627,9 +1702,42 @@
   for (int i = lane; i < NC * n; i += 64) s.G[i / n][i % n] = G[(size_t)b * NC * n + i];
   s.vz[lane] = lane < n ? vz[(size_t)b * n + lane] : 0.0;
   s.vc[lane] = lane < NC ? vc[(size_t)b * NC + lane] : 0.0;
-  wave_sync();
-  out_grow[(size_t)b * 64 + lane] = grow_dot<N>(s, lane);
-  out_gt[(size_t)b * 64 + lane] = gt_dot<N>(s, lane);
+  const GPlan<N> gpl = gplan_make<N>(s, lane);
+  wave_sync();
+  out_grow[(size_t)b * 64 + lane] = grow_dot<N>(gpl, lane);
+  out_gt[(size_t)b * 64 + lane] = gt_dot<N>(gpl, lane);
+}
+
+template <int N>
+__global__ __launch_bounds__(64) void kin_trisolve_kernel(int B, const double* L, const double* dinv,
+                                                          const double* rhs, double* out) {
+  constexpr int n = Dims<N>::n;
+  __shared__ Smem<N> s;
+  const int lane = threadIdx.x;
+  const int b = blockIdx.x;
+  if (b >= B) return;
+  const double* Lb = L + (size_t)b * n * n;
+  for (int i = lane; i < Smem<N>::LC_ZERO + 1; i += 64) s.Lc[i] = 0.0;
+  if (lane < 48) s.zrow[lane] = 0.0;
+  s.dinv[lane] = lane < n ? dinv[(size_t)b * n + lane] : 0.0;
+  wave_sync();
+  for (int i = lane; i < n * n; i += 64) {
+    const int j = i / n, k = i % n;
+    if (j >= k) s.Lc[lc_base<n>(k) + j] = Lb[i];
+  }
+  RowRegs<N> Lr;
+#pragma unroll
+  for (int k = 0; k < n; ++k) row_put<N>(Lr, k, lane < n ? Lb[lane * n + k] : __builtin_nan(""));
+  wave_sync();
+  out[(size_t)b * 64 + lane] = chol_solve<N>(Lr, s, rhs[(size_t)b * 64 + lane], lane);
+}
+
+hipError_t launch_kin_trisolve(int B, int N, const double* L, const double* dinv, const double* rhs, double* out,
+                               hipStream_t stream) {
+  if (B <= 0) return hipSuccess;
+  if (N != 20) return hipErrorInvalidValue;
+  hipLaunchKernelGGL(kin_trisolve_kernel<20>, dim3(B), dim3(64), 0, stream, B, L, dinv, rhs, out);
+  return hipGetLastError();
 }
 
 hipError_t launch_kin_gdots(int B, int N, const double* G, const double* vz, const double* vc, double* out_grow,
diff --git a/vehicle-control_amd/csrc/vc_kernels.hpp b/vehicle-control_amd/csrc/vc_kernels.hpp
--- a/vehicle-control_amd/csrc/vc_kernels.hpp
+++ b/vehicle-control_amd/csrc/vc_kernels.hpp
@@ -277,6 +277,8 @@
 hipError_t launch_rcp_probe(int n, const double* x, double* out, hipStream_t st);
 hipError_t launch_kin_gdots(int B, int N, const double* G, const double* vz, const double* vc, double* out_grow,
                             double* out_gt, hipStream_t stream);
+hipError_t launch_kin_trisolve(int B, int N, const double* L, const double* dinv, const double* rhs, double* out,
+                               hipStream_t stream);
 hipError_t launch_kin_qp_fault(const KinLtvArgs& a, int N, int b, hipStream_t stream);
 bool kin_ric_built(int N);
 hipError_t launch_dyn_sqp(const DynSqpArgs& a, int N, hipStream_t stream);
diff --git a/vehicle-control_amd/csrc/vcmpc_abi.hip b/vehicle-control_amd/csrc/vcmpc_abi.hip
--- a/vehicle-control_amd/csrc/vcmpc_abi.hip
+++ b/vehicle-control_amd/csrc/vcmpc_abi.hip
@@ -767,6 +767,26 @@
   return st.finish();
 }
 
+int vc_debug_kin_trisolve(vc_ctx* c, int B, const void* L, const void* dinv, const void* b, void* out, int flags) {
+  if (int r = check_common(c, B, flags)) return r;
+  if (c->model != VC_MODEL_KINEMATIC || c->dtype != VC_F64 || vc::kin_ltv_smem_bytes(c->N) == 0)
+    return fail(c, VC_E_UNSUPPORTED, "vc_debug_kin_trisolve: kinematic fp64 contexts with the fused kernel's N only");
+  if (!L || !dinv || !b || !out) return fail(c, VC_E_ARG, "null pointer");
+  if (B == 0) return 0;
+  const int N = c->N, n = 2 * N;
+  Ptr dL, dd, db, dout;
+  Staging st(c, flags);
+  if (int r = st.bind([&] {
+        dL = st.in(L, (size_t)B * n * n * 8);
+        dd = st.in(dinv, (size_t)B * n * 8);
+        db = st.in(b, (size_t)B * 64 * 8);
+        dout = st.out(out, (size_t)B * 64 * 8);
+      }))
+    return r;
+  VC_HIP(c, vc::launch_kin_trisolve(B, N, dL, dd, db, dout, c->stream));
+  return st.finish();
+}
+
 int vc_debug_qp_fault(vc_ctx* c, int sqp_iter, int problem) {
   if (!c) return VC_E_ARG;
   c->fault_iter = sqp_iter;
diff --git a/vehicle-control_amd/vcmpc/_abi.py b/vehicle-control_amd/vcmpc/_abi.py
--- a/vehicle-control_amd/vcmpc/_abi.py
+++ b/vehicle-control_amd/vcmpc/_abi.py
@@ -104,6 +104,7 @@
     "vc_debug_kin_merit": (C.c_int, [_vp, C.c_int] + [_vp] * 11 + [C.c_int, C.c_int, _vp, _vp, C.c_int]),
     "vc_debug_rcp": (C.c_int, [_vp, C.c_int, _vp, _vp, C.c_int]),
     "vc_debug_kin_gdots": (C.c_int, [_vp, C.c_int, _vp, _vp, _vp, _vp, _vp, C.c_int]),
+    "vc_debug_kin_trisolve": (C.c_int, [_vp, C.c_int, _vp, _vp, _vp, _vp, C.c_int]),
     "vc_rollout": (C.c_int, [_vp, C.c_int, _vp, _vp, _vp, _vp, _vp, C.c_int]),
     "vc_linearize": (C.c_int, [_vp, C.c_int, _vp, _vp, _vp, _vp, _vp, _vp, C.c_int]),
     "vc_condense": (C.c_int, [_vp, C.c_int, _vp, _vp, _vp, _vp, _vp, _vp, C.c_int]),
diff --git a/vehicle-control_amd/vcmpc/solver.py b/vehicle-control_amd/vcmpc/solver.py
--- a/vehicle-control_amd/vcmpc/solver.py
+++ b/vehicle-control_amd/vcmpc/solver.py
@@ -252,6 +252,13 @@
                                                 flags))
         return u0, x, u, status, iters, diag
 
+    def debug_kin_trisolve(self, L, dinv, b):
+        B, n, f = self._batch(L), 2 * self.N, np.float64
+        out = self._like(L, (B, 64))
+        ptrs, flags = self._marshal([L, dinv, b, out], [(B, n, n), (B, n), (B, 64), (B, 64)], [f] * 4)
+        self._check(self.lib.vc_debug_kin_trisolve(self._h, B, *ptrs, flags))
+        return out
+
     def rollout(self, x0, ubar, kappa, ds):
         B, N, nx, f = self._batch(x0), self.N, self.nx, _NP_DT[self.dtype]
         xbar = self._like(x0, (B, N + 1, nx))
```

Result: faster. 6.022 million solves/s (median of 6 runs) (+1.0%).
